# mulns/AccFlow

Hardware: AMD Instinct MI355X
Metric: frame-pairs/s (estimator pair-evals/s), AccFlow(RAFT) 7-frame 480x1024 backward accumulation (higher is better)
Workload: dtype f32 (direct-kernel operands split into 2 fp16 terms - activations kept pre-split in HBM as fp16 hi+lo, 4 B per element; other kernels 3 bf16 terms; f32 accumulate)

## Files before the change

### accflow_amd/_lib.py

```python
import ctypes
import os
import threading

_HERE = os.path.dirname(os.path.abspath(__file__))
LIB_PATH = os.environ.get("ACCFLOW_HIP_LIB") or os.path.join(_HERE, "lib", "libaccflow_hip.so")

ABI_VERSION = 20
c_f = ctypes.c_void_p
c_ll = ctypes.c_longlong
c_i = ctypes.c_int


class ConvSrc(ctypes.Structure):
    _fields_ = [
        ("ptr", c_f), ("bs", c_ll),
        ("C", c_i), ("Hs", c_i), ("Ws", c_i),
        ("step", c_i), ("oy", c_i), ("ox", c_i),
        ("KH", c_i), ("KW", c_i), ("padH", c_i), ("padW", c_i),
        ("reserved", c_i),
    ]


MAX_SRC = 4


class ConvDesc(ctypes.Structure):
    _fields_ = [
        ("in0", c_f), ("in1", c_f),
        ("in0_bs", c_ll), ("in1_bs", c_ll),
        ("C0", c_i), ("C1", c_i),
        ("B", c_i), ("H", c_i), ("W", c_i),
        ("OH", c_i), ("OW", c_i),
        ("KH", c_i), ("KW", c_i), ("stride", c_i), ("padH", c_i), ("padW", c_i),
        ("Cout", c_i),
        ("wpack", c_f), ("ktab", c_f),
        ("Kpad", c_i), ("CoutPad", c_i),
        ("bias", c_f),
        ("out", c_f), ("out_bs", c_ll),
        ("act", c_i), ("epi", c_i),
        ("e0", c_f), ("e0_bs", c_ll),
        ("e1", c_f), ("e1_bs", c_ll),
        ("out2", c_f), ("out2_bs", c_ll),
        ("offset", c_f), ("offset_bs", c_ll),
        ("dmask", c_f), ("dmask_bs", c_ll),
        ("wsplit", c_f), ("mode", c_i),
        ("wpatch", c_f),
        ("wsplit_bs", c_ll),
        ("kws", c_f), ("kws_elems", c_ll),
        ("wpatch16", c_f), ("guard", c_f),
        ("wscale16", c_f), ("wsplit16", c_f), 
        ("stats", c_f), ("stat_slots", c_i), ("pre", c_f), ("pre_bs", c_ll), ("in_norm", c_f), ("acc_scale", ctypes.c_float),
        ("in_fmt", c_i), ("out16", c_f), ("out16_bs", c_ll),
        ("cb", c_i), ("out_cbs", c_ll), ("e0_cbs", c_ll), ("out16_cbs", c_ll),
        ("nsrc", c_i), ("src", ConvSrc * MAX_SRC),
        ("e0_fmt", c_i),
        ("tg_w16", c_f), ("tg_scale", c_f), ("tg_out", c_f), ("tg_out_bs", c_ll), ("tg_out_ps", c_ll),
        ("tg_rows", c_i), ("tg_coutpad", c_i),
        ("split_c0", c_i), ("p32", c_i),
    ]


SIGNATURES = {
    "accflow_abi_version": [],
    "accflow_conv_desc_bytes": [],
    "accflow_conv_src_bytes": [],
    "accflow_s16_item_words": [c_i, c_i, c_i],
    "accflow_to_s16_f32": [c_f, c_ll, c_f, c_ll, c_f, c_i, c_i, c_i, c_f],
    "accflow_conv_kpad": [c_i, c_i, c_i],
    "accflow_conv_coutpad": [c_i],
    "accflow_conv_pack_f32": [c_f, c_f, c_i, c_i, c_i, c_i, c_i, c_i, c_f, c_f, c_f],
    "accflow_conv_pack_bf16s": [c_f, c_f, c_i, c_i, c_i, c_i, c_f, c_f],
    "accflow_conv_patch_elems": [c_i, c_i, c_i, c_i],
    "accflow_conv_pack_patch": [c_f, c_f, c_i, c_i, c_i, c_i, c_f, c_f],
    "accflow_conv_pack_patch16": [c_f, c_f, c_i, c_i, c_i, c_i, c_f, c_f, c_f],
    "accflow_conv_pack_split16": [c_f, c_f, c_i, c_i, c_i, c_i, c_f, c_f, c_f],
    "accflow_conv_multi_pack_elems": [c_i, c_i, ctypes.POINTER(c_i), ctypes.POINTER(c_i), ctypes.POINTER(c_i)],
    "accflow_conv_pack_multi16": [ctypes.POINTER(c_f), c_f, c_i, c_i, ctypes.POINTER(c_i), ctypes.POINTER(c_i), ctypes.POINTER(c_i),
                                  c_f, c_f, c_f],
    "accflow_conv2d_f32": [ctypes.POINTER(ConvDesc), c_f],
    "accflow_conv_stat_slots": [ctypes.POINTER(ConvDesc)],
    "accflow_conv_in_norm_supported": [ctypes.POINTER(ConvDesc)],
    "accflow_conv_plan_query": [ctypes.POINTER(ConvDesc), ctypes.POINTER(c_i), c_i],
    "accflow_conv_gru16_supported": [],
    "accflow_instance_stats_finalize_f32": [c_f, c_i, c_f, c_i, c_i, ctypes.c_float, c_f],
    "accflow_instance_norm_apply_f32": [c_f, c_f, c_i, c_f, c_f, c_f, c_i, c_i, c_i, ctypes.c_float, c_i, c_f],
    "accflow_instance_norm_apply_s16_f32": [c_f, c_f, c_i, c_f, c_f, c_f, c_f, c_ll, c_f, c_i, c_i, c_i, ctypes.c_float, c_i, c_f],
    "accflow_instance_norm_apply_s16res_f32": [c_f, c_f, c_i, c_f, c_f, c_ll, c_f, c_f, c_ll, c_f, c_i, c_i, c_i, ctypes.c_float, c_f],
    "accflow_instance_stats_finalize_sub_f32": [c_f, c_i, c_i, c_i, c_f, c_i, c_i, ctypes.c_float, c_f],
    "accflow_instance_norm_apply_s16proj_f32": [c_f, c_f, c_i, c_f, c_ll, c_f, c_i, c_i, c_i, c_f, c_f, c_ll, c_f, c_i, c_i, c_i,
                                                ctypes.c_float, c_f],
    "accflow_get_occ_s16": [c_f, c_ll, c_f, c_ll, c_f, c_ll, c_f, c_ll, c_f, c_i, c_i, c_i, c_i, c_i, c_f],
    "accflow_blend_s16": [c_f, c_f, c_f, c_f, c_ll, c_f, c_i, c_i, c_i, c_f],
    "accflow_deform_columns_s16": [c_f, c_ll, c_f, c_ll, c_f, c_ll, c_i, c_f, c_ll, c_f, c_i, c_i, c_i, c_i, c_i, c_i, c_i, c_i, c_f],
    "accflow_corr_volume_f32": [c_f, c_f, c_f, c_f, c_f, c_f, c_i, c_i, c_i, c_i, c_f],
    "accflow_corr_volume_ws_bytes": [c_i, c_i, c_i],
    "accflow_corr_volume_split_f32": [c_f, c_f, c_f, c_f, c_f, c_f, c_f, c_i, c_i, c_i, c_i, c_i, c_f],
    "accflow_corr_lookup_f32": [c_f, c_f, c_f, c_f, c_f, c_f, c_ll, c_i, c_i, c_i, c_f],
    "accflow_corr_lookup_r3_f32": [c_f, c_f, c_f, c_f, c_f, c_f, c_ll, c_i, c_i, c_i, c_f],
    "accflow_corr_disp_supported": [c_i, c_i],
    "accflow_corr_disp_level_elems": [c_i, c_i, c_i],
    "accflow_corr_volume_disp_f32": [c_f, c_f, c_f, c_f, c_f, c_f, c_f, c_i, c_f, c_i, c_i, c_i, c_i, c_f],
    "accflow_corr_pack_bytes": [c_i, c_i, c_i],
    "accflow_corr_pack_f32": [c_f, c_f, c_i, c_f, c_i, c_i, c_i, c_i, c_f],
    "accflow_corr_volume_disp_packed_f32": [c_f, c_i, ctypes.POINTER(c_i), ctypes.POINTER(c_i), c_f, c_f, c_f, c_f, c_i, c_f, c_i, c_i, c_i,
                                            c_i, c_f],
    "accflow_corr_disp_pool_f32": [c_f, c_f, c_f, c_f, c_i, c_i, c_i, c_f],
    "accflow_corr_lookup_disp_f32": [c_f, c_f, c_f, c_f, c_f, c_f, c_ll, c_i, c_i, c_i, c_f],
    "accflow_corr_lookup_disp_s16": [c_f, c_f, c_f, c_f, c_f, c_f, c_ll, c_f, c_i, c_i, c_i, c_f],
    "accflow_corr_alt_pyramid_elems": [c_i, c_i, c_i],
    "accflow_corr_alt_pyramid_f32": [c_f, c_f, c_i, c_i, c_i, c_i, c_f],
    "accflow_corr_lookup_alt_f32": [c_f, c_i, c_f, c_f, c_f, c_ll, c_i, c_i, c_i, c_i, c_f],
    "accflow_corr_lookup_alt_s16": [c_f, c_i, c_f, c_f, c_f, c_ll, c_f, c_i, c_i, c_i, c_i, c_f],
    "accflow_corr_lookup_convc1_kpad": [],
    "accflow_corr_lookup_convc1_s16": [c_f, c_f, c_f, c_f, c_f, c_f, c_f, c_f, c_f, c_ll, c_f, c_ll, c_i, c_f, c_i, c_i, c_i, c_i, c_f],
    "accflow_flow_from_coords_s16": [c_f, c_f, c_ll, c_f, c_ll, c_f, c_ll, c_f, c_ll, c_i, c_f, c_i, c_i, c_i, c_i, c_f],
    "accflow_convex_upsample_f32": [c_f, c_ll, c_f, c_ll, c_f, c_i, c_i, c_i, c_f],
    "accflow_backwarp_f32": [c_f, c_ll, c_f, c_ll, c_f, c_ll, c_i, c_i, c_i, c_i, c_f],
    "accflow_compose_flow_f32": [c_f, c_ll, c_f, c_ll, c_f, c_ll, c_i, c_i, c_i, c_f],
    "accflow_get_occ_f32": [c_f, c_ll, c_f, c_ll, c_f, c_ll, c_f, c_ll, c_i, c_i, c_i, c_i, c_i, c_f],
    "accflow_downflow8_f32": [c_f, c_f, c_i, c_i, c_i, c_i, c_f],
    "accflow_upflow8_f32": [c_f, c_ll, c_f, c_ll, c_i, c_i, c_i, c_f],
    "accflow_forward_interpolate_f32": [c_f, c_f, c_i, c_i, c_i, c_f],
    "accflow_fb_occlusion_f32": [c_f, c_ll, c_f, c_ll, c_f, c_ll, c_f, c_ll, ctypes.c_float, ctypes.c_float, c_i, c_i, c_i, c_f],
    "accflow_flow_metrics_ws_bytes": [c_i, c_i, c_i],
    "accflow_flow_metrics_f32": [c_f, c_ll, c_f, c_ll, c_f, c_ll, c_f, c_ll, c_i, ctypes.c_float, ctypes.c_float, c_f, c_f, c_i, c_i,
                                 c_i, c_f],
    "accflow_instance_norm_f32": [c_f, c_f, c_f, c_i, c_i, c_i, ctypes.c_float, c_i, c_f],
    "accflow_split_tanh_relu_f32": [c_f, c_f, c_ll, c_f, c_ll, c_i, c_i, c_i, c_i, c_f],
    "accflow_split_tanh_relu_idx_f32": [c_f, c_i, ctypes.POINTER(c_i), c_f, c_ll, c_f, c_ll, c_i, c_i, c_i, c_i, c_f],
    "accflow_coords_grid_f32": [c_f, c_f, c_i, c_i, c_i, c_f],
    "accflow_flow_from_coords_f32": [c_f, c_f, c_ll, c_f, c_ll, c_f, c_i, c_i, c_i, c_i, c_f],
    "accflow_deform_columns_f32": [c_f, c_ll, c_f, c_ll, c_f, c_ll, c_f, c_i, c_i, c_i, c_i, c_i, c_i, c_i, c_i, c_f],
    "accflow_conv_pack_all_f32": [c_f, c_f, c_i, c_i, c_i, c_i, c_i, c_i, c_i, c_f, c_f, c_f, c_f, c_f, c_f, c_f, c_f],
    "accflow_tap_sum_f32": [c_f, c_f, c_f, c_ll, c_f, c_ll, c_i, c_i, c_i, c_i, c_i, c_i, c_i, c_i, c_i, c_i, c_f],
    "accflow_tap_sum_parts_f32": [c_f, c_i, c_ll, c_ll, c_f, c_f, c_ll, c_f, c_ll, c_i, c_i, c_i, c_i, c_i, c_i, c_i, c_i, c_i, c_i, c_f],
    "accflow_blend_f32": [c_f, c_f, c_f, c_f, c_i, c_i, c_i, c_f],
    "accflow_activation_f32": [c_f, c_ll, c_i, c_i, c_i, c_i, c_f],
    "accflow_copy_f32": [c_f, c_ll, c_f, c_ll, c_i, c_i, c_i, c_f],
    "accflow_gma_attention_f32": [c_f, c_f, c_i, c_i, c_i, ctypes.c_float, c_f],
    "accflow_gma_attention_ws_bytes": [c_i, c_i, c_i],
    "accflow_gma_attention_t_f32": [c_f, c_f, c_f, c_i, c_i, c_i, c_i, c_i, ctypes.c_float, c_f],
    "accflow_gma_aggregate_ws_bytes": [c_i, c_i, c_i],
    "accflow_gma_attention_s16_ws_bytes": [c_i, c_i, c_i],
    "accflow_gma_attention_s16": [c_f, c_f, c_f, c_f, c_i, c_i, c_i, c_i, ctypes.c_float, c_f],
    "accflow_gma_aggregate_s16_ws_bytes": [c_i, c_i, c_i],
    "accflow_gma_aggregate_s16": [c_f, c_f, c_f, c_ll, c_f, c_f, c_ll, c_f, c_ll, c_f, c_f, c_i, c_i, c_i, c_i, c_f],
    "accflow_gma_attention_alt_ws_bytes": [c_i, c_i, c_i],
    "accflow_gma_attention_alt": [c_f, c_f, c_f, c_f, c_f, c_f, c_i, c_i, c_i, c_i, ctypes.c_float, c_f],
    "accflow_gma_aggregate_alt_ws_bytes": [c_i, c_i, c_i],
    "accflow_gma_aggregate_alt": [c_f, c_f, c_f, c_f, c_f, c_ll, c_f, c_f, c_ll, c_f, c_ll, c_f, c_f, c_i, c_i, c_i, c_i, c_f],
    "accflow_gma_aggregate_t_f32": [c_f, c_f, c_f, c_f, c_f, c_ll, c_f, c_i, c_f, c_i, c_i, c_i, c_i, c_f],
    "accflow_gma_aggregate_f32": [c_f, c_f, c_f, c_f, c_f, c_ll, c_i, c_i, c_i, c_f],
    "accflow_gma_pos_tables_f32": [c_f, c_f, c_f, c_f, c_i, c_i, c_i, c_i, c_i, ctypes.c_float, c_f],
    "accflow_gma_attention_pos_f32": [c_f, c_f, c_f, c_i, c_i, c_i, c_i, c_i, ctypes.c_float, c_f],
    "accflow_gma_attention_pos_ws_bytes": [c_i, c_i, c_i, c_i, c_i],
    "accflow_gma_attention_pos_t": [c_f, c_f, c_f, c_f, c_f, c_i, c_i, c_i, c_i, c_i, c_i, ctypes.c_float, c_f],
    "accflow_act_backward_f32": [c_f, c_ll, c_f, c_ll, c_f, c_ll, c_i, c_ll, c_i, c_f],
    "accflow_add_f32": [c_f, c_ll, c_f, c_ll, c_i, c_ll, c_f],
    "accflow_l1_grad_f32": [c_f, c_f, c_f, c_ll, ctypes.c_float, c_f],
    "accflow_dilate_f32": [c_f, c_ll, c_f, c_i, c_i, c_i, c_i, c_i, c_i, c_i, c_f],
    "accflow_blend_backward_f32": [c_f, c_f, c_f, c_f, c_f, c_f, c_f, c_i, c_i, c_i, c_f],
    "accflow_convex_upsample_backward_f32": [c_f, c_f, c_f, c_f, c_f, c_i, c_i, c_i, c_f],
    "accflow_conv_wgrad_f32": [c_f, c_ll, c_f, c_ll, c_f, c_f, c_i, c_i, c_i, c_i, c_i, c_i, c_i, c_i, c_i, c_i, c_f],
    "accflow_deform_conv_backward_f32": [c_f, c_ll, c_f, c_ll, c_f, c_ll, c_f, c_f, c_ll, c_f, c_f, c_i, c_i, c_i, c_i, c_i, c_i, c_i,
                                         c_i, c_f],
}

RETURNS_LONGLONG = frozenset((
    "accflow_conv_patch_elems", "accflow_conv_multi_pack_elems", "accflow_corr_pack_bytes", "accflow_corr_volume_ws_bytes",
    "accflow_gma_aggregate_ws_bytes", "accflow_gma_attention_ws_bytes", "accflow_gma_aggregate_s16_ws_bytes",
    "accflow_gma_attention_s16_ws_bytes", "accflow_gma_attention_alt_ws_bytes", "accflow_gma_aggregate_alt_ws_bytes",
    "accflow_corr_disp_level_elems", "accflow_corr_alt_pyramid_elems", "accflow_s16_item_words",
    "accflow_gma_attention_pos_ws_bytes", "accflow_flow_metrics_ws_bytes",
))

_lock = threading.Lock()
_lib = None


def _promote_hip_runtime():
    import torch
    cand = os.path.join(os.path.dirname(torch.__file__), "lib", "libamdhip64.so")
    if os.path.exists(cand):
        ctypes.CDLL(cand, mode=ctypes.RTLD_GLOBAL)
    else:
        ctypes.CDLL("libamdhip64.so", mode=ctypes.RTLD_GLOBAL)


def load():
    global _lib
    if _lib is not None:
        return _lib
    with _lock:
        if _lib is not None:
            return _lib
        if not os.path.exists(LIB_PATH):
            raise RuntimeError(
                "accflow_amd: %s not found - run `python -m accflow_amd.build` (hipcc, gfx950). "
                "There is no non-HIP fallback." % LIB_PATH)
        _promote_hip_runtime()
        lib = ctypes.CDLL(LIB_PATH)
        for name, argtypes in SIGNATURES.items():
            fn = getattr(lib, name)
            fn.argtypes = argtypes
            fn.restype = ctypes.c_longlong if name in RETURNS_LONGLONG else ctypes.c_int
        if lib.accflow_abi_version() != ABI_VERSION:
            raise RuntimeError("accflow_amd: ABI version mismatch")
        if (lib.accflow_conv_desc_bytes() != ctypes.sizeof(ConvDesc) or lib.accflow_conv_src_bytes() != ctypes.sizeof(ConvSrc)):
            raise RuntimeError("accflow_amd: accflow_conv_desc is %d / %d bytes in the library, %d / %d in _lib.py's mirror" % (
                lib.accflow_conv_desc_bytes(), lib.accflow_conv_src_bytes(), ctypes.sizeof(ConvDesc), ctypes.sizeof(ConvSrc)))
        _lib = lib
    return _lib
# ... 1 lines not shown
```

### accflow_amd/csrc/conv2d_direct.hip

```cpp
#include "conv2d_direct_kernel.h"

namespace {

__global__ __launch_bounds__(256) void conv_ksplit_reduce_kernel(const accflow_conv_desc d, int Z) {
  const int OHW = d.OH * d.OW;
  const long long n = (long long)d.B * d.Cout * OHW;
  const long long i = (long long)blockIdx.x * 256 + threadIdx.x;
  if (i >= n) return;
  const int px = (int)(i % OHW);
  const int ch = (int)((i / OHW) % d.Cout);
  const int b = (int)(i / ((long long)OHW * d.Cout));
  float v = d.kws[i];
  for (int z = 1; z < Z; ++z) v += d.kws[(long long)z * n + i];
  v = fmaf(v, d.wscale16 ? d.wscale16[(d.wsplit_bs ? (long long)b * d.CoutPad : 0) + ch] : 1.0f, d.bias ? d.bias[ch] : 0.0f);
  if (d.pre && (d.epi == ACCFLOW_EPI_GRU_ZR || d.epi == ACCFLOW_EPI_GRU_Q)) v += d.pre[b * d.pre_bs + (long long)ch * OHW + px];
  v = apply_act(v, d.act);
  const long long o = (long long)ch * OHW + px;
  const int half = d.Cout >> 1;
  if (d.cb) {
    const int blk = ch / d.cb;
    const long long oc = (long long)(ch - blk * d.cb) * OHW + px;
    const float r = d.epi == ACCFLOW_EPI_ACCUM ? d.e0[b * d.e0_bs + blk * d.e0_cbs + oc] + v : v;
    d.out[b * d.out_bs + blk * d.out_cbs + oc] = r;
    return;
  }
  switch (d.epi) {
    case ACCFLOW_EPI_RES_RELU: d.out[b * d.out_bs + o] = fmaxf(d.e0[b * d.e0_bs + o] + v, 0.0f); break;
    case ACCFLOW_EPI_GRU_ZR:
      if (ch < half) d.out[b * d.out_bs + o] = v;
      else d.out2[b * d.out2_bs + o - (long long)half * OHW] = v * d.e0[b * d.e0_bs + o - (long long)half * OHW];
      break;
    case ACCFLOW_EPI_GRU_Q: {
      const float z = d.e1[b * d.e1_bs + o], h = d.e0[b * d.e0_bs + o];
      d.out[b * d.out_bs + o] = gru_blend(z, h, v);
    } break;
    case ACCFLOW_EPI_ACCUM: d.out[b * d.out_bs + o] = d.e0[b * d.e0_bs + o] + v; break;
    default: d.out[b * d.out_bs + o] = v;
  }
}


__global__ __launch_bounds__(256) void conv_ksplit_reduce_s16_kernel(const accflow_conv_desc d, int Z) {
  const int OHW = d.OH * d.OW;
  const int O = (d.Cout + 7) >> 3;
  const long long n = (long long)d.B * d.Cout * OHW;
  const long long i = (long long)blockIdx.x * 256 + threadIdx.x;
  if (i >= (long long)d.B * O * OHW) return;
  const int px = (int)(i % OHW);
  const int oct = (int)((i / OHW) % O);
  const int b = (int)(i / ((long long)OHW * O));
  const int half = d.Cout >> 1;
  const bool zr = d.epi == ACCFLOW_EPI_GRU_ZR;
  float res[8];
  bool in16[8];
#pragma unroll
  for (int j = 0; j < 8; ++j) {
    const int ch = oct * 8 + j;
    res[j] = 0.0f;
    in16[j] = false;
    if (ch >= d.Cout) continue;
    const long long e = ((long long)b * d.Cout + ch) * OHW + px;
    float v = d.kws[e];
    for (int z = 1; z < Z; ++z) v += d.kws[(long long)z * n + e];
    v = fmaf(v, d.wscale16 ? d.wscale16[(d.wsplit_bs ? (long long)b * d.CoutPad : 0) + ch] : 1.0f, d.bias ? d.bias[ch] : 0.0f);
    if (d.pre && (zr || d.epi == ACCFLOW_EPI_GRU_Q)) v += d.pre[b * d.pre_bs + (long long)ch * OHW + px];
    v = apply_act(v, d.act);
    const long long o = (long long)ch * OHW + px;
    float r = v;
    if (d.cb) {
      const int blk = ch / d.cb;
      const long long oc = (long long)(ch - blk * d.cb) * OHW + px;
      r = d.epi == ACCFLOW_EPI_ACCUM ? d.e0[b * d.e0_bs + blk * d.e0_cbs + oc] + v : v;
      if (d.out) d.out[b * d.out_bs + blk * d.out_cbs + oc] = r;
      res[j] = r;
      in16[j] = true;
      continue;
    }
    switch (d.epi) {
      case ACCFLOW_EPI_RES_RELU: r = fmaxf(d.e0[b * d.e0_bs + o] + v, 0.0f); break;
      case ACCFLOW_EPI_GRU_ZR:
        if (ch >= half) r = v * d.e0[b * d.e0_bs + o - (long long)half * OHW];
        break;
      case ACCFLOW_EPI_GRU_Q: {
        const float z = d.e1[b * d.e1_bs + o], h = d.e0[b * d.e0_bs + o];
        r = gru_blend(z, h, v);
      } break;
      case ACCFLOW_EPI_ACCUM: r = d.e0[b * d.e0_bs + o] + v; break;
      default: break;
    }
    if (zr && ch >= half) {
      if (d.out2) d.out2[b * d.out2_bs + o - (long long)half * OHW] = r;
    } else if (d.out) {
      d.out[b * d.out_bs + o] = r;
    }
    res[j] = r;
    in16[j] = !zr || ch >= half;
  }
  if (!d.out16) return;
  const int c16 = oct * 8 - (zr ? half : 0);
  if (c16 < 0) return;
  const int n16 = zr ? half : d.Cout;
  const int nvalid = min(8, ((n16 + 1) & ~1) - c16);
  constexpr float ASC = (float)(1 << ACCFLOW_F16_ASHIFT);
  unsigned hi[4], lo[4];
  bool bad = false;
#pragma unroll
  for (int k = 0; k < 4; ++k) {
    const float a = in16[2 * k] ? res[2 * k] * ASC : 0.0f, c = in16[2 * k + 1] ? res[2 * k + 1] * ASC : 0.0f;
    bad |= !(fabsf(a) < 65520.0f) | !(fabsf(c) < 65520.0f);
    const f32x2 v2 = {a, c};
    const f16x2 hq = __builtin_convertvector(v2, f16x2);
    const f32x2 back = __builtin_convertvector(hq, f32x2);
    const f32x2 rest = {a - back[0], c - back[1]};
    const f16x2 lq = __builtin_convertvector(rest, f16x2);
    hi[k] = __builtin_bit_cast(unsigned, hq);
    lo[k] = __builtin_bit_cast(unsigned, lq);
  }
  unsigned* base = reinterpret_cast<unsigned*>(d.out16) + b * d.out16_bs;
  int o16 = c16 >> 3;
  if (d.cb) {
    base += (long long)(c16 / d.cb) * d.out16_cbs;
    o16 = (c16 % d.cb) >> 3;
  }
  unsigned* ph = base + (((long long)(o16 * 2 + 0)) * OHW + px) * 4;
  unsigned* pl = base + (((long long)(o16 * 2 + 1)) * OHW + px) * 4;
#pragma unroll
  for (int k = 0; k < 4; ++k)
    if (2 * k < nvalid) { ph[k] = hi[k]; pl[k] = lo[k]; }
  if (bad && d.guard) atomicOr(d.guard, 1);
}

__global__ __launch_bounds__(256) void conv_ksplit_reduce_s16q_kernel(const accflow_conv_desc d, int Z) {
  const int OHW = d.OH * d.OW;
  const int Q = d.Cout >> 2;
  const long long n = (long long)d.B * d.Cout * OHW;
  const long long i = (long long)blockIdx.x * 256 + threadIdx.x;
  if (i >= (long long)d.B * Q * OHW) return;
  const int px = (int)(i % OHW);
  const int q = (int)((i / OHW) % Q);
  const int b = (int)(i / ((long long)OHW * Q));
  float v[4];
#pragma unroll
  for (int j = 0; j < 4; ++j) v[j] = d.kws[((long long)b * d.Cout + q * 4 + j) * OHW + px];
  for (int z = 1; z < Z; ++z)
#pragma unroll
    for (int j = 0; j < 4; ++j) v[j] += d.kws[(long long)z * n + ((long long)b * d.Cout + q * 4 + j) * OHW + px];
  float res[4];
#pragma unroll
  for (int j = 0; j < 4; ++j) {
    const int ch = q * 4 + j;
    float t = fmaf(v[j], d.wscale16 ? d.wscale16[(d.wsplit_bs ? (long long)b * d.CoutPad : 0) + ch] : 1.0f, d.bias ? d.bias[ch] : 0.0f);
    if (d.pre && d.epi == ACCFLOW_EPI_GRU_Q) t += d.pre[b * d.pre_bs + (long long)ch * OHW + px];
    t = apply_act(t, d.act);
    const long long o = (long long)ch * OHW + px;
    if (d.cb) {
      const int blk = ch / d.cb;
      const long long oc = (long long)(ch - blk * d.cb) * OHW + px;
      if (d.epi == ACCFLOW_EPI_ACCUM) t = d.e0[b * d.e0_bs + blk * d.e0_cbs + oc] + t;
      if (d.out) d.out[b * d.out_bs + blk * d.out_cbs + oc] = t;
      res[j] = t;
      continue;
    }
    switch (d.epi) {
      case ACCFLOW_EPI_RES_RELU: t = fmaxf(d.e0[b * d.e0_bs + o] + t, 0.0f); break;
      case ACCFLOW_EPI_GRU_Q: {
        const float zz = d.e1[b * d.e1_bs + o], h = d.e0[b * d.e0_bs + o];
        t = gru_blend(zz, h, t);
      } break;
      case ACCFLOW_EPI_ACCUM: t = d.e0[b * d.e0_bs + o] + t; break;
      default: break;
    }
    if (d.out) d.out[b * d.out_bs + o] = t;
    res[j] = t;
  }
  constexpr float ASC = (float)(1 << ACCFLOW_F16_ASHIFT);
  unsigned hi[2], lo[2];
  bool bad = false;
#pragma unroll
  for (int k = 0; k < 2; ++k) {
    const float a = res[2 * k] * ASC, c = res[2 * k + 1] * ASC;
    bad |= !(fabsf(a) < 65520.0f) | !(fabsf(c) < 65520.0f);
    const f32x2 v2 = {a, c};
    const f16x2 hq = __builtin_convertvector(v2, f16x2);
    const f32x2 back = __builtin_convertvector(hq, f32x2);
    const f32x2 rest = {a - back[0], c - back[1]};
    const f16x2 lq = __builtin_convertvector(rest, f16x2);
    hi[k] = __builtin_bit_cast(unsigned, hq);
    lo[k] = __builtin_bit_cast(unsigned, lq);
  }
  unsigned* base = reinterpret_cast<unsigned*>(d.out16) + b * d.out16_bs;
  int oct = q >> 1;
  const int w0 = (q & 1) * 2;
  if (d.cb) {
    base += (long long)((q * 4) / d.cb) * d.out16_cbs;
    oct = ((q * 4) % d.cb) >> 3;
  }
  unsigned* ph = base + (((long long)(oct * 2 + 0)) * OHW + px) * 4 + w0;
  unsigned* pl = base + (((long long)(oct * 2 + 1)) * OHW + px) * 4 + w0;
  typedef unsigned u2_ __attribute__((ext_vector_type(2)));
  *reinterpret_cast<u2_*>(ph) = u2_{hi[0], hi[1]};
  *reinterpret_cast<u2_*>(pl) = u2_{lo[0], lo[1]};
  if (bad && d.guard) atomicOr(d.guard, 1);
}

}

int conv_ksplit_reduce_launch(const accflow_conv_desc& d, int Z, hipStream_t st) {
  if (d.out16 && !(d.Cout & 7) && !(d.cb & 7) && d.epi != ACCFLOW_EPI_GRU_ZR) {
    const long long nthr = (long long)d.B * (d.Cout / 4) * d.OH * d.OW;
    hipLaunchKernelGGL(conv_ksplit_reduce_s16q_kernel, dim3(cdiv(nthr, 256)), dim3(256), 0, st, d, Z);
  } else if (d.out16) {
    const long long nthr = (long long)d.B * ((d.Cout + 7) / 8) * d.OH * d.OW;
    hipLaunchKernelGGL(conv_ksplit_reduce_s16_kernel, dim3(cdiv(nthr, 256)), dim3(256), 0, st, d, Z);
  } else {
    const long long nout = (long long)d.B * d.Cout * d.OH * d.OW;
    hipLaunchKernelGGL(conv_ksplit_reduce_kernel, dim3(cdiv(nout, 256)), dim3(256), 0, st, d, Z);
  }
  ACCFLOW_RETURN_LAUNCH_STATUS();
}

namespace {

int launch_conv_direct(const accflow_conv_desc& d, const conv_plan& p, hipStream_t st) {
  const int tiles = cdiv(d.OW, DIR_TW) * cdiv(d.OH, DIR_TH);
  dim3 grid((unsigned)((long long)d.B * tiles), cdiv(d.Cout, 2 * p.tc * 32), p.Z);
  const bool f16 = p.mode == ACCFLOW_CONV_F16X3 && d.wpatch16;
  const int nt = p.mode == ACCFLOW_CONV_BF16X3 ? 2 : 3;
  int rc;
  if (p.tapgemm) {
    rc = p.loop == CONV_LOOP_TAP9 ? accflow_direct_launch_s16k9(d, 2, true, grid, st) : accflow_direct_launch_s16tg(d, grid, st);
  } else if (d.in_fmt) {
    if (p.loop == CONV_LOOP_TAP5) rc = accflow_direct_launch_s16k(d, 5, grid, st);
    else if (p.loop == CONV_LOOP_TAP9) rc = accflow_direct_launch_s16k9(d, p.tc, false, grid, st);
    else rc = accflow_direct_launch_s16(d, p.tc, grid, st);
  } else if (p.norm) {
// ... 447 lines not shown
```

### accflow_amd/csrc/conv_common.h

```cpp
#pragma once
#include "common.h"
#include <stdlib.h>
#include "launchers.h"

#ifndef ACCFLOW_EPI_GRU_AHEAD
#define ACCFLOW_EPI_GRU_AHEAD 3
#endif
#ifndef ACCFLOW_CONV_XCD_ORDER
#define ACCFLOW_CONV_XCD_ORDER 1
#endif
#ifndef ACCFLOW_CONV_XCD_MIN_K
#define ACCFLOW_CONV_XCD_MIN_K 8192
#endif

namespace {


struct XLoaderCtx {
  const float* base0;
  const float* base1;
  int iy0, ix0, H, W, HW;
  unsigned pixbyte0, pixbyte1;
  bool pvalid;
  const float* off;
  const float* dmk;
  int OHW, KW;
};

__device__ __forceinline__ float load_x_deform(const XLoaderCtx& c, const int4 e) {
  const float* src = e.w ? c.base1 : c.base0;
  if (!c.pvalid || e.y >= (1 << 19)) return 0.0f;
  const int tap = e.y * c.KW + e.z;
  const float dy = c.off[(2 * tap) * c.OHW], dx = c.off[(2 * tap + 1) * c.OHW];
  const float m = c.dmk[tap * c.OHW];
  const float h = (float)(c.iy0 + e.y) + dy, w = (float)(c.ix0 + e.z) + dx;
  if (!(h > -1.0f && h < (float)c.H && w > -1.0f && w < (float)c.W)) return 0.0f;
  const float* plane = src + e.x * c.HW;
  const float fh = floorf(h), fw = floorf(w);
  const int hl = (int)fh, wl = (int)fw, hh = hl + 1, wh = wl + 1;
  const float lh = h - fh, lw = w - fw, uh = 1.0f - lh, uw = 1.0f - lw;
  const float v1 = (hl >= 0 && wl >= 0) ? plane[hl * c.W + wl] : 0.0f;
  const float v2 = (hl >= 0 && wh <= c.W - 1) ? plane[hl * c.W + wh] : 0.0f;
  const float v3 = (hh <= c.H - 1 && wl >= 0) ? plane[hh * c.W + wl] : 0.0f;
  const float v4 = (hh <= c.H - 1 && wh <= c.W - 1) ? plane[hh * c.W + wh] : 0.0f;
  return m * (uh * uw * v1 + uh * lw * v2 + lh * uw * v3 + lh * lw * v4);
}

template <int CTRL>
__device__ __forceinline__ float dpp_add(float v) {
  return v + __builtin_bit_cast(float, __builtin_amdgcn_update_dpp(0, __builtin_bit_cast(int, v), CTRL, 0xF, 0xF, true));
}
__device__ __forceinline__ float row16_sum(float v) {
  v = dpp_add<0xB1>(v);
  v = dpp_add<0x4E>(v);
  v = dpp_add<0x141>(v);
  v = dpp_add<0x140>(v);
  return v;
}
__device__ __forceinline__ float half32_sum(float v) {
  v = row16_sum(v);
  return v + __builtin_bit_cast(float, __builtin_amdgcn_ds_swizzle(__builtin_bit_cast(int, v), 0x401F));
}
__device__ __forceinline__ void stat_store(const accflow_conv_desc& d, int b, int ch, int slot, float s, float m2, float n) {
  float* p = d.stats + (((long long)b * d.Cout + ch) * d.stat_slots + slot) * 3;
  p[0] = s; p[1] = m2; p[2] = n;
}

__device__ __forceinline__ float gru_blend(float z, float h, float q) { return __builtin_fmaf(z, q, (1.0f - z) * h); }

template <int EPI, int ACT, int WC, int WP, int TC, int TP, class PixMap, bool OUT16 = false>
__device__ __forceinline__ void conv_epilogue_impl(const accflow_conv_desc& d, f32x16 (&acc)[TC][TP], int cblk0, int wc,
                                                   int wp, int lane, int OHW, PixMap pixmap, int stat_b = 0,
                                                   int stat_slot = 0) {
  constexpr unsigned MASKED = 0xFFFFFFFFu;
  const int l31 = lane & 31, lh4 = (lane >> 5) * 4;
  const int epi = EPI >= 0 ? EPI : d.epi;
  const int half = d.Cout >> 1;
  const bool has_h = epi != ACCFLOW_EPI_STORE, has_z = epi == ACCFLOW_EPI_GRU_Q, zr = epi == ACCFLOW_EPI_GRU_ZR;
  const int nout = zr ? half : d.Cout;
  auto span = [&](long long bs, int nch) { return (int)(unsigned)((((long long)(d.B - 1)) * bs + (long long)nch * OHW) * 4); };
  const int cb = d.cb;
  auto chbyte = [&](int ch, long long cbs) -> int {
    if (!cb) return ch * OHW * 4;
    const int blk = ch / cb;
    return (int)(unsigned)(((long long)blk * cbs + (long long)(ch - blk * cb) * OHW) * 4);
  };
  auto span_cb = [&](long long bs, int nch, long long cbs) {
    if (!cb) return span(bs, nch);
    return (int)(unsigned)((((long long)(d.B - 1)) * bs + (long long)((nch - 1) / cb) * cbs + (long long)cb * OHW) * 4);
  };
  const __amdgpu_buffer_rsrc_t r_out =
      __builtin_amdgcn_make_buffer_rsrc(d.out, 0, d.out ? span_cb(d.out_bs, nout, d.out_cbs) : 0, 0x00020000);
  const __amdgpu_buffer_rsrc_t r_o2 =
      __builtin_amdgcn_make_buffer_rsrc(zr ? d.out2 : d.out, 0, (zr && d.out2) ? span(d.out2_bs, half) : 0, 0x00020000);
  const bool has16 = OUT16 && d.out16 != nullptr;
  const int n16 = zr ? half : d.Cout, O16 = (n16 + 7) >> 3;
  const __amdgpu_buffer_rsrc_t r_o16 = __builtin_amdgcn_make_buffer_rsrc(
      d.out16 ? d.out16 : (void*)d.out, 0,
      has16 ? (cb ? (int)(unsigned)((((long long)(d.B - 1)) * d.out16_bs + (long long)((n16 - 1) / cb) * d.out16_cbs +
                                     (long long)(cb / 8) * 2 * OHW * 4) * 4)
                  : (int)(unsigned)((((long long)(d.B - 1)) * d.out16_bs + (long long)O16 * 2 * OHW * 4) * 4)) : 0, 0x00020000);
  const __amdgpu_buffer_rsrc_t r_e0 = __builtin_amdgcn_make_buffer_rsrc(
      const_cast<float*>(has_h ? d.e0 : d.out), 0, has_h ? span_cb(d.e0_bs, zr ? half : d.Cout, d.e0_cbs) : 0, 0x00020000);
  const __amdgpu_buffer_rsrc_t r_e1 = __builtin_amdgcn_make_buffer_rsrc(
      const_cast<float*>(has_z ? d.e1 : d.out), 0, has_z ? span(d.e1_bs, d.Cout) : 0, 0x00020000);
  const bool has_pre = (EPI == ACCFLOW_EPI_GRU_ZR || EPI == ACCFLOW_EPI_GRU_Q) && d.pre != nullptr;
  const __amdgpu_buffer_rsrc_t r_pre = __builtin_amdgcn_make_buffer_rsrc(
      const_cast<float*>(has_pre ? d.pre : d.out), 0, has_pre ? span(d.pre_bs, d.Cout) : 0, 0x00020000);

  unsigned vo_out[TP], vo_o2[TP], vo_e0[TP], vo_e1[TP], vo_pre[TP], vo_16[TP];
#pragma unroll
  for (int tp = 0; tp < TP; ++tp) {
    int b;
    const int rem = pixmap(wp * TP * 32 + tp * 32 + l31, b);
    const bool ok = rem >= 0;
    const long long lp = (long long)rem + (long long)lh4 * OHW;
    vo_16[tp] = ok && has16 ? (unsigned)((b * d.out16_bs + (long long)rem * 4) * 4 + lh4 * 2) : MASKED;
    vo_out[tp] = ok ? (unsigned)((b * d.out_bs + lp) * 4) : MASKED;
    vo_o2[tp] = ok && zr ? (unsigned)((b * d.out2_bs + lp) * 4) : MASKED;
    vo_e0[tp] = ok && has_h ? (unsigned)((b * d.e0_bs + lp) * 4) : MASKED;
    vo_e1[tp] = ok && has_z ? (unsigned)((b * d.e1_bs + lp) * 4) : MASKED;
    vo_pre[tp] = ok && has_pre ? (unsigned)((b * d.pre_bs + lp) * 4) : MASKED;
  }
  const int rowbase = cblk0 + wc * TC * 32;
  const int OHW4 = OHW * 4;
  typedef const __attribute__((address_space(4))) float* cfloat_ptr;
  const cfloat_ptr sbias = (cfloat_ptr)(unsigned long long)d.bias;
  float sb0[2], sb1[2];
  const cfloat_ptr sscale = (cfloat_ptr)(unsigned long long)d.wscale16;
  float ss0[2], ss1[2];
  constexpr bool GRU_EPI = EPI == ACCFLOW_EPI_GRU_ZR || EPI == ACCFLOW_EPI_GRU_Q;
  constexpr int AH = GRU_EPI ? ACCFLOW_EPI_GRU_AHEAD : 1, NS = AH + 1;
  float h[NS][TP], z[NS][TP], pa[NS][TP];
  float s16v[TP][4];
  bool bad16 = false;
  typedef float f32x2_ __attribute__((ext_vector_type(2)));
  typedef _Float16 f16x2_ __attribute__((ext_vector_type(2)));
  typedef unsigned u32x2_ __attribute__((ext_vector_type(2)));
#pragma unroll
  for (int i = 0; i < NS; ++i)
#pragma unroll
    for (int tp = 0; tp < TP; ++tp) pa[i][tp] = 0.0f;
#define EPI_CHU(G) (rowbase + ((G) / 16) * 32 + ((G) & 3) + 8 * (((G) & 15) >> 2))
#define EPI_FETCH(G, HH, ZZ)                                                                                     \
  do {                                                                                                           \
    if (has_h) {                                                                                                 \
      const int chu_ = EPI_CHU(G);                                                                               \
      const int che_ = zr ? chu_ - half : chu_;                                                                  \
      const bool live_ = che_ >= 0;                                                                              \
      const bool in_ = chu_ + lh4 < d.Cout;                                                                      \
      _Pragma("unroll") for (int tp = 0; tp < TP; ++tp) {                                                        \
        HH[tp] = __builtin_bit_cast(float, __builtin_amdgcn_raw_buffer_load_b32(                                 \
            r_e0, (int)((live_ && in_) ? vo_e0[tp] : MASKED), live_ ? chbyte(che_, d.e0_cbs) : 0, 0));           \
        if (has_z) ZZ[tp] = __builtin_bit_cast(float, __builtin_amdgcn_raw_buffer_load_b32(                      \
            r_e1, (int)(in_ ? vo_e1[tp] : MASKED), chu_ * OHW4, 0));                                             \
        if (has_pre) pa[(G) % NS][tp] = __builtin_bit_cast(float, __builtin_amdgcn_raw_buffer_load_b32(          \
            r_pre, (int)(in_ ? vo_pre[tp] : MASKED), chu_ * OHW4, 0));                                           \
      }                                                                                                          \
    }                                                                                                            \
  } while (0)
#define EPI_BIAS(G, S)                                                                                           \
  do {                                                                                                           \
    const int chu_ = EPI_CHU(G);                                                                                 \
    sb0[S] = d.bias ? sbias[min(chu_, d.Cout - 1)] : 0.0f;                                                       \
    sb1[S] = d.bias ? sbias[min(chu_ + 4, d.Cout - 1)] : 0.0f;                                                   \
    ss0[S] = d.wscale16 ? sscale[min(chu_, d.Cout - 1)] : 1.0f;                                                  \
    ss1[S] = d.wscale16 ? sscale[min(chu_ + 4, d.Cout - 1)] : 1.0f;                                              \
  } while (0)
#pragma unroll
  for (int g0 = 0; g0 < AH && g0 < TC * 16; ++g0) EPI_FETCH(g0, h[g0 % NS], z[g0 % NS]);
  EPI_BIAS(0, 0);
  constexpr bool CAN_STATS = EPI == ACCFLOW_EPI_STORE && ACT == ACCFLOW_ACT_NONE;
  float stat_n = 0.0f;
  if constexpr (CAN_STATS) {
    if (d.stats) {
#pragma unroll
      for (int tp = 0; tp < TP; ++tp) stat_n += vo_out[tp] != MASKED ? 1.0f : 0.0f;
      stat_n = half32_sum(stat_n);
    }
  }
#pragma unroll
  for (int g = 0; g < TC * 16; ++g) {
    __builtin_amdgcn_sched_barrier(0);
    const float bv = lh4 ? sb1[g & 1] : sb0[g & 1];
    const float sv = lh4 ? ss1[g & 1] : ss0[g & 1];
    __builtin_amdgcn_sched_barrier(0);
    if (g + AH < TC * 16) EPI_FETCH(g + AH, h[(g + AH) % NS], z[(g + AH) % NS]);
    if (g + 1 < TC * 16) EPI_BIAS(g + 1, (g + 1) & 1);
    const int tc = g / 16, r = g & 15;
    const int chu = EPI_CHU(g);
    const bool in = chu + lh4 < d.Cout;
    if constexpr (CAN_STATS) {
      if (d.stats) {
        float s = 0.0f;
#pragma unroll
        for (int tp = 0; tp < TP; ++tp) s += vo_out[tp] != MASKED ? fmaf(acc[tc][tp][r], sv, bv) : 0.0f;
        s = half32_sum(s);
        const float mean = s / fmaxf(stat_n, 1.0f);
        float q = 0.0f;
#pragma unroll
        for (int tp = 0; tp < TP; ++tp) {
          const float dv = fmaf(acc[tc][tp][r], sv, bv) - mean;
          q += vo_out[tp] != MASKED ? dv * dv : 0.0f;
        }
        q = half32_sum(q);
// ... 114 lines not shown
  const bool no_scale = d.wscale16 == nullptr;
  bool bad16 = false;
  typedef float f32x2_ __attribute__((ext_vector_type(2)));
  typedef _Float16 f16x2_ __attribute__((ext_vector_type(2)));
  typedef unsigned u32x2_ __attribute__((ext_vector_type(2)));
  constexpr float ASC16 = (float)(1 << ACCFLOW_F16_ASHIFT);
#pragma unroll
  for (int tc = 0; tc < TC; ++tc)
#pragma unroll
    for (int m = 0; m < 4; ++m) {
      float o[TP][4];
#pragma unroll
      for (int q = 0; q < 4; ++q) {
        const int r = 4 * m + q;
        const float s = no_scale ? 1.0f : sv[tc][m][q];
        const int so = (rowbase + tc * 32 + 8 * m + q) * OHW4;
#pragma unroll
        for (int tp = 0; tp < TP; ++tp) {
          float v = fmaf(acc[tc][tp][r], s, bv[tc][m][q]) + 0.0f;
          if (ACT == ACCFLOW_ACT_RELU) v = fmaxf(v, 0.0f);
          o[tp][q] = v;
#ifndef ACCFLOW_KPROF_NOSTORE
          if (!p32o) __builtin_amdgcn_raw_buffer_store_b32(__builtin_bit_cast(unsigned, v), r_out, (int)vo_out[tp], so, 0);
#endif
        }
      }
      if (p32o) {
        const int so32 = ((rowbase + tc * 32 + 8 * m) >> 3) * OHW * 32;
#pragma unroll
        for (int tp = 0; tp < TP; ++tp) {
          const u32x4_ pv = {__builtin_bit_cast(unsigned, o[tp][0]), __builtin_bit_cast(unsigned, o[tp][1]),
                             __builtin_bit_cast(unsigned, o[tp][2]), __builtin_bit_cast(unsigned, o[tp][3])};
          __builtin_amdgcn_raw_buffer_store_b128(pv, r_out, (int)vo_out[tp], so32, 0);
        }
      }
      if (has16) {
        const int so16 = ((rowbase + tc * 32 + 8 * m) >> 3) * 2 * OHW * 16;
#pragma unroll
        for (int tp = 0; tp < TP; ++tp) {
          unsigned hi2[2], lo2[2];
#pragma unroll
          for (int k = 0; k < 2; ++k) {
            const float a = o[tp][2 * k] * ASC16, b = o[tp][2 * k + 1] * ASC16;
            bad16 |= !(fabsf(a) < 65520.0f) | !(fabsf(b) < 65520.0f);
            const f32x2_ v2 = {a, b};
            const f16x2_ hq = __builtin_convertvector(v2, f16x2_);
            const f32x2_ back = __builtin_convertvector(hq, f32x2_);
            const f32x2_ rest = {a - back[0], b - back[1]};
            const f16x2_ lq = __builtin_convertvector(rest, f16x2_);
            hi2[k] = __builtin_bit_cast(unsigned, hq);
            lo2[k] = __builtin_bit_cast(unsigned, lq);
          }
          const u32x2_ hv = {hi2[0], hi2[1]}, lv = {lo2[0], lo2[1]};
#ifndef ACCFLOW_KPROF_NOSTORE
          __builtin_amdgcn_raw_buffer_store_b64(hv, r_o16, (int)vo_16[tp], so16, 0);
          __builtin_amdgcn_raw_buffer_store_b64(lv, r_o16, (int)vo_16[tp], so16 + OHW * 16, 0);
#endif
        }
      }
    }
  if (has16 && bad16 && d.guard) atomicOr(d.guard, 1);
}


template <bool ZR, int TP, class PixMap>
__device__ __forceinline__ void conv_epilogue_gru16(const accflow_conv_desc& d, f32x16 (&acc)[1][TP], int cblk0, int wc, int lane,
                                                    int OHW, PixMap pixmap) {
  static_assert(TP == 4, "the 4 x 1 wave layout: 32 channels x 128 pixels per wave");
  constexpr unsigned MASKED = 0xFFFFFFFFu;
  constexpr int TPH = 2;
  typedef float f32x4_ __attribute__((ext_vector_type(4)));
  typedef float f32x2_ __attribute__((ext_vector_type(2)));
  typedef _Float16 f16x2_ __attribute__((ext_vector_type(2)));
  typedef unsigned u32x2_ __attribute__((ext_vector_type(2)));
  typedef unsigned u32x4_ __attribute__((ext_vector_type(4)));
  const int l31 = lane & 31, lh4 = (lane >> 5) * 4;
  const int rowbase = cblk0 + wc * 32;
  const int half = d.Cout >> 1;
  const bool zrow = ZR && rowbase < half;
  const bool need_h = !zrow;
  const int nst = ZR ? half : d.Cout;
  const int cst = ZR ? rowbase - half : rowbase;
  auto rng = [&](long long bs, int nch) { return (int)(unsigned)((((long long)(d.B - 1)) * bs + (long long)nch * OHW) * 4); };
  const __amdgpu_buffer_rsrc_t r_pre = __builtin_amdgcn_make_buffer_rsrc(const_cast<float*>(d.pre), 0, rng(d.pre_bs, d.Cout), 0x00020000);
  const __amdgpu_buffer_rsrc_t r_z = __builtin_amdgcn_make_buffer_rsrc(ZR ? (float*)d.out : const_cast<float*>(d.e1), 0,
                                                                      ZR ? rng(d.out_bs, half) : rng(d.e1_bs, d.Cout), 0x00020000);
  const int s16rng = (int)(unsigned)((((long long)(d.B - 1)) * d.e0_bs + (long long)((nst + 7) >> 3) * 2 * OHW * 4) * 4);
  const __amdgpu_buffer_rsrc_t r_h = __builtin_amdgcn_make_buffer_rsrc(const_cast<float*>(d.e0), 0, s16rng, 0x00020000);
  const __amdgpu_buffer_rsrc_t r_o16 = __builtin_amdgcn_make_buffer_rsrc(
      d.out16, 0, (int)(unsigned)((((long long)(d.B - 1)) * d.out16_bs + (long long)((nst + 7) >> 3) * 2 * OHW * 4) * 4), 0x00020000);
  const __amdgpu_buffer_rsrc_t r_b = __builtin_amdgcn_make_buffer_rsrc(const_cast<float*>(d.bias ? d.bias : d.wscale16), 0,
                                                                      d.bias ? d.Cout * 4 : 0, 0x00020000);
  const __amdgpu_buffer_rsrc_t r_s = __builtin_amdgcn_make_buffer_rsrc(const_cast<float*>(d.wscale16), 0, d.CoutPad * 4, 0x00020000);
  constexpr float ASC16 = (float)(1 << ACCFLOW_F16_ASHIFT);
  bool bad16 = false;
#pragma unroll
  for (int hh = 0; hh < TP / TPH; ++hh) {
    unsigned vo_p[TPH], vo_z[TPH], vo_h[TPH], vo_o[TPH];
#pragma unroll
    for (int t = 0; t < TPH; ++t) {
      int b;
      const int rem = pixmap((hh * TPH + t) * 32 + l31, b);
      const bool ok = rem >= 0;
      vo_p[t] = ok ? (unsigned)((b * d.pre_bs + (long long)rem * 8 + lh4) * 4) : MASKED;
      vo_z[t] = ok ? (unsigned)((b * (ZR ? d.out_bs : d.e1_bs) + (long long)rem * 8 + lh4) * 4) : MASKED;
      vo_h[t] = ok ? (unsigned)((b * d.e0_bs + (long long)rem * 4) * 4 + lh4 * 2) : MASKED;
      vo_o[t] = ok ? (unsigned)((b * d.out16_bs + (long long)rem * 4) * 4 + lh4 * 2) : MASKED;
    }
    f32x4_ pre[2][TPH], zz[2][TPH], bv[2], sv[2];
    u32x2_ hhi[2][TPH], hlo[2][TPH];
#define GRU16_FETCH(M, S)                                                                                          \
    do {                                                                                                           \
      const int ch_ = rowbase + 8 * (M);                             \
      bv[S] = __builtin_bit_cast(f32x4_, __builtin_amdgcn_raw_buffer_load_b128(r_b, (ch_ + lh4) * 4, 0, 0));       \
      sv[S] = __builtin_bit_cast(f32x4_, __builtin_amdgcn_raw_buffer_load_b128(r_s, (ch_ + lh4) * 4, 0, 0));       \
      const int sop_ = (ch_ >> 3) * OHW * 32;                           \
      const int so16_ = ((cst + 8 * (M)) >> 3) * 2 * OHW * 16;                   \
      _Pragma("unroll") for (int t = 0; t < TPH; ++t) {                                                            \
        pre[S][t] = __builtin_bit_cast(f32x4_, __builtin_amdgcn_raw_buffer_load_b128(r_pre, (int)vo_p[t], sop_, 0)); \
        if (!ZR) zz[S][t] = __builtin_bit_cast(f32x4_, __builtin_amdgcn_raw_buffer_load_b128(r_z, (int)vo_z[t], sop_, 0)); \
        if (need_h) {                                                                                              \
          hhi[S][t] = __builtin_bit_cast(u32x2_, __builtin_amdgcn_raw_buffer_load_b64(r_h, (int)vo_h[t], so16_, 0)); \
          hlo[S][t] = __builtin_bit_cast(u32x2_, __builtin_amdgcn_raw_buffer_load_b64(r_h, (int)vo_h[t], so16_ + OHW * 16, 0)); \
        }                                                                                                          \
      }                                                                                                            \
    } while (0)
    GRU16_FETCH(0, 0);
#pragma unroll
    for (int m = 0; m < 4; ++m) {
      const int S = m & 1;
      if (m + 1 < 4) GRU16_FETCH(m + 1, S ^ 1);
#pragma unroll
      for (int t = 0; t < TPH; ++t) {
        const int tp = hh * TPH + t;
        float o[4];
#pragma unroll
        for (int q = 0; q < 4; ++q) {
          const float v = apply_act(fmaf(acc[0][tp][4 * m + q], sv[S][q], bv[S][q]) + pre[S][t][q],
                                    ZR ? ACCFLOW_ACT_SIGMOID : ACCFLOW_ACT_TANH);
          if (need_h) {
            const unsigned wh = hhi[S][t][q >> 1], wl = hlo[S][t][q >> 1];
            const unsigned short hq = (unsigned short)((q & 1) ? wh >> 16 : wh & 0xFFFFu), lq = (unsigned short)((q & 1) ? wl >> 16 : wl & 0xFFFFu);
            const float hv = ((float)__builtin_bit_cast(_Float16, hq) + (float)__builtin_bit_cast(_Float16, lq)) * (1.0f / ASC16);
            o[q] = ZR ? v * hv : gru_blend(zz[S][t][q], hv, v);
          } else {
            o[q] = v;
          }
        }
        if (zrow) {
          const u32x4_ pv = {__builtin_bit_cast(unsigned, o[0]), __builtin_bit_cast(unsigned, o[1]), __builtin_bit_cast(unsigned, o[2]),
                             __builtin_bit_cast(unsigned, o[3])};
          __builtin_amdgcn_raw_buffer_store_b128(pv, r_z, (int)vo_z[t], ((rowbase + 8 * m) >> 3) * OHW * 32, 0);
        } else {
          unsigned hi2[2], lo2[2];
#pragma unroll
          for (int k = 0; k < 2; ++k) {
            const float a = o[2 * k] * ASC16, b2 = o[2 * k + 1] * ASC16;
            bad16 |= !(fabsf(a) < 65520.0f) | !(fabsf(b2) < 65520.0f);
            const f32x2_ v2 = {a, b2};
            const f16x2_ hq2 = __builtin_convertvector(v2, f16x2_);
            const f32x2_ back = __builtin_convertvector(hq2, f32x2_);
            const f32x2_ rest = {a - back[0], b2 - back[1]};
            const f16x2_ lq2 = __builtin_convertvector(rest, f16x2_);
            hi2[k] = __builtin_bit_cast(unsigned, hq2);
            lo2[k] = __builtin_bit_cast(unsigned, lq2);
          }
          const u32x2_ hv2 = {hi2[0], hi2[1]}, lv2 = {lo2[0], lo2[1]};
          const int so16 = ((cst + 8 * m) >> 3) * 2 * OHW * 16;
          __builtin_amdgcn_raw_buffer_store_b64(hv2, r_o16, (int)vo_o[t], so16, 0);
          __builtin_amdgcn_raw_buffer_store_b64(lv2, r_o16, (int)vo_o[t], so16 + OHW * 16, 0);
        }
      }
    }
#undef GRU16_FETCH
  }
  if (bad16 && d.guard) atomicOr(d.guard, 1);
}

template <int WC, int WP, int TC, int TP, class PixMap, bool OUT16 = false>
__device__ __forceinline__ void conv_epilogue_px(const accflow_conv_desc& d, f32x16 (&acc)[TC][TP], int cblk0, int wc,
                                                 int wp, int lane, int OHW, PixMap pixmap, int stat_b = 0,
                                                 int stat_slot = 0) {
#define ACCFLOW_EPI_CASE(E, A)                                                                          \
  case (E) * 8 + (A): conv_epilogue_impl<E, A, WC, WP, TC, TP, PixMap, OUT16>(d, acc, cblk0, wc, wp, lane, OHW, pixmap, stat_b, stat_slot); break;
  switch (d.epi * 8 + d.act) {
    ACCFLOW_EPI_CASE(ACCFLOW_EPI_STORE, ACCFLOW_ACT_NONE)
    ACCFLOW_EPI_CASE(ACCFLOW_EPI_STORE, ACCFLOW_ACT_RELU)
// ... 245 lines not shown
```

### accflow_amd/csrc/conv_plan.cpp

```cpp
#include "conv_plan.h"
#include <stdlib.h>

namespace {

inline int cdiv(long long a, long long b) { return (int)((a + b - 1) / b); }

long long env_ll(const char* name, long long dflt) {
  const char* e = getenv(name);
  return e ? atoll(e) : dflt;
}

int fill_parts(long long nb) {
  int Z = 1;
  double best = 0.0;
  for (int z = 1; z <= 8; ++z) {
    const double fill = (double)(nb * z) / (double)(cdiv(nb * z, 768) * 768);
    if (fill > best + 0.03) { best = fill; Z = z; }
  }
  return Z;
}

int conv_split_k(const accflow_conv_desc& d, bool want_stats, long long nb, bool deep, int zenv, int nchunk) {
  if (!d.kws || want_stats || d.e0_fmt || d.split_c0) return 1;
  if (d.out16 && d.epi == ACCFLOW_EPI_GRU_ZR && ((d.Cout >> 1) & 7)) return 1;
// ... 166 lines not shown
  auto tile = [&](int wc, int wp, int tc, int tp) { p.wc = wc; p.wp = wp; p.tc = tc; p.tp = tp; return 0; };
  constexpr long long MIN_BLOCKS = 384;
  if (d.Cout <= 32) return tile(1, 4, 1, blocks(32, 256) >= MIN_BLOCKS ? 2 : 1);
  if (d.Cout <= 64) return tile(2, 2, 1, blocks(64, 128) >= MIN_BLOCKS ? 2 : 1);
  if (d.Cout % 96 == 0 && d.Cout % 128 != 0 && blocks(96, 128) >= MIN_BLOCKS) return tile(1, 4, 3, 1);
  if (blocks(128, 128) >= MIN_BLOCKS) return tile(2, 2, 2, 2);
  if (blocks(128, 64) >= MIN_BLOCKS) return tile(2, 2, 2, 1);
  return tile(2, 2, 1, 1);
}

}

const conv_switches& conv_switches_get() {
  static const conv_switches sw = [] {
    conv_switches s;
    s.direct_w4 = env_ll("ACCFLOW_DIRECT_W4", 1) != 0;
    s.direct_kt = env_ll("ACCFLOW_DIRECT_KT", 1) != 0;
    s.direct_kt9 = env_ll("ACCFLOW_DIRECT_KT9", 1) != 0;
    s.s16m = env_ll("ACCFLOW_S16M", 0) != 0;
    s.s16m_kt9 = env_ll("ACCFLOW_S16M_KT9", 1) != 0;
    s.s16m_lay = (int)env_ll("ACCFLOW_S16M_LAY", -1);
    s.stem = env_ll("ACCFLOW_CONV_STEM", 1) != 0;
    s.patch_min_blocks = env_ll("ACCFLOW_PATCH_MIN_BLOCKS", 300);
    s.direct_ksplit = (int)env_ll("ACCFLOW_DIRECT_KSPLIT", 0);
    s.im2col_ksplit = (int)env_ll("ACCFLOW_IM2COL_KSPLIT", 0);
    return s;
  }();
  return sw;
}

extern "C" long long accflow_s16_item_words(int C, int H, int W) {
  return (long long)((C + 7) / 8) * 2 * H * W * 4;
}

extern "C" int accflow_conv_kpad(int Cin, int KH, int KW) {
  const int K = Cin * KH * KW;
  return (K + 31) / 32 * 32;
}

extern "C" int accflow_conv_coutpad(int Cout) { return (Cout + 127) / 128 * 128; }

extern "C" int accflow_conv_gru16_supported(void) {
  const conv_switches& sw = conv_switches_get();
  return sw.direct_kt && sw.direct_w4 && !sw.s16m ? 1 : 0;
}

bool accflow_conv_direct_eligible(const accflow_conv_desc& d) {
  if (!d.wpatch || d.wsplit_bs || d.mode == ACCFLOW_CONV_F32 || d.offset || d.stride != 1 || d.Cout <= 4) return false;
  if (d.OH != d.H || d.OW != d.W) return false;
  if ((DIR_TH + d.KH - 1) * (DIR_TW + d.KW - 1) > DIR_NPMAX) return false;
  if (d.C0 + d.C1 < 16) return false;
  if (d.in1 && (d.C0 % (d.KH * d.KW == 1 ? 32 : 16))) return false;
  return true;
}

int conv_validate(const accflow_conv_desc* desc, accflow_conv_desc& dd) {
  if (!desc) return 1;
  dd = *desc;
  if (dd.mode == ACCFLOW_CONV_F16X3 && (dd.wpatch16 || dd.wsplit16) && !dd.wscale16) return 1;
  if (dd.mode != ACCFLOW_CONV_F16X3) { dd.wpatch16 = nullptr; dd.wsplit16 = nullptr; }
  if (!dd.wpatch16 && !dd.wsplit16) dd.wscale16 = nullptr;
  dd.acc_scale = 0.0f;
  if (dd.nsrc < 0 || dd.nsrc > ACCFLOW_CONV_MAX_SRC) return 1;
  const bool gru16 = !dd.nsrc && dd.e0_fmt;
  if (gru16 && !(dd.in_fmt == (dd.in1 ? 3 : 1) && dd.e0 && dd.pre && dd.out16 && dd.mode == ACCFLOW_CONV_F16X3 && !dd.cb && !dd.kws &&
                 dd.KH * dd.KW == 5 && dd.stride == 1 && accflow_conv_gru16_supported() && !dd.stats &&
                 ((dd.epi == ACCFLOW_EPI_GRU_ZR && dd.p32 == 3 && dd.out && dd.Cout == 256) ||
                  (dd.epi == ACCFLOW_EPI_GRU_Q && dd.p32 == 6 && dd.e1 && dd.Cout == 128))))
    return 1;
  if (!gru16 && dd.p32 && !(dd.p32 == 1 && !dd.nsrc && dd.in_fmt == (dd.in1 ? 3 : 1) && dd.mode == ACCFLOW_CONV_F16X3 && dd.out && !dd.out16 &&
                            dd.epi == ACCFLOW_EPI_STORE && (dd.act == ACCFLOW_ACT_NONE || dd.act == ACCFLOW_ACT_RELU) && !dd.cb &&
                            !dd.kws && !dd.stats && dd.stride == 1 && (dd.Cout % 128) == 0 && accflow_conv_gru16_supported()))
    return 1;
  const bool multi = dd.nsrc > 0;
  if (multi) {
    if (dd.mode != ACCFLOW_CONV_F16X3 || !dd.wpatch16 || dd.in_norm || dd.offset || dd.wsplit_bs) return 1;
    dd.in_fmt = 0; dd.in0 = nullptr; dd.in1 = nullptr; dd.H = dd.OH; dd.W = dd.OW;
    dd.CoutPad = accflow_conv_coutpad(dd.Cout);
  }
  const accflow_conv_desc& d = dd;
  if ((!multi && (!d.in0 || !d.wpack || !d.ktab)) || d.B <= 0 || d.Cout <= 0 || d.OH <= 0 || d.OW <= 0) return 1;
  if (d.epi == ACCFLOW_EPI_TAPGEMM) {
    if (multi || d.mode != ACCFLOW_CONV_F16X3 || !d.wpatch16 || !d.wscale16 || d.in_fmt != (d.in1 ? 3 : 1) || d.act != ACCFLOW_ACT_RELU ||
        (d.Cout & 127) || d.kws || d.stats || d.in_norm || d.cb || d.pre || d.offset || !d.tg_w16 || !d.tg_scale || !d.tg_out ||
        d.tg_rows < 1 || d.tg_rows > ACCFLOW_TAPGEMM_MAXROWS || d.tg_coutpad < 32 || (d.tg_coutpad & 31) ||
        d.tg_out_bs < (long long)d.tg_rows * d.OH * d.OW || (d.Cout > 128 && d.tg_out_ps <= 0) || !accflow_conv_direct_eligible(d) ||
        d.Kpad != accflow_conv_kpad(d.C0 + d.C1, d.KH, d.KW) || d.CoutPad != accflow_conv_coutpad(d.Cout))
      return 1;
    if ((((long long)(d.B - 1)) * d.in0_bs + accflow_s16_item_words(d.C0, d.H, d.W)) * 4 >= (1LL << 32)) return 1;
    if (d.in1 && (((long long)(d.B - 1)) * d.in1_bs + accflow_s16_item_words(d.C1, d.H, d.W)) * 4 >= (1LL << 32)) return 1;
    return 0;
  }
  if (!d.out && (!d.out16 || d.epi == ACCFLOW_EPI_GRU_ZR)) return 1;
  if (d.epi == ACCFLOW_EPI_GRU_ZR && !d.out2 && !d.out16) return 1;
  if ((d.in_fmt || d.out16) && d.mode != ACCFLOW_CONV_F16X3) return 1;
  if (d.in_fmt & ~3) return 1;
  if (d.out16) {
    const int ea = d.epi * 8 + d.act;
    if (ea != ACCFLOW_EPI_STORE * 8 + ACCFLOW_ACT_NONE && ea != ACCFLOW_EPI_STORE * 8 + ACCFLOW_ACT_RELU &&
        ea != ACCFLOW_EPI_STORE * 8 + ACCFLOW_ACT_SIGMOID && ea != ACCFLOW_EPI_RES_RELU * 8 + ACCFLOW_ACT_RELU &&
        ea != ACCFLOW_EPI_RES_RELU * 8 + ACCFLOW_ACT_NONE &&
        ea != ACCFLOW_EPI_GRU_ZR * 8 + ACCFLOW_ACT_SIGMOID && ea != ACCFLOW_EPI_GRU_Q * 8 + ACCFLOW_ACT_TANH &&
        ea != ACCFLOW_EPI_ACCUM * 8 + ACCFLOW_ACT_NONE)
      return 1;
  }
  if (d.cb && ((d.cb & 31) || (d.epi != ACCFLOW_EPI_STORE && d.epi != ACCFLOW_EPI_ACCUM) || d.stats || d.Cout % d.cb)) return 1;
  if (!multi && (d.Kpad != accflow_conv_kpad(d.C0 + d.C1, d.KH, d.KW) || d.CoutPad != accflow_conv_coutpad(d.Cout))) return 1;
  if ((d.epi == ACCFLOW_EPI_RES_RELU || d.epi == ACCFLOW_EPI_ACCUM) && !d.e0) return 1;
  if (d.epi == ACCFLOW_EPI_GRU_ZR && (!d.e0 || (d.Cout & 1))) return 1;
  if (d.epi == ACCFLOW_EPI_GRU_ZR && d.out16 && ((d.Cout >> 1) & 7)) return 1;
  if (d.epi == ACCFLOW_EPI_GRU_Q && (!d.e0 || !d.e1)) return 1;
  if (d.pre && d.epi != ACCFLOW_EPI_GRU_ZR && d.epi != ACCFLOW_EPI_GRU_Q) return 1;
  if (d.offset && !d.dmask) return 1;
  if ((long long)d.B * d.OH * d.OW >= (1LL << 31)) return 1;
  if (!multi) {
    const long long w0 = (d.in_fmt & 1) ? accflow_s16_item_words(d.C0, d.H, d.W) : (long long)d.C0 * d.H * d.W;
    const long long w1 = (d.in_fmt & 2) ? accflow_s16_item_words(d.C1, d.H, d.W) : (long long)d.C1 * d.H * d.W;
    if ((((long long)(d.B - 1)) * d.in0_bs + w0) * 4 >= (1LL << 32)) return 1;
    if (d.in1 && (((long long)(d.B - 1)) * d.in1_bs + w1) * 4 >= (1LL << 32)) return 1;
  }
  if (d.out16 && (((long long)(d.B - 1)) * d.out16_bs + accflow_s16_item_words(d.Cout, d.OH, d.OW)) * 4 >= (1LL << 32)) return 1;
  if (d.stats && (d.epi != ACCFLOW_EPI_STORE || d.act != ACCFLOW_ACT_NONE || d.stat_slots <= 0)) return 1;
  return 0;
}

int conv_plan_direct(const accflow_conv_desc& d, int tc, bool want_stats, conv_plan& p) {
  if (!accflow_conv_direct_eligible(d)) return 1;
  const int rc = plan_direct_tile(d, tc, want_stats, p);
  if (!rc && tc == 2)
    p.ch0 = conv_tail_ch0(d, want_stats, (long long)d.B * cdiv(d.OW, DIR_TW) * cdiv(d.OH, DIR_TH) * cdiv(d.Cout, 128));
  return rc;
}

void conv_tail_split(const accflow_conv_desc& d, int ch0, accflow_conv_desc& head, accflow_conv_desc& tail) {
  const long long OHW = (long long)d.OH * d.OW;
  head = d;
  tail = d;
  head.Cout = ch0;
  tail.Cout = d.Cout - ch0;
  tail.out = d.out ? d.out + ch0 * OHW : nullptr;
  if (d.bias) tail.bias = d.bias + ch0;
  if (d.wscale16) tail.wscale16 = d.wscale16 + ch0;
  if (d.e0) tail.e0 = d.e0 + ch0 * OHW;
  if (d.out16) tail.out16 = reinterpret_cast<char*>(d.out16) + (long long)(ch0 / 8) * 2 * OHW * 16;
  if (d.wpatch) tail.wpatch = reinterpret_cast<const char*>(d.wpatch) + (long long)ch0 * 16;
  if (d.wpatch16) tail.wpatch16 = reinterpret_cast<const char*>(d.wpatch16) + (long long)ch0 * 16;
}

int conv_plan_part(const accflow_conv_desc& part, const conv_plan& whole, bool tail, conv_plan& p) {
  if (whole.family == CONV_FAM_S16M) return plan_s16m_lay(part, tail ? 2 : 0, false, p);
  return plan_direct_tile(part, tail ? 1 : 2, false, p);
}

int conv_make_plan(accflow_conv_desc& d, bool want_stats, conv_plan& p) {
  const conv_switches& sw = conv_switches_get();
  if (d.epi == ACCFLOW_EPI_TAPGEMM) return conv_plan_direct(d, 2, want_stats, p);
  if (d.nsrc > 0) return plan_s16m(d, want_stats, p);
  if (sw.stem && stem_eligible(d)) {
    plan_init(p, CONV_FAM_STEM, d.mode);
    p.slots = cdiv(d.OW, ST_TW) * cdiv(d.OH, ST_TH) * 2;
    return 0;
  }
  if (d.in_fmt && sw.s16m) {
    if (!accflow_conv_direct_eligible(d) || !d.wpatch16 || d.in_norm) return 1;
    if (d.in_fmt != (d.in1 ? 3 : 1)) return 1;
    s16m_from_legacy(d);
    return plan_s16m(d, want_stats, p);
  }
  if (d.in_fmt || d.out16 || d.cb) {
    if (!d.wpatch16 || d.stats || d.in_norm) return 1;
    if (d.in_fmt && d.in_fmt != (d.in1 ? 3 : 1)) return 1;
    return conv_plan_direct(d, d.Cout > 64 ? 2 : 1, want_stats, p);
  }
  if (d.Cout <= 4 && !d.offset && (d.epi == ACCFLOW_EPI_STORE || d.epi == ACCFLOW_EPI_ACCUM || d.epi == ACCFLOW_EPI_RES_RELU)) {
    const bool same = d.stride == 1 && d.OH == d.H && d.OW == d.W && d.KH * d.KW >= 2 && d.C0 + d.C1 >= 16 &&
                      (8 + d.KH - 1) * (16 + d.KW - 1) <= 192 && d.KH * d.KW <= 25 && (!d.in1 || d.C0 % 16 == 0);
    plan_init(p, same ? CONV_FAM_SMALL_PATCH : CONV_FAM_SMALL, d.mode);
    return 0;
  }
  if (accflow_conv_direct_eligible(d)) {
    const long long nb = (long long)d.B * cdiv(d.OW, DIR_TW) * cdiv(d.OH, DIR_TH);
    const long long minb = (d.kws && (d.KH * d.KW >= 2 || d.C0 + d.C1 >= 512)) ? 0 : sw.patch_min_blocks;
    if (d.Cout > 64 && nb * cdiv(d.Cout, 128) >= minb) return conv_plan_direct(d, 2, want_stats, p);
    if (nb * cdiv(d.Cout, 64) >= minb) return conv_plan_direct(d, 1, want_stats, p);
  }
  if (d.mode == ACCFLOW_CONV_F16X3 && !(d.wsplit16 && !d.offset && d.Cout > 32)) {
    d.mode = ACCFLOW_CONV_BF16X6;
    d.wpatch = nullptr;
    d.wpatch16 = nullptr; d.wsplit16 = nullptr; d.wscale16 = nullptr;
  }
  if (d.wsplit_bs) {
    if ((d.OH * d.OW) % 64) return 1;
    if (d.mode != ACCFLOW_CONV_F16X3 && (d.mode == ACCFLOW_CONV_F32 || !d.wsplit || d.offset || d.Cout <= 32)) return 1;
    return plan_im2col(d, d.Cout > 64 ? 2 : 1, 1, want_stats, true, p);
  }
// ... 8 lines not shown
```

### accflow_amd/csrc/misc.hip

```cpp
#include "common.h"

namespace {

__device__ __forceinline__ double block_sum(double v, double* red) {
#pragma unroll
  for (int o = 32; o > 0; o >>= 1) v += __shfl_xor(v, o, 64);
  const int lane = threadIdx.x & 63, wave = threadIdx.x >> 6, nw = blockDim.x >> 6;
  __syncthreads();
  if (lane == 0) red[wave] = v;
  __syncthreads();
  double t = 0.0;
  for (int i = 0; i < nw; ++i) t += red[i];
  return t;
}

__global__ __launch_bounds__(512) void instance_norm_kernel(const float* x, const float* res,
                                                            float* out, int HW, float eps, int mode) {
  __shared__ double red[8];
  const long long base = (long long)blockIdx.x * HW;
  const float* p = x + base;
  const bool vec = (HW & 3) == 0;
  double s = 0.0;
  if (vec) {
    const float4* p4 = reinterpret_cast<const float4*>(p);
// ... 60 lines not shown
  for (int u = 0; u < MAXR; ++u) { s += (double)rs[u]; n += (double)rn[u]; }
  for (int i = tid + 256 * MAXR; i < slots; i += 256) { s += (double)p[3 * i]; n += (double)p[3 * i + 2]; }
  for (int off = 32; off > 0; off >>= 1) { s += __shfl_xor(s, off, 64); n += __shfl_xor(n, off, 64); }
  if (lane == 0) { red[0][wave] = s; red[1][wave] = n; }
  __syncthreads();
  s = ((red[0][0] + red[0][1]) + red[0][2]) + red[0][3];
  n = ((red[1][0] + red[1][1]) + red[1][2]) + red[1][3];
  const double mean = n > 0.0 ? s / n : 0.0;
  double m2 = 0.0;
#pragma unroll
  for (int u = 0; u < MAXR; ++u) {
    const double nb = rn[u];
    if (nb > 0.0) {
      const double dd = (double)rs[u] - nb * mean;
      m2 += (double)rm[u] + dd * dd / nb;
    }
  }
  for (int i = tid + 256 * MAXR; i < slots; i += 256) {
    const double nb = p[3 * i + 2];
    if (nb > 0.0) {
      const double dd = (double)p[3 * i] - nb * mean;
      m2 += (double)p[3 * i + 1] + dd * dd / nb;
    }
  }
  for (int off = 32; off > 0; off >>= 1) m2 += __shfl_xor(m2, off, 64);
  if (lane == 0) red[2][wave] = m2;
  __syncthreads();
  if (tid == 0) {
    m2 = ((red[2][0] + red[2][1]) + red[2][2]) + red[2][3];
    const double var = n > 0.0 ? m2 / n : 0.0;
    meanrstd[2 * plane] = (float)mean;
    meanrstd[2 * plane + 1] = (float)(1.0 / sqrt(var + (double)eps));
  }
}
static void launch_finalize(const float* stats, int slots, int Ctot, int c0, float* mr, int B, int C, float eps, hipStream_t st,
                            const float* stats2 = nullptr, int slots2 = 0, int Ctot2 = 0, int c02 = 0, float* mr2 = nullptr) {
  finalize_args a0{stats, slots, Ctot, c0, mr}, a1{stats2, slots2, Ctot2, c02, mr2};
  hipLaunchKernelGGL(instance_stats_finalize_kernel, dim3((unsigned)((long long)B * C), stats2 ? 2 : 1), dim3(256), 0, st, a0, a1,
                     eps, C);
}

__global__ __launch_bounds__(256) void instance_norm_apply_kernel(const float* __restrict__ x, const float* __restrict__ meanrstd,
                                                                  const float* __restrict__ res, float* __restrict__ out,
                                                                  int HW, long long total, int mode) {
  const long long i4 = ((long long)blockIdx.x * 256 + threadIdx.x) * 4;
  if (i4 >= total) return;
  if ((HW & 3) == 0) {
    const long long plane = i4 / HW;
    const float mean = meanrstd[2 * plane], rstd = meanrstd[2 * plane + 1];
    const float4 v = *reinterpret_cast<const float4*>(x + i4);
    float o[4] = {(v.x - mean) * rstd, (v.y - mean) * rstd, (v.z - mean) * rstd, (v.w - mean) * rstd};
    if (mode >= 1)
      for (int k = 0; k < 4; ++k) o[k] = fmaxf(o[k], 0.0f);
    if (mode == 2) {
      const float4 r = *reinterpret_cast<const float4*>(res + i4);
      o[0] = fmaxf(r.x + o[0], 0.0f); o[1] = fmaxf(r.y + o[1], 0.0f); o[2] = fmaxf(r.z + o[2], 0.0f); o[3] = fmaxf(r.w + o[3], 0.0f);
    }
    *reinterpret_cast<float4*>(out + i4) = make_float4(o[0], o[1], o[2], o[3]);
  } else {
    for (long long i = i4; i < i4 + 4 && i < total; ++i) {
      const long long plane = i / HW;
      float v = (x[i] - meanrstd[2 * plane]) * meanrstd[2 * plane + 1];
      if (mode >= 1) v = fmaxf(v, 0.0f);
      if (mode == 2) v = fmaxf(res[i] + v, 0.0f);
      out[i] = v;
    }
  }
}

__global__ void split_tanh_relu_kernel(const float* __restrict__ cnet, float* __restrict__ net, long long net_bs,
                                       float* __restrict__ inp, long long inp_bs, int B, int hd, int cd, int HW) {
  const long long per = (long long)(hd + cd) * HW;
  const long long g = (long long)blockIdx.x * blockDim.x + threadIdx.x;
  if (g >= B * per) return;
  const int b = (int)(g / per);
  const long long r = g - b * per;
  const int c = (int)(r / HW), pix = (int)(r - (long long)c * HW);
  const float v = cnet[g];
  if (c < hd) net[b * net_bs + (long long)c * HW + pix] = tanhf(v);
  else inp[b * inp_bs + (long long)(c - hd) * HW + pix] = fmaxf(v, 0.0f);
}

struct split_idx { int v[64]; };
__global__ void split_tanh_relu_idx_kernel(const float* __restrict__ cnet, split_idx idx, float* __restrict__ net,
                                           long long net_bs, float* __restrict__ inp, long long inp_bs, int B, int hd, int cd,
                                           int HW) {
  const long long per = (long long)(hd + cd) * HW;
  const long long g = (long long)blockIdx.x * blockDim.x + threadIdx.x;
  if (g >= B * per) return;
  const int b = (int)(g / per);
  const long long r = g - b * per;
  const int c = (int)(r / HW), pix = (int)(r - (long long)c * HW);
  const float v = cnet[(long long)idx.v[b] * per + r];
  if (c < hd) net[b * net_bs + (long long)c * HW + pix] = tanhf(v);
  else inp[b * inp_bs + (long long)(c - hd) * HW + pix] = fmaxf(v, 0.0f);
}

__global__ void coords_grid_kernel(float* __restrict__ coords, const float* __restrict__ flow_init, int B, int H8,
                                   int W8) {
  const int P = H8 * W8;
  const long long g = (long long)blockIdx.x * blockDim.x + threadIdx.x;
  if (g >= (long long)B * 2 * P) return;
  const int pix = (int)(g % P), ch = (int)((g / P) & 1);
  const int y = pix / W8, x = pix - y * W8;
  float v = ch == 0 ? (float)x : (float)y;
  if (flow_init) v += flow_init[g];
  coords[g] = v;
}

__global__ void flow_from_coords_kernel(const float* __restrict__ coords1, float* __restrict__ dst0,
                                        long long dst0_bs, float* __restrict__ dst1, long long dst1_bs,
                                        float* __restrict__ stack, int B, int H8, int W8, int is_flow) {
  const int P = H8 * W8;
  const long long g = (long long)blockIdx.x * blockDim.x + threadIdx.x;
  if (g >= (long long)B * 2 * P) return;
  const int b = (int)(g / (2 * P));
  const int r = (int)(g - (long long)b * 2 * P);
  const int ch = r / P, pix = r - ch * P;
  const int y = pix / W8, x = pix - y * W8;
  const float v = is_flow ? coords1[g] : coords1[g] - (ch == 0 ? (float)x : (float)y);
  if (dst0) dst0[b * dst0_bs + r] = v;
  if (dst1) dst1[b * dst1_bs + r] = v;
  if (stack) {
    float* s = stack + (long long)b * 16 * P + pix;
#pragma unroll
    for (int ky = 0; ky < 7; ++ky) {
      const int ys = y + ky - 3;
      const bool ok = (unsigned)ys < (unsigned)H8;
      const float c = ok ? coords1[g + (long long)(ky - 3) * W8] : 0.0f;
      const float u = (ok && !is_flow) ? c - (ch == 0 ? (float)x : (float)ys) : c;
      s[(long long)(ch * 7 + ky) * P] = u;
    }
    s[(long long)(14 + ch) * P] = 0.0f;
  }
}

__global__ __launch_bounds__(256) void flow_from_coords_s16_kernel(const float* __restrict__ coords1, float* __restrict__ dst0,
                                                                   long long dst0_bs, float* __restrict__ dst1, long long dst1_bs,
                                                                   mu32x4* __restrict__ stack, long long stack_bs,
                                                                   unsigned* __restrict__ motion, long long motion_bs, int motion_ch,
                                                                   int* guard, int B, int H8, int W8, int is_flow) {
  const int P = H8 * W8;
  const long long g = (long long)blockIdx.x * 256 + threadIdx.x;
  if (g >= (long long)B * P) return;
  const int b = (int)(g / P), pix = (int)(g - (long long)b * P);
  const int y = pix / W8, x = pix - y * W8;
  const float* c = coords1 + (long long)b * 2 * P + pix;
  float st[16];
#pragma unroll
  for (int ch = 0; ch < 2; ++ch)
#pragma unroll
    for (int ky = 0; ky < 7; ++ky) {
      const int ys = y + ky - 3;
      const bool ok = (unsigned)ys < (unsigned)H8;
      const float cv = ok ? c[(long long)ch * P + (long long)(ky - 3) * W8] : 0.0f;
      st[ch * 7 + ky] = (ok && !is_flow) ? cv - (ch == 0 ? (float)x : (float)ys) : cv;
    }
  st[14] = 0.0f; st[15] = 0.0f;
  const float fx = st[3], fy = st[10];
  if (dst0) { dst0[b * dst0_bs + pix] = fx; dst0[b * dst0_bs + P + pix] = fy; }
  if (dst1) { dst1[b * dst1_bs + pix] = fx; dst1[b * dst1_bs + P + pix] = fy; }
  bool bad = false;
  if (stack) {
    mu32x4* sb = stack + (b * stack_bs) / 4;
#pragma unroll
    for (int o = 0; o < 2; ++o) {
      float v[8];
#pragma unroll
      for (int j = 0; j < 8; ++j) v[j] = st[o * 8 + j];
      mu32x4 hi, lo;
      s16_split8(v, hi, lo, bad);
      sb[((long long)(o * 2 + 0)) * P + pix] = hi;
      sb[((long long)(o * 2 + 1)) * P + pix] = lo;
    }
  }
  if (motion) {
    float v[8] = {fx, fy, 0.0f, 0.0f, 0.0f, 0.0f, 0.0f, 0.0f};
    mu32x4 hi, lo;
// ... 186 lines not shown
  hipLaunchKernelGGL(instance_norm_kernel, dim3((unsigned)((long long)B * C)), dim3(512), 0, as_stream(stream), x, res,
                     out, HW, eps, mode);
  ACCFLOW_RETURN_LAUNCH_STATUS();
}

extern "C" int accflow_instance_stats_finalize_f32(const float* stats, int slots, float* meanrstd, int B, int C, float eps,
                                                   void* stream) {
  if (!stats || !meanrstd || slots <= 0 || B <= 0 || C <= 0) return 1;
  launch_finalize(stats, slots, C, 0, meanrstd, B, C, eps, as_stream(stream));
  ACCFLOW_RETURN_LAUNCH_STATUS();
}

extern "C" int accflow_instance_stats_finalize_sub_f32(const float* stats, int slots, int Ctot, int c0, float* meanrstd, int B,
                                                       int C, float eps, void* stream) {
  if (!stats || !meanrstd || slots <= 0 || B <= 0 || C <= 0 || c0 < 0 || c0 + C > Ctot) return 1;
  launch_finalize(stats, slots, Ctot, c0, meanrstd, B, C, eps, as_stream(stream));
  ACCFLOW_RETURN_LAUNCH_STATUS();
}

extern "C" int accflow_instance_norm_apply_s16proj_f32(const float* x, const float* stats, int slots, const float* res,
                                                       long long res_bs, const float* res_stats, int res_slots, int res_ctot,
                                                       int res_c0, float* meanrstd, void* out16, long long out16_bs, int* guard,
                                                       int B, int C, int HW, float eps, void* stream) {
  if (!x || !stats || !res || !res_stats || !meanrstd || !out16 || slots <= 0 || res_slots <= 0 || B <= 0 || C <= 0 || HW <= 0 ||
      res_c0 < 0 || res_c0 + C > res_ctot)
    return 1;
  hipStream_t st = as_stream(stream);
  float* mr3 = meanrstd + 2LL * B * C;
  launch_finalize(stats, slots, C, 0, meanrstd, B, C, eps, st, res_stats, res_slots, res_ctot, res_c0, mr3);
  const long long n = (long long)B * ((C + 7) / 8) * HW;
  hipLaunchKernelGGL(instance_norm_apply_s16proj_kernel, dim3(cdiv(n, 256)), dim3(256), 0, st, x, meanrstd, res, res_bs, mr3,
                     reinterpret_cast<mu32x4*>(out16), out16_bs, guard, B, C, HW);
  ACCFLOW_RETURN_LAUNCH_STATUS();
}

extern "C" int accflow_instance_norm_apply_f32(const float* x, const float* stats, int slots, float* meanrstd,
                                               const float* res, float* out, int B, int C, int HW, float eps, int mode,
                                               void* stream) {
  if (!x || !stats || !meanrstd || !out || slots <= 0 || B <= 0 || C <= 0 || HW <= 0 || mode < 0 || mode > 2 ||
      (mode == 2 && !res))
    return 1;
  const long long total = (long long)B * C * HW;
  launch_finalize(stats, slots, C, 0, meanrstd, B, C, eps, as_stream(stream));
  hipLaunchKernelGGL(instance_norm_apply_kernel, dim3(cdiv(cdiv(total, 4), 256)), dim3(256), 0, as_stream(stream), x,
                     meanrstd, res, out, HW, total, mode);
  ACCFLOW_RETURN_LAUNCH_STATUS();
}

extern "C" int accflow_instance_norm_apply_s16_f32(const float* x, const float* stats, int slots, float* meanrstd,
                                                   const float* res, float* out, void* out16, long long out16_bs, int* guard,
                                                   int B, int C, int HW, float eps, int mode, void* stream) {
  if (!x || !stats || !meanrstd || !out16 || slots <= 0 || B <= 0 || C <= 0 || HW <= 0 || mode < 0 || mode > 2 ||
      (mode == 2 && !res))
    return 1;
  launch_finalize(stats, slots, C, 0, meanrstd, B, C, eps, as_stream(stream));
  const long long n = (long long)B * ((C + 7) / 8) * HW;
  hipLaunchKernelGGL(instance_norm_apply_s16_kernel, dim3(cdiv(n, 256)), dim3(256), 0, as_stream(stream), x, meanrstd, res,
                     out, reinterpret_cast<mu32x4*>(out16), out16_bs, guard, B, C, HW, mode);
  ACCFLOW_RETURN_LAUNCH_STATUS();
}

extern "C" int accflow_instance_norm_apply_s16res_f32(const float* x, const float* stats, int slots, float* meanrstd,
                                                      const void* res16, long long res16_bs, float* out, void* out16,
                                                      long long out16_bs, int* guard, int B, int C, int HW, float eps,
                                                      void* stream) {
  if (!x || !stats || !meanrstd || !res16 || !out16 || slots <= 0 || B <= 0 || C <= 0 || HW <= 0) return 1;
  launch_finalize(stats, slots, C, 0, meanrstd, B, C, eps, as_stream(stream));
  const long long n = (long long)B * ((C + 7) / 8) * HW;
  hipLaunchKernelGGL(instance_norm_apply_s16res_kernel, dim3(cdiv(n, 256)), dim3(256), 0, as_stream(stream), x, meanrstd,
                     reinterpret_cast<const mu32x4*>(res16), res16_bs, out, reinterpret_cast<mu32x4*>(out16), out16_bs, guard,
                     B, C, HW);
  ACCFLOW_RETURN_LAUNCH_STATUS();
}

extern "C" int accflow_split_tanh_relu_f32(const float* cnet, float* net, long long net_bs, float* inp,
                                           long long inp_bs, int B, int hd, int cd, int HW, void* stream) {
  if (!cnet || !net || !inp || B <= 0 || hd <= 0 || cd <= 0 || HW <= 0) return 1;
  const long long n = (long long)B * (hd + cd) * HW;
  hipLaunchKernelGGL(split_tanh_relu_kernel, dim3(cdiv(n, 256)), dim3(256), 0, as_stream(stream), cnet, net, net_bs,
                     inp, inp_bs, B, hd, cd, HW);
  ACCFLOW_RETURN_LAUNCH_STATUS();
}

extern "C" int accflow_split_tanh_relu_idx_f32(const float* cnet, int n_items, const int* idx, float* net, long long net_bs,
                                               float* inp, long long inp_bs, int B, int hd, int cd, int HW, void* stream) {
  if (!cnet || !idx || !net || !inp || n_items <= 0 || B <= 0 || hd <= 0 || cd <= 0 || HW <= 0) return 1;
  for (int b = 0; b < B; ++b)
    if (idx[b] < 0 || idx[b] >= n_items) return 1;
  for (int b0 = 0; b0 < B; b0 += 64) {
    const int nb = B - b0 < 64 ? B - b0 : 64;
    split_idx a;
    for (int k = 0; k < 64; ++k) a.v[k] = k < nb ? idx[b0 + k] : 0;
    const long long n = (long long)nb * (hd + cd) * HW;
    hipLaunchKernelGGL(split_tanh_relu_idx_kernel, dim3(cdiv(n, 256)), dim3(256), 0, as_stream(stream), cnet, a,
                       net + b0 * net_bs, net_bs, inp + b0 * inp_bs, inp_bs, nb, hd, cd, HW);
  }
  ACCFLOW_RETURN_LAUNCH_STATUS();
}

extern "C" int accflow_coords_grid_f32(float* coords, const float* flow_init, int B, int H8, int W8, void* stream) {
  if (!coords || B <= 0 || H8 <= 0 || W8 <= 0) return 1;
  const long long n = (long long)B * 2 * H8 * W8;
  hipLaunchKernelGGL(coords_grid_kernel, dim3(cdiv(n, 256)), dim3(256), 0, as_stream(stream), coords, flow_init, B, H8,
                     W8);
  ACCFLOW_RETURN_LAUNCH_STATUS();
}

extern "C" int accflow_flow_from_coords_f32(const float* coords1, float* dst0, long long dst0_bs, float* dst1,
                                            long long dst1_bs, float* stack16, int is_flow, int B, int H8, int W8,
                                            void* stream) {
  if (!coords1 || (!dst0 && !dst1 && !stack16) || B <= 0 || H8 <= 0 || W8 <= 0) return 1;
  const long long n = (long long)B * 2 * H8 * W8;
  hipLaunchKernelGGL(flow_from_coords_kernel, dim3(cdiv(n, 256)), dim3(256), 0, as_stream(stream), coords1, dst0,
                     dst0_bs, dst1, dst1_bs, stack16, B, H8, W8, is_flow);
  ACCFLOW_RETURN_LAUNCH_STATUS();
}

extern "C" int accflow_flow_from_coords_s16(const float* coords1, float* dst0, long long dst0_bs, float* dst1,
                                            long long dst1_bs, void* stack16, long long stack16_bs, void* motion16,
                                            long long motion16_bs, int motion_ch, int* guard, int is_flow, int B, int H8,
                                            int W8, void* stream) {
  if (!coords1 || (!dst0 && !dst1 && !stack16 && !motion16) || B <= 0 || H8 <= 0 || W8 <= 0 || motion_ch < 0 || (motion_ch & 1))
    return 1;
  const long long n = (long long)B * H8 * W8;
  hipLaunchKernelGGL(flow_from_coords_s16_kernel, dim3(cdiv(n, 256)), dim3(256), 0, as_stream(stream), coords1, dst0, dst0_bs,
                     dst1, dst1_bs, reinterpret_cast<mu32x4*>(stack16), stack16_bs, reinterpret_cast<unsigned*>(motion16),
                     motion16_bs, motion_ch, guard, B, H8, W8, is_flow);
  ACCFLOW_RETURN_LAUNCH_STATUS();
}

extern "C" int accflow_to_s16_f32(const float* src, long long src_bs, void* dst16, long long dst16_bs, int* guard, int B,
                                  int C, int HW, void* stream) {
  if (!src || !dst16 || B <= 0 || C <= 0 || HW <= 0) return 1;
  const long long n = (long long)B * ((C + 7) / 8) * HW;
  hipLaunchKernelGGL(to_s16_kernel, dim3(cdiv(n, 256)), dim3(256), 0, as_stream(stream), src, src_bs,
                     reinterpret_cast<mu32x4*>(dst16), dst16_bs, guard, B, C, HW);
  ACCFLOW_RETURN_LAUNCH_STATUS();
}

extern "C" int accflow_blend_f32(const float* f1, const float* f2, const float* m, float* out, int B, int C, int HW,
                                 void* stream) {
  if (!f1 || !f2 || !m || !out || B <= 0 || C <= 0 || HW <= 0) return 1;
  const long long n = (long long)B * C * HW;
  hipLaunchKernelGGL(blend_kernel, dim3(cdiv(n, 256)), dim3(256), 0, as_stream(stream), f1, f2, m, out, B, C, HW);
  ACCFLOW_RETURN_LAUNCH_STATUS();
}

extern "C" int accflow_blend_s16(const float* f1, const float* f2, const float* m, void* out16, long long out16_bs, int* guard,
                                 int B, int C, int HW, void* stream) {
  if (!f1 || !f2 || !m || !out16 || B <= 0 || C <= 0 || HW <= 0) return 1;
  const long long n = (long long)B * ((C + 7) / 8) * HW;
  hipLaunchKernelGGL(blend_s16_kernel, dim3(cdiv(n, 256)), dim3(256), 0, as_stream(stream), f1, f2, m,
                     reinterpret_cast<mu32x4*>(out16), out16_bs, guard, B, C, HW);
  ACCFLOW_RETURN_LAUNCH_STATUS();
}

extern "C" int accflow_copy_f32(const float* src, long long src_bs, float* dst, long long dst_bs, int B, int C, int HW,
                                void* stream) {
  if (!src || !dst || B <= 0 || C <= 0 || HW <= 0) return 1;
  const long long per = (long long)C * HW;
  hipLaunchKernelGGL(copy_kernel, dim3(cdiv(B * per, 256)), dim3(256), 0, as_stream(stream), src, src_bs, dst, dst_bs,
                     B, per);
  ACCFLOW_RETURN_LAUNCH_STATUS();
}

__global__ __launch_bounds__(256) void tap_sum_kernel(const float* __restrict__ z, const float* __restrict__ bias,
                                                      const float* __restrict__ e0, long long e0_bs, float* __restrict__ out,
                                                      long long out_bs, int B, int Cout, int H, int W, int KH, int KW,
                                                      int padH, int padW, int act, int epi, int nparts, long long part_stride,
                                                      long long z_bs) {
  const long long n = (long long)B * Cout * H * W;
  const long long i = (long long)blockIdx.x * 256 + threadIdx.x;
  if (i >= n) return;
  const int x = (int)(i % W), y = (int)((i / W) % H);
  const int co = (int)((i / ((long long)W * H)) % Cout), b = (int)(i / ((long long)W * H * Cout));
  const int HW = H * W;
  const float* zb = z + (long long)b * z_bs;
  float v = 0.0f;
  for (int ky = 0; ky < KH; ++ky) {
    const int yy = y + ky - padH;
// ... 47 lines not shown
```

### accflow_amd/networks/gma/gma.py

```python
import argparse
import os

import torch.nn as nn

from ... import ops
from ..raft.extractor import BasicEncoder
from ..raft.raft import RAFT
from .modules import Attention
from .update import GMAUpdateBlock

SHARE_ATTENTION = os.environ.get("ACCFLOW_GMA_SHARE_ATTENTION", "1") != "0"
ALTERNATE_ATTENTION = os.environ.get("ACCFLOW_ALTERNATE_ATTENTION", "0") == "1"


class RAFTGMA(RAFT):
    KEEP_CONTEXT_RUNS = True

    def __init__(self, args):
        nn.Module.__init__(self)
        self.args = args
        self.hidden_dim = hdim = 128
        self.context_dim = cdim = 128
        args.corr_levels = 4
        args.corr_radius = 4
        if "dropout" not in self.args:
            self.args.dropout = 0
        if "alternate_attention" not in self.args:
            self.args.alternate_attention = False
        self.fnet = BasicEncoder(output_dim=256, norm_fn="instance", dropout=args.dropout)
        self.cnet = BasicEncoder(output_dim=hdim + cdim, norm_fn="batch", dropout=args.dropout)
        self.update_block = GMAUpdateBlock(self.args, hidden_dim=hdim)
        self.att = Attention(args=self.args, dim=cdim, heads=self.args.num_heads, max_pos_size=160, dim_head=cdim)

    def _x_dim(self):
        return 384

    def _alternate_attention(self):
        return ALTERNATE_ATTENTION or bool(getattr(self.args, "alternate_attention", False))

    def _positional(self):
        return bool(getattr(self.args, "position_only", False) or getattr(self.args, "position_and_content", False))

    def _prepack(self):
        super()._prepack()
        self.att._packs.conv("qk", self.att.to_qk)

    def _prepare_context(self, ws, cnet_feat, ids=None):
        super()._prepare_context(ws, cnet_feat)
        fast = ops.current_mode() != ops.CONV_F32
        inp = ws.inp.contiguous()
        if not fast:
            ws.attention = self.att(inp)
            return
        runs = None
        if ids is not None and SHARE_ATTENTION and len(set(ids)) < len(ids):
            slot, reps, runs = {}, [], []
            for b, key in enumerate(ids):
                if key not in slot:
                    slot[key] = len(reps)
                    reps.append(b)
                if runs and runs[-1][0] == slot[key]:
                    runs[-1][2] = b + 1
                else:
                    runs.append([slot[key], b, b + 1])
            inp = inp[reps].contiguous()
        if self._alternate_attention() and ops.s16_active() and not self._positional():
            ws.attention = self.att.forward_alt(inp, runs=runs)
            return
        ws.attention = self.att.forward_t(inp, runs=runs)

    def _iteration(self, ws, corr_fn, coords1, last):
        self._lookup_and_flow(ws, corr_fn, coords1)
        return self.update_block.step(ws, coords1, want_mask=last, attention=ws.attention)


def gma_args(position_only=False, position_and_content=False):
    return argparse.Namespace(num_heads=1, mixed_precision=True, position_only=bool(position_only),
                              position_and_content=bool(position_and_content))
```

### accflow_amd/networks/raft/raft.py

```python
import argparse

import torch
import torch.nn as nn

from ... import ops
from .._packs import require_cuda
from . import corr as _corr
from .corr import AlternateCorrBlock, CorrBlock
from .extractor import BasicEncoder, SmallEncoder
from . import update as _update
from .update import BasicUpdateBlock, SmallUpdateBlock, UpdateWorkspace


import os

N_STREAMS = max(1, int(os.environ.get("ACCFLOW_STREAMS", "2")))
PROFILE_STANDALONE_LOOKUP = False
USE_CORR_PACKS = os.environ.get("ACCFLOW_CORR_PACKS", "1") == "1"
ALTERNATE_CORR = os.environ.get("ACCFLOW_ALTERNATE_CORR", "0") == "1"
_STREAMS = {}


ENCODER_STREAMS = int(os.environ.get("ACCFLOW_ENCODER_STREAMS", "2"))
GROUP_STREAM_PRIORITY = int(os.environ.get("ACCFLOW_GROUP_PRIORITY", "-1"))


def _side_streams(device, n):
    key = (str(device), n)
    if key not in _STREAMS:
        _STREAMS[key] = [torch.cuda.Stream(device=device, priority=GROUP_STREAM_PRIORITY) for _ in range(n)]
    return _STREAMS[key]


class RAFT(nn.Module):
    KEEP_CONTEXT_RUNS = False
    small = False

    def __init__(self, args):
        super().__init__()
        self.args = args
        self.small = bool(getattr(args, "small", False))
        if self.small:
            self.hidden_dim = hdim = 96
            self.context_dim = cdim = 64
            args.corr_levels = 4
            args.corr_radius = 3
        else:
            self.hidden_dim = hdim = 128
            self.context_dim = cdim = 128
            args.corr_levels = 4
            args.corr_radius = 4
        if "dropout" not in self.args:
            self.args.dropout = 0
        if "alternate_corr" not in self.args:
            self.args.alternate_corr = False
        if self.small:
            self.fnet = SmallEncoder(output_dim=128, norm_fn="instance", dropout=args.dropout)
            self.cnet = SmallEncoder(output_dim=hdim + cdim, norm_fn="none", dropout=args.dropout)
            self.update_block = SmallUpdateBlock(self.args, hidden_dim=hdim)
        else:
            self.fnet = BasicEncoder(output_dim=256, norm_fn="instance", dropout=args.dropout)
            self.cnet = BasicEncoder(output_dim=hdim + cdim, norm_fn="batch", dropout=args.dropout)
            self.update_block = BasicUpdateBlock(self.args, hidden_dim=hdim)

    def freeze_bn(self):
        for m in self.modules():
            if isinstance(m, nn.BatchNorm2d):
                m.eval()

    def initialize_flow(self, img):
        N, _, H, W = img.shape
        return (ops.coords_grid(N, H // 8, W // 8, img.device), ops.coords_grid(N, H // 8, W // 8, img.device))

    def upsample_flow(self, flow, mask):
        require_cuda(flow, mask)
        return ops.convex_upsample(flow.float(), mask.float())

    def _x_dim(self):
        return 256

    def _alternate(self):
        alt = ALTERNATE_CORR or bool(getattr(self.args, "alternate_corr", False))
        if alt and self.small:
            raise NotImplementedError("alternate_corr is built for radius 4: RAFT-small (radius 3) looks up the correlation volume")
        return alt

    def _workspace(self, B, h, w, dev):
        if self.small:
            return self.update_block.workspace(B, h, w, dev)
        return UpdateWorkspace(B, h, w, dev, hidden=self.hidden_dim, x_dim=self._x_dim())

    def _prepack(self):
        self.update_block.prepack()

    def _prepare_context(self, ws, cnet_feat, ids=None):
        if isinstance(cnet_feat, tuple):
            ops.split_tanh_relu_indexed(cnet_feat[0], cnet_feat[1], ws.net, ws.inp, self.hidden_dim, self.context_dim)
        else:
            ops.split_tanh_relu(cnet_feat, ws.net, ws.inp, self.hidden_dim, self.context_dim)
        if ws.s16:
            ops.to_s16(ws.net, ws.h16)

    def _lookup_and_flow(self, ws, corr_fn, coords1):
        if ws.s16 and corr_fn.supports_s16():
            ub = self.update_block
            if _update.FUSE_LOOKUP and ub.encoder.convc1.out_channels == 256 and isinstance(corr_fn, CorrBlock):
                if PROFILE_STANDALONE_LOOKUP and ops.profiler.ACTIVE is not None:
                    corr_fn.lookup_s16(coords1, ws.corr16)
                corr_fn.lookup_convc1(coords1, ub._packs.conv("c1f", ub.encoder.convc1, lookup_fused=True), ws.c1_16,
                                      cache=(ws.descs, "lookup"))
                ws.c1_fused = True
            else:
                corr_fn.lookup_s16(coords1, ws.corr16, cache=(ws.descs, "lookup"))
            ops.flow_from_coords_s16(coords1, ws.flow, ws.motion_flow if ws.x_dim > 256 else None, ws.stack16, ws.motion16, 126,
                                     cache=(ws.descs, "flow"))
            return
        if ws.s16:
            corr_fn(coords1, out=ws.corr)
            ws.fill_s16_inputs(coords1, is_flow=False)
            return
        corr_fn(coords1, out=ws.corr)
        ops.flow_from_coords(coords1, dst0=ws.flow, dst1=ws.motion_flow, stack16=ws.flow16)

    def _iteration(self, ws, corr_fn, coords1, last):
        self._lookup_and_flow(ws, corr_fn, coords1)
        return self.update_block.step(ws, coords1, want_mask=last)

    @classmethod
    def _group_cuts(cls, B, n_groups, flip=False, ctx_ids=None):
        flip = flip and not cls.KEEP_CONTEXT_RUNS
        cuts = [(g * B + (n_groups - 1 if flip else 0)) // n_groups for g in range(n_groups + 1)]
        if ctx_ids is not None and cls.KEEP_CONTEXT_RUNS:
            for g in range(1, n_groups):
                while cuts[g] < cuts[g + 1] - 1 and ctx_ids[cuts[g]] == ctx_ids[cuts[g] - 1]:
                    cuts[g] += 1
        return cuts

    def _refine(self, fmap1, fmap2, cnet_feat, iters, flow_init, packed=None, ctx_ids=None, ready=None, return_low=False):
        if iters < 1:
            raise ValueError("iters must be >= 1")
        indexed = isinstance(cnet_feat, tuple)
        B = len(cnet_feat[1]) if indexed else cnet_feat.shape[0]
        dev = (cnet_feat[0] if indexed else cnet_feat).device
        _, _, h, w = (cnet_feat[0] if indexed else cnet_feat).shape
        self._prepack()
        n_groups = N_STREAMS if B >= 4 else 1
        ctx_ready, flip = None, False
        if isinstance(ready, tuple):
            ready, ctx_ready, flip = ready
        cuts = self._group_cuts(B, n_groups, flip, ctx_ids)
        bounds = list(zip(cuts[:-1], cuts[1:]))
        main = torch.cuda.current_stream()
        streams = [main] if n_groups == 1 else _side_streams(dev, n_groups)
        out_all = torch.empty((B, 2, 8 * h, 8 * w), dtype=torch.float32, device=dev)
        low_all = torch.empty((B, 2, h, w), dtype=torch.float32, device=dev) if return_low else None
        forked = None
        if ctx_ready is not None:
            forked = torch.cuda.Event()
            forked.record(main)
        state = []
        early = ready is not None and packed is not None and n_groups > 1
        for (b0, b1), st in zip(bounds, streams):
            if st != main:
                if early:
                    st.wait_event(ready)
                else:
                    st.wait_stream(main)
            with torch.cuda.stream(st):
                if packed is not None and isinstance(packed[0], ops.AltPyramid):
                    corr_fn = AlternateCorrBlock.from_frames(packed[0], packed[1][b0:b1], packed[2][b0:b1])
                elif packed is not None:
                    corr_fn = CorrBlock.from_packs(packed[0], packed[1][b0:b1], packed[2][b0:b1])
                else:
                    block = AlternateCorrBlock if self._alternate() else CorrBlock
                    corr_fn = block(fmap1[b0:b1], fmap2[b0:b1], radius=self.args.corr_radius)
                if early and ctx_ready is not None:
                    st.wait_event(ctx_ready)
                elif early:
                    st.wait_stream(main)
                ws = self._workspace(b1 - b0, h, w, dev)
                self._prepare_context(ws, (cnet_feat[0], cnet_feat[1][b0:b1]) if indexed else cnet_feat[b0:b1],
                                      ctx_ids[b0:b1] if ctx_ids is not None else None)
                fi = flow_init[b0:b1] if flow_init is not None else None
                coords1 = ops.coords_grid(b1 - b0, h, w, dev, flow_init=fi)
            state.append((st, corr_fn, ws, coords1))
        masks = [None] * n_groups
        for itr in range(iters):
            for g, (st, corr_fn, ws, coords1) in enumerate(state):
                with torch.cuda.stream(st):
                    masks[g] = self._iteration(ws, corr_fn, coords1, last=(itr == iters - 1))
        for g, (st, corr_fn, ws, coords1) in enumerate(state):
            with torch.cuda.stream(st):
                if forked is not None and early:
                    st.wait_event(forked)
                ops.flow_from_coords(coords1, dst0=ws.flow)
                if masks[g] is None:
                    ops.upflow8(ws.flow, out=out_all[bounds[g][0]:bounds[g][1]])
                else:
                    ops.convex_upsample(ws.flow, masks[g], out=out_all[bounds[g][0]:bounds[g][1]])
                if return_low:
                    low_all[bounds[g][0]:bounds[g][1]].copy_(ws.flow)
            if st != main:
                main.wait_stream(st)
        return (out_all, low_all) if return_low else out_all

    @torch.no_grad()
    def forward(self, image1, image2, iters=12, flow_init=None):
        require_cuda(image1, image2)
        image1 = image1.float().contiguous()
        image2 = image2.float().contiguous()

        def run():
            fmap1, fmap2 = self.fnet([image1, image2])
            cnet_feat = self.cnet(image1)
            return self._refine_guarded(fmap1.contiguous(), fmap2.contiguous(), cnet_feat, iters, flow_init)

        out, tripped = ops.optimistic(run, image1.device)
        return run() if tripped else out

    def _refine_guarded(self, *args, **kwargs):
        dev = next(self.parameters()).device
        return ops.with_range_guard(lambda: self._refine(*args, **kwargs), dev, name="%s.refine" % type(self).__name__)

    @torch.no_grad()
    def encode_frames(self, frames, fnet_ids, cnet_ids, features=None, after_fmap=None):
        feats = features if features is not None else {}
        if feats.get("mode") != ops.current_mode():
            feats.clear()
            feats.update({"fmap": {}, "cnet": {}, "mode": ops.current_mode()})
        jobs = [(key, enc, [f for f in sorted(set(ids)) if f not in feats[key]])
                for key, enc, ids in (("fmap", self.fnet, fnet_ids), ("cnet", self.cnet, cnet_ids))]
        dev = frames[0].device
        side = None
        if (ENCODER_STREAMS in (1, 3) and N_STREAMS > 1 and all(todo for _, _, todo in jobs)
                and (ops.current_mode() != ops.CONV_F16X3 or ops.inside_guard())):
            main = torch.cuda.current_stream(dev)
            side = _side_streams(dev, N_STREAMS)[-1]
            side.wait_stream(main)
        for key, enc, todo in jobs:
            if todo:
                if side is not None and key == "cnet":
                    with torch.cuda.stream(side):
                        outs = enc([frames[f].float().contiguous() for f in todo])
                else:
                    outs = enc([frames[f].float().contiguous() for f in todo])
                base = getattr(outs[0], "_base", None)
                whole = not feats[key] and base is not None and base.shape[0] == len(todo) * outs[0].shape[0]
                feats[key + "_base"] = (base, {f: k for k, f in enumerate(todo)}) if whole else None
                if key == "fmap":
                    feats.pop("corr_packs", None)
                feats[key].update(zip(todo, outs))
            if key == "fmap" and after_fmap is not None:
                after_fmap(feats)
        if side is not None:
            main.wait_stream(side)
            base = feats.get("cnet_base")
            for t in ([base[0]] if base is not None else []) + list(feats["cnet"].values()):
                t.record_stream(main)
        return feats

    @torch.no_grad()
    def estimate_pairs(self, frames, pairs, iters=12, flow_init=None, features=None, return_low=False):
        require_cuda(*frames)
        N = frames[0].shape[0]
        feats = self.encode_pairs(frames, pairs, features)
# ... 107 lines not shown
```

### accflow_amd/networks/raft/update.py

```python
import torch
import torch.nn as nn

import os

from ... import ops
from .._packs import PackCache, require_cuda

FUSE_LOOKUP = os.environ.get("ACCFLOW_FUSE_LOOKUP", "1") == "1"
USE_H16_STATE = os.environ.get("ACCFLOW_H16_STATE", "1") == "1"


def h16_state_supported():
    return not ops.S16_VIA_MULTI and ops.conv_gru16_supported()


class FlowHead(nn.Module):
    def __init__(self, input_dim=128, hidden_dim=256):
        super().__init__()
        self.conv1 = nn.Conv2d(input_dim, hidden_dim, 3, padding=1)
        self.conv2 = nn.Conv2d(hidden_dim, 2, 3, padding=1)
        self.relu = nn.ReLU(inplace=True)


class SepConvGRU(nn.Module):
    def __init__(self, hidden_dim=128, input_dim=192 + 128):
        super().__init__()
        cin = hidden_dim + input_dim
        for suffix, ks, pad in (("1", (1, 5), (0, 2)), ("2", (5, 1), (2, 0))):
            for gate in "zrq":
                setattr(self, "conv%s%s" % (gate, suffix), nn.Conv2d(cin, hidden_dim, ks, padding=pad))
        self.hidden_dim = hidden_dim
        self.input_dim = input_dim


class BasicMotionEncoder(nn.Module):
    def __init__(self, args):
        super().__init__()
        cor_planes = args.corr_levels * (2 * args.corr_radius + 1) ** 2
        self.convc1 = nn.Conv2d(cor_planes, 256, 1, padding=0)
        self.convc2 = nn.Conv2d(256, 192, 3, padding=1)
        self.convf1 = nn.Conv2d(2, 128, 7, padding=3)
        self.convf2 = nn.Conv2d(128, 64, 3, padding=1)
        self.conv = nn.Conv2d(64 + 192, 128 - 2, 3, padding=1)


class UpdateWorkspace:

    def __init__(self, B, h, w, device, hidden=128, x_dim=256):
        def buf(c):
            return torch.empty((B, c, h, w), dtype=torch.float32, device=device)
        self.B, self.h, self.w, self.hidden, self.x_dim = B, h, w, hidden, x_dim
        self._buf = buf
        self.s16 = bool(ops.s16_active())
        self.net_in_h16 = False
        self.c1_fused = False
        self.descs = {}
        self.hx = buf(hidden + x_dim)
        self.net = self.hx[:, :hidden]
        self.inp = self.hx[:, hidden:hidden + 128]
        self.motion = self.hx[:, hidden + 128:hidden + 256]
        self.motion_conv = self.hx[:, hidden + 128:hidden + 254]
        self.motion_flow = self.hx[:, hidden + 254:hidden + 256]
        self.x = self.hx[:, hidden:]
        self.z = buf(hidden)
        self.flow = buf(2)
        self._corr = None
        if not self.s16:
            self.rh = buf(hidden)
            self.flow16 = buf(16)
            self.c1 = buf(256)
            self.corflo = buf(256)
            self.f1 = buf(128)
            self.head = buf(256)
        self.mask = None
        self.gru_pre = None
        if self.s16:
            def s(c, zero=False):
                return ops.S16.empty(B, c, h, w, device, zero=zero)
            self._corr16 = None
            self.stack16 = s(16)
            self.c1_16, self.corflo16, self.f1_16, self.head16 = s(256), s(256), s(128), s(256)
            self.h16, self.rh16 = s(hidden), s(hidden)
            self.net_in_h16 = USE_H16_STATE and h16_state_supported()
            self.x16 = s(x_dim - 128)
            self.motion16 = self.x16.channels(0, 128)


def _fill_s16_inputs(ws, flow_or_coords, is_flow):
    if not ws.s16:
        return
    B, h, w = ws.B, ws.h, ws.w
    c = ws.corr.view(B, 4, 9, 9, h, w).transpose(2, 3).reshape(B, 4, 81, h, w)
    c88 = torch.zeros((B, 4, 88, h, w), dtype=torch.float32, device=ws.corr.device)
    c88[:, :, :81] = c
    ops.to_s16(c88.view(B, 352, h, w), ws.corr16)
    ops.to_s16(ws.net, ws.h16)
    ops.flow_from_coords_s16(flow_or_coords, ws.flow, ws.motion_flow, ws.stack16, ws.motion16, 126, is_flow=is_flow)


UpdateWorkspace.fill_s16_inputs = _fill_s16_inputs


def _ws_corr(ws):
    if ws._corr is None:
        ws._corr = ws._buf(324)
    return ws._corr


UpdateWorkspace.corr = property(_ws_corr)


def _ws_corr16(ws):
    if ws._corr16 is None:
        ws._corr16 = ops.S16.empty(ws.B, ops.LOOKUP_S16_CHANNELS, ws.h, ws.w, ws.hx.device)
    return ws._corr16


UpdateWorkspace.corr16 = property(_ws_corr16)


def _ws_net32(ws):
    return ws.h16.to_float() if (ws.s16 and ws.net_in_h16) else ws.net.contiguous()


UpdateWorkspace.net32 = _ws_net32


class ConvGRU(nn.Module):

    def __init__(self, hidden_dim=128, input_dim=192 + 128):
        super().__init__()
        for gate in "zrq":
            setattr(self, "conv" + gate, nn.Conv2d(hidden_dim + input_dim, hidden_dim, 3, padding=1))
        self.hidden_dim = hidden_dim
        self.input_dim = input_dim


class SmallMotionEncoder(nn.Module):
    def __init__(self, args):
        super().__init__()
        cor_planes = args.corr_levels * (2 * args.corr_radius + 1) ** 2
        self.convc1 = nn.Conv2d(cor_planes, 96, 1, padding=0)
        self.convf1 = nn.Conv2d(2, 64, 7, padding=3)
        self.convf2 = nn.Conv2d(64, 32, 3, padding=1)
        self.conv = nn.Conv2d(128, 80, 3, padding=1)


class SmallUpdateWorkspace:
    HIDDEN, CONTEXT, MOTION, LOOKUP = 96, 64, 80, 196
    s16 = False

    def __init__(self, B, h, w, device):
        def buf(c):
            return torch.empty((B, c, h, w), dtype=torch.float32, device=device)
        hd, cd, md = self.HIDDEN, self.CONTEXT, self.MOTION
        self.B, self.h, self.w, self.hidden, self.x_dim = B, h, w, hd, cd + md + 2
        self.descs = {}
        self.hx = buf(hd + self.x_dim)
# ... 64 lines not shown
        return None

    @torch.no_grad()
    @ops.range_guarded
    def forward(self, net, inp, corr, flow):
        require_cuda(net, inp, corr, flow)
        B, _, h, w = net.shape
        ws = self.workspace(B, h, w, net.device)
        ops.copy_into(net.float(), ws.net)
        ops.copy_into(inp.float(), ws.inp)
        ops.copy_into(corr.float(), ws.corr)
        ops.flow_from_coords(flow.float().contiguous(), dst0=ws.flow, dst1=ws.motion_flow, stack16=ws.flow16, is_flow=True)
        self.motion_encoder(ws)
        self.gru_step(ws)
        delta = self.flow_delta(ws)
        return ws.net32(), None, delta


class BasicUpdateBlock(nn.Module):
    def __init__(self, args, hidden_dim=128, input_dim=128):
        super().__init__()
        self.args = args
        self.encoder = BasicMotionEncoder(args)
        self.gru = SepConvGRU(hidden_dim=hidden_dim, input_dim=128 + hidden_dim)
        self.flow_head = FlowHead(hidden_dim, hidden_dim=256)
        self.mask = nn.Sequential(nn.Conv2d(128, 256, 3, padding=1), nn.ReLU(inplace=True),
                                  nn.Conv2d(256, 64 * 9, 1, padding=0))
        self._packs = PackCache()

    def prepack(self):
        pk, e, g, f = self._packs, self.encoder, self.gru, self.flow_head
        pk.conv("c1", e.convc1); pk.conv("c2", e.convc2); pk.conv("f1s", e.convf1, rows_as_channels=True)
        if ops.s16_active():
            pk.conv("c1s", e.convc1, lookup88=True)
            if FUSE_LOOKUP:
                pk.conv("c1f", e.convc1, lookup_fused=True)
        pk.conv("f2", e.convf2)
        pk.conv("cf", e.conv)
        for s in ("1", "2"):
            self._gru_packs(s)
        pk.conv("fh1", f.conv1); pk.conv("fh2", f.conv2)
        pk.conv("m0", self.mask[0]); pk.conv("m2", self.mask[2], const_scale=0.25)

    def motion_encoder(self, ws):
        pk, e = self._packs, self.encoder
        if ws.s16:
            R, D = ops.ACT_RELU, ws.descs
            fused = ws.c1_fused
            if "c2" in D:
                for k in ("c2", "f1", "f2", "cf") if fused else ("c1", "c2", "f1", "f2", "cf"):
                    ops.conv2d(None, None, cache=(D, k))
                return
            if not fused:
                ops.conv2d(pk.conv("c1s", e.convc1, lookup88=True), ws.corr16, out16=ws.c1_16, act=R, fp32_out=False,
                           algo_cin=324, cache=(D, "c1"))
            ops.conv2d(pk.conv("c2", e.convc2), ws.c1_16, out16=ws.corflo16.channels(0, 192), act=R, fp32_out=False,
                       cache=(D, "c2"))
            ops.conv2d(pk.conv("f1s", e.convf1, rows_as_channels=True), ws.stack16, out16=ws.f1_16, act=R, fp32_out=False,
                       algo_cin=2 * 7, cache=(D, "f1"))
            ops.conv2d(pk.conv("f2", e.convf2), ws.f1_16, out16=ws.corflo16.channels(192, 256), act=R, fp32_out=False,
                       cache=(D, "f2"))
            want32 = ws.x_dim > 256
            ops.conv2d(pk.conv("cf", e.conv), ws.corflo16, out16=ws.motion16.channels(0, 126), act=R, fp32_out=want32,
                       out=ws.motion_conv if want32 else None, cache=(D, "cf"))
            return
        ops.conv2d(pk.conv("c1", e.convc1), ws.corr, out=ws.c1, act=ops.ACT_RELU)
        ops.conv2d(pk.conv("c2", e.convc2), ws.c1, out=ws.corflo[:, :192], act=ops.ACT_RELU)
        ops.conv2d(pk.conv("f1s", e.convf1, rows_as_channels=True), ws.flow16, out=ws.f1, act=ops.ACT_RELU, algo_cin=2 * 7)
        ops.conv2d(pk.conv("f2", e.convf2), ws.f1, out=ws.corflo[:, 192:], act=ops.ACT_RELU)
        ops.conv2d(pk.conv("cf", e.conv), ws.corflo, out=ws.motion_conv, act=ops.ACT_RELU)

    def _gru_packs(self, s):
        pk, g, hd = self._packs, self.gru, self.gru.hidden_dim
        cin = hd + g.input_dim
        var, ctx = [(0, hd), (hd + 128, cin)], [(hd, hd + 128)]
        zr = [getattr(g, "convz" + s), getattr(g, "convr" + s)]
        q = [getattr(g, "convq" + s)]
        return (pk.conv_cat("zr%sv" % s, zr, C0=hd, in_slices=var), pk.conv_cat("zr%sc" % s, zr, in_slices=ctx, with_bias=False),
                pk.conv_cat("q%sv" % s, q, C0=hd, in_slices=var), pk.conv_cat("q%sc" % s, q, in_slices=ctx, with_bias=False))

    def gru_context(self, ws):
        B, h, w, hd = ws.B, ws.h, ws.w, ws.hidden
        ws.gru_pre = {}
        inp = ops.to_s16(ws.inp) if ws.s16 else ws.inp
        p32 = ws.s16 and ws.net_in_h16
        for s in ("1", "2"):
            _, zrc, _, qc = self._gru_packs(s)
            ws.gru_pre["zr" + s] = ops.conv2d(zrc, inp, algo_cin=0, p32_out=p32)
            ws.gru_pre["q" + s] = ops.conv2d(qc, inp, algo_cin=0, p32_out=p32)

    def gru_step(self, ws):
        if getattr(ws, "gru_pre", None) is None:
            self.gru_context(ws)
        rest = ws.hx[:, ws.hidden + 128:]
        cin = ws.hidden + ws.x_dim
        if ws.s16:
            D = ws.descs
            if "zr1" in D:
                for k in ("zr1", "q1", "zr2", "q2"):
                    ops.conv2d(None, None, cache=(D, k))
                return
            h16s = ws.net_in_h16
            for s in ("1", "2"):
                zrv, _, qv, _ = self._gru_packs(s)
                ops.conv2d(zrv, ws.h16, in1=ws.x16, out=ws.z, act=ops.ACT_SIGMOID, epi=ops.EPI_GRU_ZR, e0=ws.h16 if h16s else ws.net,
                           out16=ws.rh16, fp32_out=False, pre=ws.gru_pre["zr" + s], algo_cin=cin, cache=(D, "zr" + s))
                ops.conv2d(qv, ws.rh16, in1=ws.x16, out=None if h16s else ws.net, act=ops.ACT_TANH, epi=ops.EPI_GRU_Q,
                           e0=ws.h16 if h16s else ws.net, e1=ws.z, out16=ws.h16, fp32_out=not h16s,
                           pre=ws.gru_pre["q" + s], algo_cin=cin, cache=(D, "q" + s))
            return
        for s in ("1", "2"):
            zrv, _, qv, _ = self._gru_packs(s)
            ops.conv2d(zrv, ws.net, in1=rest, out=ws.z, act=ops.ACT_SIGMOID, epi=ops.EPI_GRU_ZR, e0=ws.net, out2=ws.rh,
                       pre=ws.gru_pre["zr" + s], algo_cin=cin)
            ops.conv2d(qv, ws.rh, in1=rest, out=ws.net, act=ops.ACT_TANH, epi=ops.EPI_GRU_Q, e0=ws.net, e1=ws.z,
                       pre=ws.gru_pre["q" + s], algo_cin=cin)

    def flow_delta(self, ws, coords1=None, out=None):
        pk, f = self._packs, self.flow_head
        if ws.s16:
            D = ws.descs
            if coords1 is not None and ops.profiler.ACTIVE is None and "fh12" in D and D["fh12"][2] is coords1:
                return ops.conv2d_tapgemm(None, None, None, cache=(D, "fh12"))
            p1, p2 = pk.conv("fh1", f.conv1), pk.conv("fh2", f.conv2)
            if ops.tapgemm_eligible(p1, p2, ws.h16):
                if coords1 is not None:
                    return ops.conv2d_tapgemm(p1, p2, ws.h16, out=coords1, epi=ops.EPI_ACCUM, e0=coords1, cache=(D, "fh12"))
                return ops.conv2d_tapgemm(p1, p2, ws.h16, out=out)
            ops.conv2d(p1, ws.h16, out16=ws.head16, act=ops.ACT_RELU, fp32_out=False, cache=(ws.descs, "fh1"))
            if coords1 is not None:
                return ops.conv2d(pk.conv("fh2", f.conv2), ws.head16, out=coords1, epi=ops.EPI_ACCUM, e0=coords1)
            return ops.conv2d(pk.conv("fh2", f.conv2), ws.head16, out=out)
        ops.conv2d(pk.conv("fh1", f.conv1), ws.net, out=ws.head, act=ops.ACT_RELU)
        if coords1 is not None:
            return ops.conv2d(pk.conv("fh2", f.conv2), ws.head, out=coords1, epi=ops.EPI_ACCUM, e0=coords1)
        return ops.conv2d(pk.conv("fh2", f.conv2), ws.head, out=out)

    def up_mask(self, ws):
        pk = self._packs
        if ws.mask is None:
            ws.mask = torch.empty((ws.B, 576, ws.h, ws.w), dtype=torch.float32, device=ws.hx.device)
        if ws.s16:
            ops.conv2d(pk.conv("m0", self.mask[0]), ws.h16, out16=ws.head16, act=ops.ACT_RELU, fp32_out=False)
            return ops.conv2d(pk.conv("m2", self.mask[2], const_scale=0.25), ws.head16, out=ws.mask)
        ops.conv2d(pk.conv("m0", self.mask[0]), ws.net, out=ws.head, act=ops.ACT_RELU)
        return ops.conv2d(pk.conv("m2", self.mask[2], const_scale=0.25), ws.head, out=ws.mask)

    def step(self, ws, coords1, want_mask):
        self.motion_encoder(ws)
        self.gru_step(ws)
        self.flow_delta(ws, coords1=coords1)
        return self.up_mask(ws) if want_mask else None

    @torch.no_grad()
    @ops.range_guarded
    def forward(self, net, inp, corr, flow, upsample=True):
        require_cuda(net, inp, corr, flow)
        B, _, h, w = net.shape
        ws = UpdateWorkspace(B, h, w, net.device)
        ops.copy_into(net.float(), ws.net)
        ops.copy_into(inp.float(), ws.inp)
        ops.copy_into(corr.float(), ws.corr)
        ws.fill_s16_inputs(flow.float().contiguous(), is_flow=True)
        if not ws.s16:
            ops.flow_from_coords(flow.float().contiguous(), dst0=ws.flow, dst1=ws.motion_flow, stack16=ws.flow16, is_flow=True)
        self.motion_encoder(ws)
        self.gru_step(ws)
        delta = self.flow_delta(ws)
        mask = self.up_mask(ws)
        return ws.net32(), mask, delta
```

### accflow_amd/ops.py

```python
import collections
import contextlib
import ctypes
import functools
import threading

import torch

from . import _lib, profiler
from ._lib import ConvDesc

import os

ACT_NONE, ACT_RELU, ACT_SIGMOID, ACT_TANH = 0, 1, 2, 3
CONV_F32, CONV_BF16X3, CONV_BF16X6, CONV_F16X3 = 0, 2, 3, 4
_MODES = {"f32": CONV_F32, "bf16x3": CONV_BF16X3, "bf16x6": CONV_BF16X6, "f16x3": CONV_F16X3}
CONV_MODE = _MODES[os.environ.get("ACCFLOW_CONV_MODE", "f16x3").lower()]
_tls = threading.local()


USE_PATCH = os.environ.get("ACCFLOW_CONV_PATCH", "1") == "1"


def set_conv_mode(name):
    global CONV_MODE
# ... 316 lines not shown
                                                 _p(self.wpatch), _p(self.wpatch16), _p(self.wscale16), _p(self.wsplit16), _stream()),
                   "accflow_conv_pack_all_f32")
        else:
            _check(lib.accflow_conv_pack_f32(_p(w), _p(sc), self.Cout, self.Cin, self.KH, self.KW, self.C0,
                                             int(self.tap_major), _p(self.wpack), _p(self.ktab), _stream()),
                   "accflow_conv_pack_f32")
            if has_split:
                _check(lib.accflow_conv_pack_bf16s(_p(w), _p(sc), self.Cout, self.Cin, self.KH, self.KW,
                                                   _p(self.wsplit), _stream()), "accflow_conv_pack_bf16s")
            if has_patch:
                _check(lib.accflow_conv_pack_patch(_p(w), _p(sc), self.Cout, self.Cin, self.KH, self.KW,
                                                   _p(self.wpatch), _stream()), "accflow_conv_pack_patch")
                _check(lib.accflow_conv_pack_patch16(_p(w), _p(sc), self.Cout, self.Cin, self.KH, self.KW, _p(self.wpatch16),
                                                     _p(self.wscale16), _stream()), "accflow_conv_pack_patch16")
            if has_split16:
                _check(lib.accflow_conv_pack_split16(_p(w), _p(sc), self.Cout, self.Cin, self.KH, self.KW, _p(self.wsplit16),
                                                     _p(self.wscale16), _stream()), "accflow_conv_pack_split16")
        self.zcols = None
        if self.tap_major and self.stride == 1 and USE_DEFORM_COLUMNS:
            wz = w * sc.view(-1, 1, 1, 1) if sc is not None else w
            wz = wz.permute(0, 2, 3, 1).reshape(self.Cout, self.KH * self.KW * self.Cin, 1, 1).contiguous()
            self.zcols = PackedConv(wz, bias)
        self.ztaps = self.ztaps_acc = None
        if (USE_TAPSUM and not self.tap_major and self.Cout <= 4 and self.stride == 1 and self.KH * self.KW >= 2
                and self.Cin >= 16 and 2 * self.padH == self.KH - 1 and 2 * self.padW == self.KW - 1):
            wz = w * sc.view(-1, 1, 1, 1) if sc is not None else w
            wz = wz.permute(2, 3, 0, 1).reshape(self.KH * self.KW * self.Cout, self.Cin, 1, 1).contiguous()
            self.ztaps = PackedConv(wz, None, C0=self.C0)
            if self.Cin % 128 == 0 and self.KH * self.KW * self.Cout <= TAPGEMM_MAXROWS and self.C0 == self.Cin:
                self.ztaps_acc = PackedConv(wz[:, tapgemm_channel_order(self.Cin, w.device)].contiguous(), None)
        self.bias = _dense(bias.detach().float().contiguous(), "bias") if bias is not None else None

    def out_size(self, H, W):
        OH = (H + 2 * self.padH - self.KH) // self.stride + 1
        OW = (W + 2 * self.padW - self.KW) // self.stride + 1
        return OH, OW


class ConvStats:
    __slots__ = ("partial", "slots")

    def __init__(self, partial, slots):
        self.partial, self.slots = partial, slots


USE_NORM_STATS = os.environ.get("ACCFLOW_NORM_STATS", "1") == "1"
USE_NORM_ON_LOAD = os.environ.get("ACCFLOW_NORM_ON_LOAD", "1") == "1"


def _replay(cache, name):
    if cache is None or profiler.ACTIVE is not None:
        return None
    hit = cache[0].get(cache[1])
    if hit is None:
        return None
    _check(hit[0](*hit[1], _stream()), name + " (cached)")
    return hit[2]


def _launch(fn, args, name, timer=None, cache=None, ret=None, keep=None):
    tm = profiler.ACTIVE
    if tm is not None and timer is not None and tm.wants(timer[0]):
        t0 = tm.begin()
        _check(fn(*args, _stream()), name)
        tm.end(timer[0], t0, *timer[1]())
        return ret
    _check(fn(*args, _stream()), name)
    if cache is not None and tm is None:
        cache[0][cache[1]] = (fn, args, ret, keep)
    return ret


_Form = collections.namedtuple("_Form", "who s16_src via_multi patch_switch f16_always wsplit alloc_out s16_e0")
_FORM_F32 = _Form("conv2d", s16_src=False, via_multi=False, patch_switch=True, f16_always=False, wsplit=True,
                  alloc_out="always", s16_e0=None)
_FORM_S16 = _Form("conv2d", s16_src=True, via_multi=True, patch_switch=False, f16_always=True, wsplit=True,
                  alloc_out="fp32", s16_e0="gru")
_FORM_TAPGEMM = _Form("conv2d_tapgemm", s16_src=True, via_multi=False, patch_switch=False, f16_always=True, wsplit=False,
                      alloc_out="never", s16_e0=None)
_FORM_MULTI = _Form("conv2d_multi", s16_src=True, via_multi=False, patch_switch=False, f16_always=True, wsplit=False,
                    alloc_out="fp32_or_lone", s16_e0="any")


def _set_src(s, ptr, bs, C, Hs, Ws, geo):
    s.ptr, s.bs, s.C, s.Hs, s.Ws = ptr, bs, C, Hs, Ws
    s.step, s.oy, s.ox, s.KH, s.KW, s.padH, s.padW = geo


def _conv_desc(form, pk, srcs, act, epi, md, out=None, out16=None, fp32_out=True, e0=None, e1=None, out2=None, pre=None,
               p32_out=False, offset=None, dmask=None, in_norm=None, stats=False, kws_ok=False, out_hw=None, lay=None, tg=None):
    lib = _lib.load()
    who = form.who
    d = ConvDesc()
    if form is _FORM_MULTI:
        B = srcs[0].shape[0]
        OH, OW = out_hw
        d.nsrc = len(srcs)
        for k, (t, c, g) in enumerate(zip(srcs, pk.C, pk.geo)):
            if not isinstance(t, S16) or t.C != c or t.shape[0] != B:
                raise RuntimeError("conv2d_multi: source %d must be an ops.S16 of %d channels and batch %d" % (k, c, B))
            _set_src(d.src[k], t.ptr(), t.bs, c, t.shape[2], t.shape[3], g)
        if lay is not None:
            d.src[0].reserved = int(lay) + 1
        d.H, d.W = OH, OW
        d.KH = d.KW = d.stride = 1
        d.split_c0 = pk.split_c0
        d.wpatch16, d.wscale16 = pk.wpatch16.data_ptr(), pk.wscale16.data_ptr()
    else:
        in0, in1 = srcs
        fmt, S = 0, []
        for k, t in enumerate(srcs):
            if t is None:
                S.append((None, 0, 0))
            elif form.s16_src and isinstance(t, S16):
                fmt |= 1 << k
                S.append((t.ptr(), t.bs, t.C))
            else:
                bs = _plane4(t, "in%d" % k)
                S.append((t.data_ptr(), bs, t.shape[1]))
        if fmt and fmt != (3 if in1 is not None else 1):
            raise RuntimeError("%s: both sources must have the same format" % who)
        B, _, H, W = in0.shape
        if in1 is not None and (in1.shape[0] != B or tuple(in1.shape[2:]) != (H, W)):
            raise RuntimeError("%s: in0/in1 shape mismatch" % who)
        C0, C1 = S[0][2], S[1][2]
        if C0 != pk.C0 or C0 + C1 != pk.Cin:
            raise RuntimeError("%s: channel split (%d,%d) does not match packed weights (C0=%d, Cin=%d)"
                               % (who, C0, C1, pk.C0, pk.Cin))
        OH, OW = pk.out_size(H, W)
        (d.in0, d.in0_bs, _), (d.in1, d.in1_bs, _) = S
        d.in_fmt = fmt
        if form.via_multi and S16_VIA_MULTI and fmt:
            d.nsrc = 2 if in1 is not None else 1
            for k in range(d.nsrc):
                _set_src(d.src[k], S[k][0], S[k][1], S[k][2], H, W, (1, 0, 0, pk.KH, pk.KW, pk.padH, pk.padW))
        d.C0, d.C1, d.H, d.W = C0, C1, H, W
        d.KH, d.KW, d.stride, d.padH, d.padW = pk.KH, pk.KW, pk.stride, pk.padH, pk.padW
        d.wpack, d.ktab, d.Kpad = pk.wpack.data_ptr(), pk.ktab.data_ptr(), pk.Kpad
        if form.wsplit and pk.wsplit is not None:
            d.wsplit = pk.wsplit.data_ptr()
        if pk.wpatch is not None and (USE_PATCH or not form.patch_switch):
            d.wpatch = pk.wpatch.data_ptr()
        if form.f16_always or (md == CONV_F16X3 and pk.wscale16 is not None):
            if d.wpatch and pk.wpatch16 is not None:
                d.wpatch16 = pk.wpatch16.data_ptr()
            if form.wsplit and pk.wsplit16 is not None:
                d.wsplit16 = pk.wsplit16.data_ptr()
            d.wscale16 = pk.wscale16.data_ptr()
    dev = srcs[0].device
    if d.wscale16:
        d.guard = _guard(dev).data_ptr()
    d.B, d.OH, d.OW, d.Cout, d.CoutPad = B, OH, OW, pk.Cout, pk.CoutPad
    d.bias = pk.bias.data_ptr() if pk.bias is not None else None
    d.act, d.epi, d.mode = act, epi, md
    n_out = pk.Cout // 2 if epi == EPI_GRU_ZR else pk.Cout
    if out is None and form.alloc_out != "never" and (form.alloc_out == "always" or fp32_out or epi == EPI_GRU_ZR
                                                      or (form.alloc_out == "fp32_or_lone" and out16 is None)):
        out = torch.empty((B, n_out, OH, OW), dtype=torch.float32, device=dev)
    if out is not None:
        d.out_bs = _plane4(out, "out")
        if tuple(out.shape) != (B, n_out, OH, OW):
            raise RuntimeError("%s: out shape %s != %s" % (who, tuple(out.shape), (B, n_out, OH, OW)))
        d.out = out.data_ptr()
    if out16 is not None:
        if tuple(out16.shape) != (B, n_out, OH, OW):
            raise RuntimeError("%s: out16 shape %s != %s" % (who, out16.shape, (B, n_out, OH, OW)))
        d.out16, d.out16_bs = out16.ptr(), out16.bs
    ws = None
    if kws_ok and _ksplit_on() and B * OH * OW <= KSPLIT_MAX_PIXELS and pk.Cout > 4:
        ws = _ksplit_ws(4 * B * pk.Cout * OH * OW, dev)
        d.kws, d.kws_elems = ws.data_ptr(), ws.numel()
    if form.s16_e0 == "gru" and isinstance(e0, S16):
        if epi not in (EPI_GRU_ZR, EPI_GRU_Q) or tuple(e0.shape) != (B, n_out, OH, OW):
            raise RuntimeError("conv2d: an S16 e0 is the GRU epilogues' state operand, shape (B, hidden, OH, OW)")
        d.e0_bs, d.e0, d.e0_fmt = e0.bs, e0.ptr(), 1
        d.p32 = 3 if epi == EPI_GRU_ZR else 6
    elif form.s16_e0 == "any" and isinstance(e0, S16):
        if tuple(e0.shape) != (B, pk.Cout, OH, OW):
            raise RuntimeError("conv2d_multi: S16 e0 shape %s != %s" % (e0.shape, (B, pk.Cout, OH, OW)))
        d.e0_bs, d.e0, d.e0_fmt = e0.bs, e0.ptr(), 1
        d.kws, d.kws_elems = None, 0
    elif e0 is not None:
        d.e0_bs, d.e0 = _plane4(e0, "e0"), e0.data_ptr()
    if e1 is not None:
        d.e1_bs, d.e1 = _plane4(e1, "e1"), e1.data_ptr()
    if out2 is not None:
        d.out2_bs, d.out2 = _plane4(out2, "out2"), out2.data_ptr()
    if pre is not None:
        if epi not in (EPI_GRU_ZR, EPI_GRU_Q) or tuple(pre.shape) != (B, pk.Cout, OH, OW):
            raise RuntimeError("%s: `pre` is a (B, Cout, OH, OW) addend of the GRU epilogues" % who)
        d.pre_bs, d.pre = _plane4(pre, "pre"), pre.data_ptr()
    if p32_out:
        if epi != EPI_STORE or out is None or pk.Cout % 128 or isinstance(e0, S16):
            raise RuntimeError("conv2d: p32_out is a plain fp32 store onto a multiple of 128 channels")
        d.p32 = 1
    if offset is not None:
        d.offset_bs, d.offset = _plane4(offset, "offset"), offset.data_ptr()
        d.dmask_bs, d.dmask = _plane4(dmask, "dmask"), dmask.data_ptr()
        if not pk.tap_major:
            raise RuntimeError("deformable conv needs tap-major packed weights")
    if tg is not None:
        pz, z = tg
        rows = pz.Cout
        d.tg_w16, d.tg_scale, d.tg_out = pz.wpatch16.data_ptr(), pz.wscale16.data_ptr(), z.data_ptr()
        d.tg_out_bs, d.tg_out_ps, d.tg_rows, d.tg_coutpad = rows * OH * OW, B * rows * OH * OW, rows, pz.CoutPad
    if in_norm is not None:
        if srcs[1] is not None or tuple(_dense(in_norm, "in_norm").shape) != (B, d.C0, 2):
            raise RuntimeError("conv2d: in_norm is (B, C0, 2) for a single-source input")
        if not lib.accflow_conv_in_norm_supported(ctypes.byref(d)):
            return None
        d.in_norm = in_norm.data_ptr()
    st = None
    if stats:
        slots = lib.accflow_conv_stat_slots(ctypes.byref(d))
        if slots > 0:
            st = ConvStats(torch.empty((B, pk.Cout, slots, 3), dtype=torch.float32, device=dev), slots)
            d.stats, d.stat_slots = st.partial.data_ptr(), slots
    ret = out if (out is not None and (fp32_out or out16 is None)) else out16
    return d, ret, st, (d, pk, srcs, out, out16, e0, e1, out2, pre, ws, offset, dmask, in_norm, tg)


def _conv_figures(pk, d, tag, algo_cin):
    B, OH, OW = d.B, d.OH, d.OW
    acin = pk.Cin if algo_cin is None else algo_cin
    return (2.0 * acin * pk.KH * pk.KW * pk.Cout * B * OH * OW,
            "Cin%d Cout%d k%dx%d s%d B%d %dx%d%s%s" % (pk.Cin, pk.Cout, pk.KH, pk.KW, pk.stride, B, OH, OW, tag,
                                                      "" if algo_cin is None else " (stands for Cin%d)" % algo_cin),
            2.0 * pk.Cin * pk.KH * pk.KW * pk.Cout * B * OH * OW)


def conv2d(pk, in0, in1=None, out=None, act=ACT_NONE, epi=EPI_STORE, e0=None, e1=None, out2=None,
           offset=None, dmask=None, mode=None, want_stats=False, pre=None, algo_cin=None, in_norm=None, out16=None,
           fp32_out=True, cache=None, p32_out=False):
    r = _replay(cache, "accflow_conv2d_f32")
    if r is not None:
        return r
    if pk is None:
        raise RuntimeError("conv2d: no packed weights given and no cached descriptor for %r to replay"
                           % (cache[1] if cache is not None else None,))
    md = current_mode() if mode is None else mode
    if isinstance(in0, S16) and pk.Cout <= 4 and out16 is None and (pk.ztaps is None or (md == CONV_F16X3 and not TAPSUM_F16)):
        in0 = in0.to_float()
        in1 = in1.to_float() if isinstance(in1, S16) else in1
    if (out16 is not None or isinstance(in0, S16)) and not (pk.ztaps is not None and out16 is None):
        if want_stats or offset is not None or in_norm is not None:
            raise RuntimeError("conv2d: S16 tensors are for plain direct-kernel convolutions")
        if md != CONV_F16X3 or (pk.wpatch16 is None and pk.wsplit16 is None):
            raise RuntimeError("conv2d: S16 tensors need the f16x3 mode and a direct-kernel weight pack")
        d, ret, _, keep = _conv_desc(_FORM_S16, pk, (in0, in1), act, epi, md, out, out16, fp32_out, e0, e1, out2, pre, p32_out,
                                     kws_ok=not isinstance(e0, S16) and not p32_out)
        return _launch(_lib.load().accflow_conv2d_f32, (ctypes.byref(d),), "accflow_conv2d_f32 (S16)",
                       ("conv2d", lambda: _conv_figures(pk, d, " S16in" if d.in_fmt else " S16", algo_cin)), cache, ret, keep)
    if p32_out or isinstance(e0, S16):
        raise RuntimeError("conv2d: pixel-major / pre-split operands belong to the S16 direct-kernel form")
    if want_stats:
        if act != ACT_NONE or epi != EPI_STORE or offset is not None:
            raise RuntimeError("conv2d: statistics are gathered for plain convolutions only (store, no activation)")
        pre = algo_cin = None
    r = _conv2d(pk, in0, in1, out, act, epi, e0, e1, out2, offset, dmask, md, want_stats, pre, algo_cin, in_norm)
    if r is None:
        return None
    return r if want_stats else r[0]


def _conv2d(pk, in0, in1, out, act, epi, e0, e1, out2, offset, dmask, md, want_stats, pre, algo_cin, in_norm):
    lib = _lib.load()
    if (pk.ztaps is not None and md != CONV_F32 and offset is None and epi in (EPI_STORE, EPI_ACCUM, EPI_RES_RELU)
            and (isinstance(in0, S16) or in0.shape[0] * in0.shape[2] * in0.shape[3] >= TAPSUM_MIN_PIXELS)):
        z = conv2d(pk.ztaps, in0, in1, mode=CONV_BF16X6 if (md == CONV_F16X3 and not TAPSUM_F16) else md)
        B, _, H, W = in0.shape
        if out is None:
            out = torch.empty((B, pk.Cout, H, W), dtype=torch.float32, device=in0.device)
        out_bs = _plane4(out, "out")
        e0_bs = _plane4(e0, "e0") if e0 is not None else 0
        args = (_p(z), _p(pk.bias) if pk.bias is not None else None, _p(e0) if e0 is not None else None, e0_bs, _p(out), out_bs,
                B, pk.Cout, H, W, pk.KH, pk.KW, pk.padH, pk.padW, int(act), int(epi))
        _launch(lib.accflow_tap_sum_f32, args, "accflow_tap_sum_f32",
                ("conv2d", lambda: (0.0, "tap_sum Cout%d k%dx%d B%d %dx%d" % (pk.Cout, pk.KH, pk.KW, B, H, W))))
        return out, None
    if offset is not None and pk.zcols is not None and md != CONV_F32 and in1 is None:
        cols = _deform_columns(pk, in0, offset, dmask)
        return conv2d(pk.zcols, cols, out=out, act=act, epi=epi, e0=e0, e1=e1, out2=out2, mode=md), None
    b = _conv_desc(_FORM_F32, pk, (in0, in1), act, epi, md, out, e0=e0, e1=e1, out2=out2, pre=pre, offset=offset, dmask=dmask,
                   in_norm=in_norm, stats=want_stats and USE_NORM_STATS, kws_ok=pk.wpatch is not None and USE_PATCH)
    if b is None:
        return None
    d, ret, st, _ = b
    _launch(lib.accflow_conv2d_f32, (ctypes.byref(d),), "accflow_conv2d_f32",
            ("conv2d", lambda: _conv_figures(pk, d, " deform" if offset is not None else "", algo_cin)))
    return ret, st


def _deform_columns(pk, x, offset, dmask, name="in0"):
    B, C, H, W = x.shape
    cols = torch.empty((B, pk.KH * pk.KW * C, H, W), dtype=torch.float32, device=x.device)
    args = (_p(x), _plane4(x, name), _p(offset), _plane4(offset, "offset"), _p(dmask), _plane4(dmask, "dmask"), _p(cols),
            B, C, H, W, pk.KH, pk.KW, pk.padH, pk.padW)
    _launch(_lib.load().accflow_deform_columns_f32, args, "accflow_deform_columns_f32",
            ("conv2d", lambda: (0.0, "deform_columns C%d k%dx%d B%d %dx%d" % (C, pk.KH, pk.KW, B, H, W))))
    return cols



def tapgemm_eligible(pk1, pk2, in0, in1=None):
    if not (FUSE_TAPGEMM and current_mode() == CONV_F16X3 and isinstance(in0, S16) and (in1 is None or isinstance(in1, S16))):
        return False
    B, _, H, W = in0.shape
    nb = B * ((W + 31) // 32) * ((H + 3) // 4) * (pk1.Cout // 128)
    return (pk1.wpatch16 is not None and pk1.Cout % 128 == 0 and pk1.stride == 1 and pk2.ztaps_acc is not None
            and pk2.Cin == pk1.Cout and pk1.out_size(H, W) == (H, W) and not (_ksplit_on() and nb < 320))


def conv2d_tapgemm(pk1, pk2, in0, in1=None, out=None, epi=EPI_STORE, e0=None, cache=None):
    cache2 = (cache[0], (cache[1], "tap_sum")) if cache is not None else None
    if _replay(cache, "accflow_conv2d_f32 (tapgemm)") is not None:
        return _replay(cache2, "accflow_tap_sum_parts_f32")
    if pk1 is None:
        raise RuntimeError("conv2d_tapgemm: no packed weights given and no cached descriptor for %r to replay"
                           % (cache[1] if cache is not None else None,))
    if not tapgemm_eligible(pk1, pk2, in0, in1):
        raise RuntimeError("conv2d_tapgemm: shapes / mode outside the fused form (ops.tapgemm_eligible)")
    if epi not in (EPI_STORE, EPI_ACCUM, EPI_RES_RELU) or (epi != EPI_STORE and e0 is None):
        raise RuntimeError("conv2d_tapgemm: epi is STORE, ACCUM (+ e0) or RES_RELU (+ e0)")
    lib = _lib.load()
    B, _, H, W = in0.shape
    dev = in0.device
    pz = pk2.ztaps_acc
    rows, nparts = pz.Cout, pk1.Cout // 128
    z = torch.empty((nparts, B, rows, H, W), dtype=torch.float32, device=dev)
    if out is None:
        out = torch.empty((B, pk2.Cout, H, W), dtype=torch.float32, device=dev)
    d, _, _, keep = _conv_desc(_FORM_TAPGEMM, pk1, (in0, in1), ACT_RELU, EPI_TAPGEMM, CONV_F16X3, tg=(pz, z), kws_ok=False)
    out_bs = _plane4(out, "out")
    e0_bs = _plane4(e0, "e0") if e0 is not None else 0
    targs = (z.data_ptr(), nparts, B * rows * H * W, rows * H * W, _p(pk2.bias) if pk2.bias is not None else None,
             _p(e0) if e0 is not None else None, e0_bs, _p(out), out_bs, B, pk2.Cout, H, W, pk2.KH, pk2.KW, pk2.padH, pk2.padW,
             int(ACT_NONE), int(epi))
    _launch(lib.accflow_conv2d_f32, (ctypes.byref(d),), "accflow_conv2d_f32 (tapgemm)",
            ("conv2d", lambda: (2.0 * (pk1.Cin * pk1.KH * pk1.KW * pk1.Cout + pk1.Cout * rows) * (B * H * W),
                                "Cin%d Cout%d k%dx%d s1 B%d %dx%d S16in +tapgemm%d" % (pk1.Cin, pk1.Cout, pk1.KH, pk1.KW, B, H, W, rows))),
            cache, out, keep)
    return _launch(lib.accflow_tap_sum_parts_f32, targs, "accflow_tap_sum_parts_f32",
                   ("conv2d", lambda: (0.0, "tap_sum Cout%d k%dx%d B%d %dx%d (%d parts)" % (pk2.Cout, pk2.KH, pk2.KW, B, H, W, nparts))),
                   cache2, out, (pk2, out, e0, z))


class PackedMulti:
    __slots__ = ("wpatch16", "wscale16", "bias", "Cout", "CoutPad", "C", "geo", "out_hw", "flop_per_px", "split_c0")

    def __init__(self, weights, bias, geo, scale=None, split_c0=0):
        lib = _lib.load()
        n = len(weights)
        if not 1 <= n <= _lib.MAX_SRC or len(geo) != n:
            raise RuntimeError("PackedMulti: 1..%d sources" % _lib.MAX_SRC)
        ws = [_dense(w.detach().float().contiguous(), "weight") for w in weights]
        self.Cout = ws[0].shape[0]
        self.C = [w.shape[1] for w in ws]
        self.geo = [tuple(int(v) for v in g) for g in geo]
        for w, g in zip(ws, self.geo):
            if w.shape[0] != self.Cout or tuple(w.shape[2:]) != (g[3], g[4]):
                raise RuntimeError("PackedMulti: weight %s does not match its source geometry %s" % (tuple(w.shape), g))
        self.CoutPad = lib.accflow_conv_coutpad(self.Cout)
        arr = lambda v: (ctypes.c_int * n)(*v)
        C, KH, KW = arr(self.C), arr([g[3] for g in self.geo]), arr([g[4] for g in self.geo])
        dev = ws[0].device
        self.wpatch16 = torch.empty(lib.accflow_conv_multi_pack_elems(self.Cout, n, C, KH, KW), dtype=torch.int16, device=dev)
        self.wscale16 = torch.empty(self.CoutPad, dtype=torch.float32, device=dev)
# ... 660 lines not shown
        nbytes = 4 * src.numel()
        if (tuple(_dense(out, "out").shape) != shape or out.device != flow.device
                or (out.data_ptr() < src.data_ptr() + nbytes and src.data_ptr() < out.data_ptr() + nbytes)):
            raise RuntimeError("forward_interpolate: out must be a float32 tensor of shape %s on %s that does not overlap flow" % (
                shape, flow.device))
    _check(lib.accflow_forward_interpolate_f32(_p(src), _p(out), B, h, w, _stream()), "accflow_forward_interpolate_f32")
    return out


def instance_stats_finalize(stats, eps=1e-5, c0=0, C=None):
    lib = _lib.load()
    B, Ctot = stats.partial.shape[:2]
    C = Ctot - c0 if C is None else C
    mr = torch.empty((B, C, 2), dtype=torch.float32, device=stats.partial.device)
    _check(lib.accflow_instance_stats_finalize_sub_f32(_p(stats.partial), stats.slots, Ctot, int(c0), _p(mr), B, C, float(eps),
                                                       _stream()), "accflow_instance_stats_finalize_sub_f32")
    return mr


def instance_norm_proj(x, stats, proj, proj_stats, proj_c0, out16, eps=1e-5):
    lib = _lib.load()
    x = _dense(x, "x")
    B, C, H, W = x.shape
    pbs = _plane4(proj, "proj")
    if (tuple(proj.shape) != (B, C, H, W) or tuple(out16.shape) != (B, C, H, W) or tuple(stats.partial.shape[:2]) != (B, C)
            or proj_stats.partial.shape[0] != B or proj_c0 + C > proj_stats.partial.shape[1]):
        raise RuntimeError("instance_norm_proj: shape mismatch")
    mr = torch.empty(4 * B * C, dtype=torch.float32, device=x.device)
    _check(lib.accflow_instance_norm_apply_s16proj_f32(_p(x), _p(stats.partial), stats.slots, _p(proj), pbs, _p(proj_stats.partial),
                                                       proj_stats.slots, proj_stats.partial.shape[1], int(proj_c0), _p(mr),
                                                       ctypes.c_void_p(out16.ptr()), out16.bs, _p(_guard(x.device)), B, C, H * W,
                                                       float(eps), _stream()), "accflow_instance_norm_apply_s16proj_f32")
    return out16


def instance_norm(x, mode, res=None, eps=1e-5, out=None, stats=None, out16=None, fp32_out=True):
    lib = _lib.load()
    x = _dense(x, "x")
    B, C, H, W = x.shape
    if out16 is not None:
        if stats is None or tuple(stats.partial.shape[:2]) != (B, C) or tuple(out16.shape) != (B, C, H, W):
            raise RuntimeError("instance_norm: out16 needs the producing convolution's statistics and a matching S16 tensor")
        o32 = (x if out is None else _dense(out, "out")) if fp32_out else None
        mr = torch.empty(2 * B * C, dtype=torch.float32, device=x.device)
        if isinstance(res, S16):
            if mode != 2 or tuple(res.shape) != (B, C, H, W):
                raise RuntimeError("instance_norm: an S16 residual belongs to mode 2 and must match x")
            _check(lib.accflow_instance_norm_apply_s16res_f32(_p(x), _p(stats.partial), stats.slots, _p(mr),
                                                              ctypes.c_void_p(res.ptr()), res.bs, _p(o32),
                                                              ctypes.c_void_p(out16.ptr()), out16.bs, _p(_guard(x.device)), B, C,
                                                              H * W, float(eps), _stream()), "accflow_instance_norm_apply_s16res_f32")
            return o32 if fp32_out else out16
        if res is not None:
            _dense(res, "res")
        _check(lib.accflow_instance_norm_apply_s16_f32(_p(x), _p(stats.partial), stats.slots, _p(mr), _p(res), _p(o32),
                                                       ctypes.c_void_p(out16.ptr()), out16.bs, _p(_guard(x.device)), B, C, H * W,
                                                       float(eps), int(mode), _stream()), "accflow_instance_norm_apply_s16_f32")
        return o32 if fp32_out else out16
    if out is None:
        out = x
    if res is not None:
        _dense(res, "res")
    if stats is not None:
        if tuple(stats.partial.shape[:2]) != (B, C):
            raise RuntimeError("instance_norm: statistics do not belong to this tensor")
        mr = torch.empty(2 * B * C, dtype=torch.float32, device=x.device)
        _check(lib.accflow_instance_norm_apply_f32(_p(x), _p(stats.partial), stats.slots, _p(mr), _p(res), _p(out), B, C, H * W,
                                                   float(eps), int(mode), _stream()), "accflow_instance_norm_apply_f32")
        return out
    _check(lib.accflow_instance_norm_f32(_p(x), _p(res), _p(out), B, C, H * W, float(eps), int(mode), _stream()),
           "accflow_instance_norm_f32")
    return out


def split_tanh_relu(cnet, net, inp, hd, cd):
    lib = _lib.load()
    cnet = _dense(cnet, "cnet")
    B, _, H, W = cnet.shape
    nbs, ibs = _plane4(net, "net"), _plane4(inp, "inp")
    _check(lib.accflow_split_tanh_relu_f32(_p(cnet), _p(net), nbs, _p(inp), ibs, B, hd, cd, H * W, _stream()),
           "accflow_split_tanh_relu_f32")


def split_tanh_relu_indexed(cnet_items, idx, net, inp, hd, cd):
    lib = _lib.load()
    cnet_items = _dense(cnet_items, "cnet")
    n, _, H, W = cnet_items.shape
    B = len(idx)
    nbs, ibs = _plane4(net, "net"), _plane4(inp, "inp")
    if net.shape[0] != B or inp.shape[0] != B:
        raise RuntimeError("split_tanh_relu_indexed: one index per output item")
    arr = (ctypes.c_int * B)(*idx)
    _check(lib.accflow_split_tanh_relu_idx_f32(_p(cnet_items), n, arr, _p(net), nbs, _p(inp), ibs, B, hd, cd, H * W, _stream()),
           "accflow_split_tanh_relu_idx_f32")


def coords_grid(B, H8, W8, device, flow_init=None):
    lib = _lib.load()
    out = torch.empty((B, 2, H8, W8), dtype=torch.float32, device=device)
    if flow_init is not None:
        flow_init = _dense(flow_init.float().contiguous(), "flow_init")
    _check(lib.accflow_coords_grid_f32(_p(out), _p(flow_init), B, H8, W8, _stream()), "accflow_coords_grid_f32")
    return out


def flow_from_coords(coords1, dst0=None, dst1=None, stack16=None, is_flow=False):
    lib = _lib.load()
    coords1 = _dense(coords1, "coords1")
    B, _, H8, W8 = coords1.shape
    b0 = _plane4(dst0, "dst0") if dst0 is not None else 0
    b1 = _plane4(dst1, "dst1") if dst1 is not None else 0
    if stack16 is not None and tuple(_dense(stack16, "stack16").shape) != (B, 16, H8, W8):
        raise RuntimeError("flow_from_coords: stack16 must be (B, 16, h, w)")
    _check(lib.accflow_flow_from_coords_f32(_p(coords1), _p(dst0), b0, _p(dst1), b1, _p(stack16), int(bool(is_flow)), B, H8, W8,
                                            _stream()),
           "accflow_flow_from_coords_f32")


def blend(f1, f2, m, out16=None):
    lib = _lib.load()
    f1, f2, m = _dense(f1, "f1"), _dense(f2, "f2"), _dense(m, "m")
    B, C, H, W = f1.shape
    if out16 is not None:
        if tuple(out16.shape) != (B, C, H, W):
            raise RuntimeError("blend: out16 shape %s" % (out16.shape,))
        _check(lib.accflow_blend_s16(_p(f1), _p(f2), _p(m), ctypes.c_void_p(out16.ptr()), out16.bs, _p(_guard(f1.device)), B, C,
                                     H * W, _stream()), "accflow_blend_s16")
        return out16
    out = torch.empty_like(f1)
    _check(lib.accflow_blend_f32(_p(f1), _p(f2), _p(m), _p(out), B, C, H * W, _stream()), "accflow_blend_f32")
    return out


def activation_(x, act):
    lib = _lib.load()
    xbs = _plane4(x, "x")
    B, C, H, W = x.shape
    _check(lib.accflow_activation_f32(_p(x), xbs, B, C, H * W, int(act), _stream()), "accflow_activation_f32")
    return x


def copy_into(src, dst):
    lib = _lib.load()
    sbs, dbs = _plane4(src, "src"), _plane4(dst, "dst")
    if src.shape != dst.shape:
        raise RuntimeError("copy_into: shape mismatch")
    B, C, H, W = src.shape
    _check(lib.accflow_copy_f32(_p(src), sbs, _p(dst), dbs, B, C, H * W, _stream()), "accflow_copy_f32")
    return dst


def gma_attention(qk, D, scale):
    lib = _lib.load()
    qk = _dense(qk, "qk")
    B, _, H, W = qk.shape
    P = H * W
    attn = torch.empty((B, 1, P, P), dtype=torch.float32, device=qk.device)
    _check(lib.accflow_gma_attention_f32(_p(qk), _p(attn), B, D, P, float(scale), _stream()),
           "accflow_gma_attention_f32")
    return attn


def gma_aggregate(attn, v, fmap, gamma, out=None):
    lib = _lib.load()
    attn, v, fmap = _dense(attn, "attn"), _dense(v, "v"), _dense(fmap, "fmap")
    gamma = _dense(gamma.detach().float().contiguous(), "gamma")
    B, D, H, W = fmap.shape
    if out is None:
        out = torch.empty_like(fmap)
    obs = _plane4(out, "out")
    _check(lib.accflow_gma_aggregate_f32(_p(attn), _p(v), _p(fmap), _p(gamma), _p(out), obs, B, D, H * W, _stream()),
           "accflow_gma_aggregate_f32")
    return out


# ... 158 lines not shown
```

### include/accflow_hip.h

```cpp
#ifndef ACCFLOW_HIP_H
#define ACCFLOW_HIP_H

#ifdef __cplusplus
extern "C" {
#endif

#define ACCFLOW_ABI_VERSION 20

enum { ACCFLOW_ACT_NONE = 0, ACCFLOW_ACT_RELU = 1, ACCFLOW_ACT_SIGMOID = 2, ACCFLOW_ACT_TANH = 3 };

enum {
  ACCFLOW_EPI_STORE = 0,
  ACCFLOW_EPI_RES_RELU = 1,
  ACCFLOW_EPI_GRU_ZR = 2,
  ACCFLOW_EPI_GRU_Q = 3,
  ACCFLOW_EPI_ACCUM = 4,
  ACCFLOW_EPI_TAPGEMM = 5
};

enum {
  ACCFLOW_CONV_F32 = 0,
  ACCFLOW_CONV_BF16X3 = 2,
  ACCFLOW_CONV_BF16X6 = 3,
  ACCFLOW_CONV_F16X3 = 4
};
#define ACCFLOW_F16_ASHIFT 4

typedef struct accflow_conv_src {
  const void* ptr;
  long long bs;
  int C, Hs, Ws;
  int step, oy, ox;
  int KH, KW, padH, padW;
  int reserved;
} accflow_conv_src;
#define ACCFLOW_CONV_MAX_SRC 4

typedef struct accflow_conv_desc {
  const float* in0;  const float* in1;
  long long in0_bs, in1_bs;
  int C0, C1;
  int B, H, W;
  int OH, OW;
  int KH, KW, stride, padH, padW;
  int Cout;
  const float* wpack;
  const int*   ktab;
  int Kpad, CoutPad;
  const float* bias;
  float* out;  long long out_bs;
  int act, epi;
  const float* e0; long long e0_bs;
  const float* e1; long long e1_bs;
  float* out2; long long out2_bs;
  const float* offset; long long offset_bs;
  const float* dmask;  long long dmask_bs;
  const void* wsplit;
  int mode;
  const void* wpatch;
  long long wsplit_bs;
  float* kws; long long kws_elems;
  const void* wpatch16; int* guard;
  const float* wscale16;
  const void* wsplit16;
  float* stats; int stat_slots;
  const float* pre; long long pre_bs;
  const float* in_norm;
  float acc_scale;
  int in_fmt;
  void* out16; long long out16_bs;
  int cb;
  long long out_cbs, e0_cbs, out16_cbs;
  int nsrc;
  accflow_conv_src src[ACCFLOW_CONV_MAX_SRC];
  int e0_fmt;
  const void* tg_w16; const float* tg_scale;
  float* tg_out; long long tg_out_bs, tg_out_ps;
  int tg_rows, tg_coutpad;
  int split_c0;
  int p32;
} accflow_conv_desc;

long long accflow_s16_item_words(int C, int H, int W);
int accflow_to_s16_f32(const float* src, long long src_bs, void* dst16, long long dst16_bs, int* guard, int B, int C,
                       int HW, void* stream);

int accflow_conv_kpad(int Cin, int KH, int KW);
int accflow_conv_coutpad(int Cout);

int accflow_conv_pack_f32(const float* w, const float* scale, int Cout, int Cin, int KH, int KW,
                          int C0, int tap_major, float* wpack, int* ktab, void* stream);

int accflow_conv_pack_bf16s(const float* w, const float* scale, int Cout, int Cin, int KH, int KW,
                            void* wsplit, void* stream);

long long accflow_conv_patch_elems(int Cout, int Cin, int KH, int KW);
int accflow_conv_pack_patch(const float* w, const float* scale, int Cout, int Cin, int KH, int KW,
                            void* wpatch, void* stream);
int accflow_conv_pack_patch16(const float* w, const float* scale, int Cout, int Cin, int KH, int KW,
                              void* wpatch16, float* wscale16, void* stream);

int accflow_conv_pack_split16(const float* w, const float* scale, int Cout, int Cin, int KH, int KW,
                              void* wsplit16, float* wscale16, void* stream);

int accflow_conv_pack_all_f32(const float* w, const float* scale, int Cout, int Cin, int KH, int KW, int C0, int tap_major,
                              int transpose_flip, float* wpack, int* ktab, void* wsplit, void* wpatch, void* wpatch16,
                              float* wscale16, void* wsplit16, void* stream);

long long accflow_conv_multi_pack_elems(int Cout, int nsrc, const int* C, const int* KH, const int* KW);
int accflow_conv_pack_multi16(const float* const* w, const float* scale, int Cout, int nsrc, const int* C, const int* KH,
                              const int* KW, void* wpatch16, float* wscale16, void* stream);

int accflow_conv2d_f32(const accflow_conv_desc* desc, void* stream);
int accflow_conv_stat_slots(const accflow_conv_desc* desc);
int accflow_conv_in_norm_supported(const accflow_conv_desc* desc);
int accflow_conv_plan_query(const accflow_conv_desc* desc, int* out, int n);
int accflow_conv_gru16_supported(void);

int accflow_corr_volume_f32(const float* fmap1, const float* fmap2, float* lvl0, float* lvl1,
                            float* lvl2, float* lvl3, int B, int C, int H8, int W8, void* stream);

long long accflow_corr_volume_ws_bytes(int C, int H8, int W8);
int accflow_corr_volume_split_f32(const float* fmap1, const float* fmap2, float* lvl0, float* lvl1,
                                  float* lvl2, float* lvl3, void* ws, int mode, int B, int C, int H8,
                                  int W8, void* stream);

int accflow_corr_lookup_f32(const float* lvl0, const float* lvl1, const float* lvl2,
                            const float* lvl3, const float* coords, float* out, long long out_bs,
                            int B, int H8, int W8, void* stream);
int accflow_corr_lookup_r3_f32(const float* lvl0, const float* lvl1, const float* lvl2,
                               const float* lvl3, const float* coords, float* out, long long out_bs,
                               int B, int H8, int W8, void* stream);

int accflow_corr_disp_supported(int H8, int W8);
long long accflow_corr_disp_level_elems(int H8, int W8, int level);
int accflow_corr_volume_disp_f32(const float* fmap1, const float* fmap2, float* lvl0, float* lvl1,
                                 float* lvl2, float* lvl3, void* ws, int mode, int* guard, int B, int C,
                                 int H8, int W8, void* stream);
long long accflow_corr_pack_bytes(int C, int H8, int W8);
int accflow_corr_pack_f32(const float* fmaps, void* packs, int mode, int* guard, int F, int C, int H8, int W8,
                          void* stream);
int accflow_corr_volume_disp_packed_f32(const void* packs, int F, const int* idx1, const int* idx2, float* lvl0,
                                        float* lvl1, float* lvl2, float* lvl3, int mode, int* guard, int B, int C, int H8,
                                        int W8, void* stream);
int accflow_corr_disp_pool_f32(const float* lvl0, float* lvl1, float* lvl2, float* lvl3, int B, int H8,
                               int W8, void* stream);
int accflow_corr_lookup_disp_f32(const float* lvl0, const float* lvl1, const float* lvl2,
                                 const float* lvl3, const float* coords, float* out, long long out_bs,
                                 int B, int H8, int W8, void* stream);

int accflow_corr_lookup_disp_s16(const float* lvl0, const float* lvl1, const float* lvl2, const float* lvl3,
                                 const float* coords, void* out16, long long out16_bs, int* guard, int B, int H8,
                                 int W8, void* stream);

long long accflow_corr_alt_pyramid_elems(int C, int H8, int W8);
int accflow_corr_alt_pyramid_f32(const float* fmaps, float* pyr, int F, int C, int H8, int W8, void* stream);
int accflow_corr_lookup_alt_f32(const float* pyr, int F, const int* idx, const float* coords, float* out, long long out_bs,
                                int B, int C, int H8, int W8, void* stream);
int accflow_corr_lookup_alt_s16(const float* pyr, int F, const int* idx, const float* coords, void* out16, long long out16_bs,
                                int* guard, int B, int C, int H8, int W8, void* stream);

int accflow_corr_lookup_convc1_kpad(void);
int accflow_corr_lookup_convc1_s16(const float* lvl0, const float* lvl1, const float* lvl2, const float* lvl3,
                                   const float* coords, const void* wpatch16, const float* wscale16, const float* bias,
                                   void* out16, long long out16_bs, float* out, long long out_bs, int act, int* guard,
                                   int B, int H8, int W8, int Cout, void* stream);

int accflow_convex_upsample_f32(const float* flow, long long flow_bs, const float* mask,
                                long long mask_bs, float* out, int B, int H8, int W8, void* stream);

int accflow_backwarp_f32(const float* img, long long img_bs, const float* flow, long long flow_bs,
                         float* out, long long out_bs, int B, int C, int H, int W, void* stream);

int accflow_compose_flow_f32(const float* step, long long step_bs, const float* acc, long long acc_bs,
                             float* out, long long out_bs, int B, int H, int W, void* stream);

int accflow_get_occ_f32(const float* flow, long long flow_bs, const float* i1, long long i1_bs,
                        const float* i2, long long i2_bs, float* out, long long out_bs, int B, int C,
                        int H, int W, int binary, void* stream);

int accflow_get_occ_s16(const float* flow, long long flow_bs, const float* i1, long long i1_bs, const float* i2,
                        long long i2_bs, void* out16, long long out16_bs, int* guard, int B, int C, int H, int W, int binary,
                        void* stream);

int accflow_downflow8_f32(const float* flow, float* out, int B, int C, int H, int W, void* stream);
int accflow_upflow8_f32(const float* flow, long long flow_bs, float* out, long long out_bs, int B, int h, int w, void* stream);
int accflow_forward_interpolate_f32(const float* flow, float* out, int B, int H8, int W8, void* stream);

int accflow_fb_occlusion_f32(const float* bflow, long long b_bs, const float* fflow, long long f_bs, float* occ_bw,
                             long long obw_bs, float* occ_fw, long long ofw_bs, float alpha, float beta, int B, int H, int W,
                             void* stream);

long long accflow_flow_metrics_ws_bytes(int B, int H, int W);
int accflow_flow_metrics_f32(const float* pred, long long p_bs, const float* gt, long long g_bs, const float* mask,
                             long long m_bs, const float* fflow, long long f_bs, int mode, float alpha, float beta,
                             double* sums, float* ws, int B, int H, int W, void* stream);

int accflow_instance_norm_f32(const float* x, const float* res, float* out, int B, int C, int HW,
                              float eps, int mode, void* stream);

int accflow_instance_stats_finalize_f32(const float* stats, int slots, float* meanrstd, int B, int C, float eps,
                                        void* stream);
int accflow_instance_norm_apply_f32(const float* x, const float* stats, int slots, float* meanrstd, const float* res,
                                    float* out, int B, int C, int HW, float eps, int mode, void* stream);
int accflow_instance_stats_finalize_sub_f32(const float* stats, int slots, int Ctot, int c0, float* meanrstd, int B, int C,
                                            float eps, void* stream);

int accflow_instance_norm_apply_s16_f32(const float* x, const float* stats, int slots, float* meanrstd, const float* res,
                                        float* out, void* out16, long long out16_bs, int* guard, int B, int C, int HW,
                                        float eps, int mode, void* stream);
int accflow_instance_norm_apply_s16res_f32(const float* x, const float* stats, int slots, float* meanrstd, const void* res16,
                                           long long res16_bs, float* out, void* out16, long long out16_bs, int* guard, int B,
                                           int C, int HW, float eps, void* stream);

int accflow_instance_norm_apply_s16proj_f32(const float* x, const float* stats, int slots, const float* res, long long res_bs,
                                            const float* res_stats, int res_slots, int res_ctot, int res_c0, float* meanrstd,
                                            void* out16, long long out16_bs, int* guard, int B, int C, int HW, float eps,
                                            void* stream);

int accflow_split_tanh_relu_f32(const float* cnet, float* net, long long net_bs, float* inp,
                                long long inp_bs, int B, int hd, int cd, int HW, void* stream);
int accflow_split_tanh_relu_idx_f32(const float* cnet, int n_items, const int* idx, float* net, long long net_bs, float* inp,
                                    long long inp_bs, int B, int hd, int cd, int HW, void* stream);

int accflow_coords_grid_f32(float* coords, const float* flow_init, int B, int H8, int W8,
                            void* stream);

int accflow_flow_from_coords_f32(const float* coords1, float* dst0, long long dst0_bs, float* dst1,
                                 long long dst1_bs, float* stack16, int is_flow, int B, int H8, int W8, void* stream);
int accflow_flow_from_coords_s16(const float* coords1, float* dst0, long long dst0_bs, float* dst1, long long dst1_bs,
                                 void* stack16, long long stack16_bs, void* motion16, long long motion16_bs, int motion_ch,
                                 int* guard, int is_flow, int B, int H8, int W8, void* stream);

int accflow_blend_f32(const float* f1, const float* f2, const float* m, float* out, int B, int C,
                      int HW, void* stream);

int accflow_blend_s16(const float* f1, const float* f2, const float* m, void* out16, long long out16_bs, int* guard, int B, int C,
                      int HW, void* stream);

int accflow_deform_columns_f32(const float* x, long long x_bs, const float* offset, long long offset_bs,
                               const float* dmask, long long dmask_bs, float* cols, int B, int C, int H, int W,
                               int KH, int KW, int padH, int padW, void* stream);

int accflow_deform_columns_s16(const float* x, long long x_bs, const float* offset, long long offset_bs, const float* dmask,
                               long long dmask_bs, int mask_is_logit, void* cols16, long long cols16_bs, int* guard, int B, int C,
                               int H, int W, int KH, int KW, int padH, int padW, void* stream);

int accflow_tap_sum_f32(const float* z, const float* bias, const float* e0, long long e0_bs, float* out,
                        long long out_bs, int B, int Cout, int H, int W, int KH, int KW, int padH, int padW,
                        int act, int epi, void* stream);
int accflow_tap_sum_parts_f32(const float* z, int nparts, long long part_stride, long long z_bs, const float* bias,
                              const float* e0, long long e0_bs, float* out, long long out_bs, int B, int Cout, int H, int W,
                              int KH, int KW, int padH, int padW, int act, int epi, void* stream);

int accflow_activation_f32(float* x, long long x_bs, int B, int C, int HW, int act, void* stream);

int accflow_copy_f32(const float* src, long long src_bs, float* dst, long long dst_bs, int B, int C,
                     int HW, void* stream);

int accflow_gma_attention_f32(const float* qk, float* attn, int B, int D, int P, float scale,
                              void* stream);
int accflow_gma_aggregate_f32(const float* attn, const float* v, const float* fmap,
                              const float* gamma, float* out, long long out_bs, int B, int D, int P,
                              void* stream);

long long accflow_gma_attention_ws_bytes(int D, int H, int W);
long long accflow_gma_attention_s16_ws_bytes(int D, int H, int W);
int accflow_gma_attention_s16(const float* qk, void* attn16, void* ws, int* guard, int B, int D, int H, int W, float scale,
                              void* stream);
long long accflow_gma_aggregate_s16_ws_bytes(int n, int D, int P);
int accflow_gma_aggregate_s16(const void* attn16, const float* v, const float* fmap, long long fmap_bs, const float* gamma,
                              float* out, long long out_bs, void* out16, long long out16_bs, void* ws, int* guard, int n, int D,
                              int H, int W, void* stream);
long long accflow_gma_attention_alt_ws_bytes(int D, int H, int W);
int accflow_gma_attention_alt(const float* qk, void* kpack, void* qpack, float* stats, void* ws, int* guard, int B, int D, int H,
                              int W, float scale, void* stream);
long long accflow_gma_aggregate_alt_ws_bytes(int n, int D, int P);
int accflow_gma_aggregate_alt(const void* kpack, const void* qpack, const float* stats, const float* v, const float* fmap,
                              long long fmap_bs, const float* gamma, float* out, long long out_bs, void* out16, long long out16_bs,
                              void* ws, int* guard, int n, int D, int H, int W, void* stream);
int accflow_gma_attention_t_f32(const float* qk, float* attnT, void* ws, int mode, int B, int D, int H, int W,
                                float scale, void* stream);
long long accflow_gma_aggregate_ws_bytes(int B, int D, int P);
int accflow_gma_aggregate_t_f32(const float* attnT, const float* v, const float* fmap, const float* gamma,
                                float* out, long long out_bs, void* ws, int mode, int* guard, int B, int D, int H, int W,
                                void* stream);
int accflow_gma_pos_tables_f32(const float* qk, const float* rel_height, const float* rel_width, float* tab, int B, int D,
                               int H, int W, int max_pos, float scale, void* stream);
int accflow_gma_attention_pos_f32(const float* qk, const float* tab, float* attn, int content, int B, int D, int H, int W,
                                  float scale, void* stream);
long long accflow_gma_attention_pos_ws_bytes(int D, int H, int W, int content, int s16);
int accflow_gma_attention_pos_t(const float* qk, const float* tab, float* attnT, void* attn16, void* ws, int mode, int content,
                                int B, int D, int H, int W, float scale, void* stream);

int accflow_act_backward_f32(const float* dy, long long dy_bs, const float* y, long long y_bs, float* dx, long long dx_bs, int B,
                             long long CHW, int act, void* stream);
int accflow_add_f32(float* dst, long long dst_bs, const float* src, long long src_bs, int B, long long CHW, void* stream);
int accflow_l1_grad_f32(const float* pred, const float* gt, float* dpred, long long n, float scale, void* stream);
int accflow_dilate_f32(const float* src, long long src_bs, float* dst, int B, int C, int OH, int OW, int Hd, int Wd, int stride,
                       void* stream);
int accflow_blend_backward_f32(const float* dy, const float* f1, const float* f2, const float* m, float* df1, float* df2,
                               float* dm, int B, int C, int HW, void* stream);
int accflow_convex_upsample_backward_f32(const float* dup, const float* flow, const float* mask, float* dflow, float* dmask,
                                         int B, int H8, int W8, void* stream);
int accflow_conv_wgrad_f32(const float* x, long long x_bs, const float* dy, long long dy_bs, float* dw, float* db, int B, int Cin,
                           int Cout, int H, int W, int KH, int KW, int stride, int padH, int padW, void* stream);
// ... 13 lines not shown
```

Baseline: 535.2.

## Share per-frame context rows across batch items via pre_map indirection

Batch items that come from the same context frame now share one row of the context features. Only the unique rows are written by split_tanh_relu, and a pre_map index table lets the GRU conv epilogues read the precomputed context addend from the shared row. This cuts the work of the per-item context projection (gru_pre) and the attention input when the context ids repeat. It adds an indirection load in the epilogues and more complex buffer-range handling, plus an ABI struct change.

After: 529.4. 0.989x the previous value.

```diff
diff --git a/accflow_amd/_lib.py b/accflow_amd/_lib.py
--- a/accflow_amd/_lib.py
+++ b/accflow_amd/_lib.py
@@ -49,7 +49,8 @@
         ("kws", c_f), ("kws_elems", c_ll),
         ("wpatch16", c_f), ("guard", c_f),
         ("wscale16", c_f), ("wsplit16", c_f), 
-        ("stats", c_f), ("stat_slots", c_i), ("pre", c_f), ("pre_bs", c_ll), ("in_norm", c_f), ("acc_scale", ctypes.c_float),
+        ("stats", c_f), ("stat_slots", c_i), ("pre", c_f), ("pre_bs", c_ll), ("pre_map", c_f), ("pre_rows", c_i),
+        ("in_norm", c_f), ("acc_scale", ctypes.c_float),
         ("in_fmt", c_i), ("out16", c_f), ("out16_bs", c_ll),
         ("cb", c_i), ("out_cbs", c_ll), ("e0_cbs", c_ll), ("out16_cbs", c_ll),
         ("nsrc", c_i), ("src", ConvSrc * MAX_SRC),
@@ -128,6 +129,8 @@
     "accflow_instance_norm_f32": [c_f, c_f, c_f, c_i, c_i, c_i, ctypes.c_float, c_i, c_f],
     "accflow_split_tanh_relu_f32": [c_f, c_f, c_ll, c_f, c_ll, c_i, c_i, c_i, c_i, c_f],
     "accflow_split_tanh_relu_idx_f32": [c_f, c_i, ctypes.POINTER(c_i), c_f, c_ll, c_f, c_ll, c_i, c_i, c_i, c_i, c_f],
+    "accflow_split_tanh_relu_rows_f32": [c_f, c_i, ctypes.POINTER(c_i), ctypes.POINTER(c_i), c_f, c_ll, c_f, c_ll, c_i, c_i, c_i, c_i,
+                                         c_i, c_f],
     "accflow_coords_grid_f32": [c_f, c_f, c_i, c_i, c_i, c_f],
     "accflow_flow_from_coords_f32": [c_f, c_f, c_ll, c_f, c_ll, c_f, c_i, c_i, c_i, c_i, c_f],
     "accflow_deform_columns_f32": [c_f, c_ll, c_f, c_ll, c_f, c_ll, c_f, c_i, c_i, c_i, c_i, c_i, c_i, c_i, c_i, c_f],
diff --git a/accflow_amd/csrc/conv2d_direct.hip b/accflow_amd/csrc/conv2d_direct.hip
--- a/accflow_amd/csrc/conv2d_direct.hip
+++ b/accflow_amd/csrc/conv2d_direct.hip
@@ -13,7 +13,10 @@
   float v = d.kws[i];
   for (int z = 1; z < Z; ++z) v += d.kws[(long long)z * n + i];
   v = fmaf(v, d.wscale16 ? d.wscale16[(d.wsplit_bs ? (long long)b * d.CoutPad : 0) + ch] : 1.0f, d.bias ? d.bias[ch] : 0.0f);
-  if (d.pre && (d.epi == ACCFLOW_EPI_GRU_ZR || d.epi == ACCFLOW_EPI_GRU_Q)) v += d.pre[b * d.pre_bs + (long long)ch * OHW + px];
+  if (d.pre && (d.epi == ACCFLOW_EPI_GRU_ZR || d.epi == ACCFLOW_EPI_GRU_Q)) {
+    const int prow = conv_pre_row(d, b);
+    if (prow >= 0) v += d.pre[prow * d.pre_bs + (long long)ch * OHW + px];
+  }
   v = apply_act(v, d.act);
   const long long o = (long long)ch * OHW + px;
   const int half = d.Cout >> 1;
@@ -63,7 +66,10 @@
     float v = d.kws[e];
     for (int z = 1; z < Z; ++z) v += d.kws[(long long)z * n + e];
     v = fmaf(v, d.wscale16 ? d.wscale16[(d.wsplit_bs ? (long long)b * d.CoutPad : 0) + ch] : 1.0f, d.bias ? d.bias[ch] : 0.0f);
-    if (d.pre && (zr || d.epi == ACCFLOW_EPI_GRU_Q)) v += d.pre[b * d.pre_bs + (long long)ch * OHW + px];
+    if (d.pre && (zr || d.epi == ACCFLOW_EPI_GRU_Q)) {
+      const int prow = conv_pre_row(d, b);
+      if (prow >= 0) v += d.pre[prow * d.pre_bs + (long long)ch * OHW + px];
+    }
     v = apply_act(v, d.act);
     const long long o = (long long)ch * OHW + px;
     float r = v;
@@ -150,7 +156,10 @@
   for (int j = 0; j < 4; ++j) {
     const int ch = q * 4 + j;
     float t = fmaf(v[j], d.wscale16 ? d.wscale16[(d.wsplit_bs ? (long long)b * d.CoutPad : 0) + ch] : 1.0f, d.bias ? d.bias[ch] : 0.0f);
-    if (d.pre && d.epi == ACCFLOW_EPI_GRU_Q) t += d.pre[b * d.pre_bs + (long long)ch * OHW + px];
+    if (d.pre && d.epi == ACCFLOW_EPI_GRU_Q) {
+      const int prow = conv_pre_row(d, b);
+      if (prow >= 0) t += d.pre[prow * d.pre_bs + (long long)ch * OHW + px];
+    }
     t = apply_act(t, d.act);
     const long long o = (long long)ch * OHW + px;
     if (d.cb) {
diff --git a/accflow_amd/csrc/conv_common.h b/accflow_amd/csrc/conv_common.h
--- a/accflow_amd/csrc/conv_common.h
+++ b/accflow_amd/csrc/conv_common.h
@@ -67,6 +67,13 @@
 }
 
 __device__ __forceinline__ float gru_blend(float z, float h, float q) { return __builtin_fmaf(z, q, (1.0f - z) * h); }
+
+__device__ __forceinline__ int conv_pre_rows(const accflow_conv_desc& d) { return d.pre_map ? d.pre_rows : d.B; }
+__device__ __forceinline__ int conv_pre_row(const accflow_conv_desc& d, int b) {
+  if (!d.pre_map) return b;
+  const int r = d.pre_map[b];
+  return (unsigned)r < (unsigned)d.pre_rows ? r : -1;
+}
 
 template <int EPI, int ACT, int WC, int WP, int TC, int TP, class PixMap, bool OUT16 = false>
 __device__ __forceinline__ void conv_epilogue_impl(const accflow_conv_desc& d, f32x16 (&acc)[TC][TP], int cblk0, int wc,
@@ -106,7 +113,8 @@
       const_cast<float*>(has_z ? d.e1 : d.out), 0, has_z ? span(d.e1_bs, d.Cout) : 0, 0x00020000);
   const bool has_pre = (EPI == ACCFLOW_EPI_GRU_ZR || EPI == ACCFLOW_EPI_GRU_Q) && d.pre != nullptr;
   const __amdgpu_buffer_rsrc_t r_pre = __builtin_amdgcn_make_buffer_rsrc(
-      const_cast<float*>(has_pre ? d.pre : d.out), 0, has_pre ? span(d.pre_bs, d.Cout) : 0, 0x00020000);
+      const_cast<float*>(has_pre ? d.pre : d.out), 0,
+      has_pre ? (int)(unsigned)((((long long)(conv_pre_rows(d) - 1)) * d.pre_bs + (long long)d.Cout * OHW) * 4) : 0, 0x00020000);
 
   unsigned vo_out[TP], vo_o2[TP], vo_e0[TP], vo_e1[TP], vo_pre[TP], vo_16[TP];
 #pragma unroll
@@ -120,7 +128,8 @@
     vo_o2[tp] = ok && zr ? (unsigned)((b * d.out2_bs + lp) * 4) : MASKED;
     vo_e0[tp] = ok && has_h ? (unsigned)((b * d.e0_bs + lp) * 4) : MASKED;
     vo_e1[tp] = ok && has_z ? (unsigned)((b * d.e1_bs + lp) * 4) : MASKED;
-    vo_pre[tp] = ok && has_pre ? (unsigned)((b * d.pre_bs + lp) * 4) : MASKED;
+    const int prow = ok && has_pre ? conv_pre_row(d, b) : -1;
+    vo_pre[tp] = prow >= 0 ? (unsigned)((prow * d.pre_bs + lp) * 4) : MASKED;
   }
   const int rowbase = cblk0 + wc * TC * 32;
   const int OHW4 = OHW * 4;
@@ -401,7 +410,14 @@
   const int nst = ZR ? half : d.Cout;
   const int cst = ZR ? rowbase - half : rowbase;
   auto rng = [&](long long bs, int nch) { return (int)(unsigned)((((long long)(d.B - 1)) * bs + (long long)nch * OHW) * 4); };
-  const __amdgpu_buffer_rsrc_t r_pre = __builtin_amdgcn_make_buffer_rsrc(const_cast<float*>(d.pre), 0, rng(d.pre_bs, d.Cout), 0x00020000);
+  int tile_b;
+  (void)pixmap(0, tile_b);
+  tile_b = __builtin_amdgcn_readfirstlane(tile_b);
+  typedef const __attribute__((address_space(4))) int* cint_ptr;
+  const int prow = d.pre_map ? ((cint_ptr)(unsigned long long)d.pre_map)[tile_b] : tile_b;
+  const bool prow_ok = (unsigned)prow < (unsigned)conv_pre_rows(d);
+  const __amdgpu_buffer_rsrc_t r_pre = __builtin_amdgcn_make_buffer_rsrc(
+      const_cast<float*>(d.pre) + (prow_ok ? prow * d.pre_bs : 0), 0, prow_ok ? d.Cout * OHW * 4 : 0, 0x00020000);
   const __amdgpu_buffer_rsrc_t r_z = __builtin_amdgcn_make_buffer_rsrc(ZR ? (float*)d.out : const_cast<float*>(d.e1), 0,
                                                                       ZR ? rng(d.out_bs, half) : rng(d.e1_bs, d.Cout), 0x00020000);
   const int s16rng = (int)(unsigned)((((long long)(d.B - 1)) * d.e0_bs + (long long)((nst + 7) >> 3) * 2 * OHW * 4) * 4);
@@ -421,7 +437,7 @@
       int b;
       const int rem = pixmap((hh * TPH + t) * 32 + l31, b);
       const bool ok = rem >= 0;
-      vo_p[t] = ok ? (unsigned)((b * d.pre_bs + (long long)rem * 8 + lh4) * 4) : MASKED;
+      vo_p[t] = ok ? (unsigned)((rem * 8 + lh4) * 4) : MASKED;
       vo_z[t] = ok ? (unsigned)((b * (ZR ? d.out_bs : d.e1_bs) + (long long)rem * 8 + lh4) * 4) : MASKED;
       vo_h[t] = ok ? (unsigned)((b * d.e0_bs + (long long)rem * 4) * 4 + lh4 * 2) : MASKED;
       vo_o[t] = ok ? (unsigned)((b * d.out16_bs + (long long)rem * 4) * 4 + lh4 * 2) : MASKED;
diff --git a/accflow_amd/csrc/conv_plan.cpp b/accflow_amd/csrc/conv_plan.cpp
--- a/accflow_amd/csrc/conv_plan.cpp
+++ b/accflow_amd/csrc/conv_plan.cpp
@@ -272,7 +272,7 @@
   if ((!multi && (!d.in0 || !d.wpack || !d.ktab)) || d.B <= 0 || d.Cout <= 0 || d.OH <= 0 || d.OW <= 0) return 1;
   if (d.epi == ACCFLOW_EPI_TAPGEMM) {
     if (multi || d.mode != ACCFLOW_CONV_F16X3 || !d.wpatch16 || !d.wscale16 || d.in_fmt != (d.in1 ? 3 : 1) || d.act != ACCFLOW_ACT_RELU ||
-        (d.Cout & 127) || d.kws || d.stats || d.in_norm || d.cb || d.pre || d.offset || !d.tg_w16 || !d.tg_scale || !d.tg_out ||
+        (d.Cout & 127) || d.kws || d.stats || d.in_norm || d.cb || d.pre || d.pre_map || d.offset || !d.tg_w16 || !d.tg_scale || !d.tg_out ||
         d.tg_rows < 1 || d.tg_rows > ACCFLOW_TAPGEMM_MAXROWS || d.tg_coutpad < 32 || (d.tg_coutpad & 31) ||
         d.tg_out_bs < (long long)d.tg_rows * d.OH * d.OW || (d.Cout > 128 && d.tg_out_ps <= 0) || !accflow_conv_direct_eligible(d) ||
         d.Kpad != accflow_conv_kpad(d.C0 + d.C1, d.KH, d.KW) || d.CoutPad != accflow_conv_coutpad(d.Cout))
@@ -301,6 +301,8 @@
   if (d.epi == ACCFLOW_EPI_GRU_ZR && d.out16 && ((d.Cout >> 1) & 7)) return 1;
   if (d.epi == ACCFLOW_EPI_GRU_Q && (!d.e0 || !d.e1)) return 1;
   if (d.pre && d.epi != ACCFLOW_EPI_GRU_ZR && d.epi != ACCFLOW_EPI_GRU_Q) return 1;
+  if (d.pre_map && (!d.pre || d.pre_rows < 1)) return 1;
+  if (d.pre_map && (((long long)(d.pre_rows - 1)) * d.pre_bs + (long long)d.Cout * d.OH * d.OW) * 4 >= (1LL << 32)) return 1;
   if (d.offset && !d.dmask) return 1;
   if ((long long)d.B * d.OH * d.OW >= (1LL << 31)) return 1;
   if (!multi) {
diff --git a/accflow_amd/csrc/misc.hip b/accflow_amd/csrc/misc.hip
--- a/accflow_amd/csrc/misc.hip
+++ b/accflow_amd/csrc/misc.hip
@@ -166,7 +166,7 @@
 }
 
 struct split_idx { int v[64]; };
-__global__ void split_tanh_relu_idx_kernel(const float* __restrict__ cnet, split_idx idx, float* __restrict__ net,
+__global__ void split_tanh_relu_idx_kernel(const float* __restrict__ cnet, split_idx idx, split_idx row, float* __restrict__ net,
                                            long long net_bs, float* __restrict__ inp, long long inp_bs, int B, int hd, int cd,
                                            int HW) {
   const long long per = (long long)(hd + cd) * HW;
@@ -175,9 +175,10 @@
   const int b = (int)(g / per);
   const long long r = g - b * per;
   const int c = (int)(r / HW), pix = (int)(r - (long long)c * HW);
+  if (c >= hd && row.v[b] < 0) return;
   const float v = cnet[(long long)idx.v[b] * per + r];
   if (c < hd) net[b * net_bs + (long long)c * HW + pix] = tanhf(v);
-  else inp[b * inp_bs + (long long)(c - hd) * HW + pix] = fmaxf(v, 0.0f);
+  else inp[row.v[b] * inp_bs + (long long)(c - hd) * HW + pix] = fmaxf(v, 0.0f);
 }
 
 __global__ void coords_grid_kernel(float* __restrict__ coords, const float* __restrict__ flow_init, int B, int H8,
@@ -530,20 +531,37 @@
   ACCFLOW_RETURN_LAUNCH_STATUS();
 }
 
+static int split_tanh_relu_rows(const float* cnet, int n_items, const int* idx, const int* inp_row, float* net, long long net_bs,
+                                float* inp, long long inp_bs, int inp_rows, int B, int hd, int cd, int HW, void* stream) {
+  if (!cnet || !idx || !net || !inp || n_items <= 0 || B <= 0 || hd <= 0 || cd <= 0 || HW <= 0) return 1;
+  for (int b = 0; b < B; ++b) {
+    if (idx[b] < 0 || idx[b] >= n_items) return 1;
+    if (inp_row && (inp_row[b] < -1 || inp_row[b] >= inp_rows)) return 1;
+  }
+  for (int b0 = 0; b0 < B; b0 += 64) {
+    const int nb = B - b0 < 64 ? B - b0 : 64;
+    split_idx a, r;
+    for (int k = 0; k < 64; ++k) {
+      a.v[k] = k < nb ? idx[b0 + k] : 0;
+      r.v[k] = k < nb ? (inp_row ? inp_row[b0 + k] : b0 + k) : -1;
+    }
+    const long long n = (long long)nb * (hd + cd) * HW;
+    hipLaunchKernelGGL(split_tanh_relu_idx_kernel, dim3(cdiv(n, 256)), dim3(256), 0, as_stream(stream), cnet, a, r,
+                       net + b0 * net_bs, net_bs, inp, inp_bs, nb, hd, cd, HW);
+  }
+  ACCFLOW_RETURN_LAUNCH_STATUS();
+}
+
 extern "C" int accflow_split_tanh_relu_idx_f32(const float* cnet, int n_items, const int* idx, float* net, long long net_bs,
                                                float* inp, long long inp_bs, int B, int hd, int cd, int HW, void* stream) {
-  if (!cnet || !idx || !net || !inp || n_items <= 0 || B <= 0 || hd <= 0 || cd <= 0 || HW <= 0) return 1;
-  for (int b = 0; b < B; ++b)
-    if (idx[b] < 0 || idx[b] >= n_items) return 1;
-  for (int b0 = 0; b0 < B; b0 += 64) {
-    const int nb = B - b0 < 64 ? B - b0 : 64;
-    split_idx a;
-    for (int k = 0; k < 64; ++k) a.v[k] = k < nb ? idx[b0 + k] : 0;
-    const long long n = (long long)nb * (hd + cd) * HW;
-    hipLaunchKernelGGL(split_tanh_relu_idx_kernel, dim3(cdiv(n, 256)), dim3(256), 0, as_stream(stream), cnet, a,
-                       net + b0 * net_bs, net_bs, inp + b0 * inp_bs, inp_bs, nb, hd, cd, HW);
-  }
-  ACCFLOW_RETURN_LAUNCH_STATUS();
+  return split_tanh_relu_rows(cnet, n_items, idx, nullptr, net, net_bs, inp, inp_bs, B, B, hd, cd, HW, stream);
+}
+
+extern "C" int accflow_split_tanh_relu_rows_f32(const float* cnet, int n_items, const int* idx, const int* inp_row, float* net,
+                                                long long net_bs, float* inp, long long inp_bs, int inp_rows, int B, int hd,
+                                                int cd, int HW, void* stream) {
+  if (!inp_row || inp_rows <= 0) return 1;
+  return split_tanh_relu_rows(cnet, n_items, idx, inp_row, net, net_bs, inp, inp_bs, inp_rows, B, hd, cd, HW, stream);
 }
 
 extern "C" int accflow_coords_grid_f32(float* coords, const float* flow_init, int B, int H8, int W8, void* stream) {
diff --git a/accflow_amd/networks/gma/gma.py b/accflow_amd/networks/gma/gma.py
--- a/accflow_amd/networks/gma/gma.py
+++ b/accflow_amd/networks/gma/gma.py
@@ -45,10 +45,14 @@
         super()._prepack()
         self.att._packs.conv("qk", self.att.to_qk)
 
-    def _prepare_context(self, ws, cnet_feat, ids=None):
-        super()._prepare_context(ws, cnet_feat)
+    def _prepare_context(self, ws, cnet_feat, ids=None, share=False):
+        super()._prepare_context(ws, cnet_feat, ids, share)
         fast = ops.current_mode() != ops.CONV_F32
-        inp = ws.inp.contiguous()
+        shared = ws.ctx_map is not None
+        inp = ws.inp[:max(ws.ctx_map) + 1].contiguous() if shared else ws.inp.contiguous()
+        if shared and not (fast and SHARE_ATTENTION):
+            inp = inp[ws.ctx_map].contiguous()
+            shared = False
         if not fast:
             ws.attention = self.att(inp)
             return
@@ -63,7 +67,8 @@
                     runs[-1][2] = b + 1
                 else:
                     runs.append([slot[key], b, b + 1])
-            inp = inp[reps].contiguous()
+            if not shared:
+                inp = inp[reps].contiguous()
         if self._alternate_attention() and ops.s16_active() and not self._positional():
             ws.attention = self.att.forward_alt(inp, runs=runs)
             return
diff --git a/accflow_amd/networks/raft/raft.py b/accflow_amd/networks/raft/raft.py
--- a/accflow_amd/networks/raft/raft.py
+++ b/accflow_amd/networks/raft/raft.py
@@ -93,8 +93,15 @@
     def _prepack(self):
         self.update_block.prepack()
 
-    def _prepare_context(self, ws, cnet_feat, ids=None):
-        if isinstance(cnet_feat, tuple):
+    def _prepare_context(self, ws, cnet_feat, ids=None, share=False):
+        rows = _update.context_rows(ids) if share and not self.small else None
+        if rows is not None:
+            reps, ws.ctx_map = rows
+            src, idx = cnet_feat if isinstance(cnet_feat, tuple) else (cnet_feat, list(range(cnet_feat.shape[0])))
+            first = set(reps)
+            ops.split_tanh_relu_indexed(src, idx, ws.net, ws.inp, self.hidden_dim, self.context_dim,
+                                        inp_rows=[r if b in first else -1 for b, r in enumerate(ws.ctx_map)])
+        elif isinstance(cnet_feat, tuple):
             ops.split_tanh_relu_indexed(cnet_feat[0], cnet_feat[1], ws.net, ws.inp, self.hidden_dim, self.context_dim)
         else:
             ops.split_tanh_relu(cnet_feat, ws.net, ws.inp, self.hidden_dim, self.context_dim)
@@ -180,7 +187,7 @@
                     st.wait_stream(main)
                 ws = self._workspace(b1 - b0, h, w, dev)
                 self._prepare_context(ws, (cnet_feat[0], cnet_feat[1][b0:b1]) if indexed else cnet_feat[b0:b1],
-                                      ctx_ids[b0:b1] if ctx_ids is not None else None)
+                                      ctx_ids[b0:b1] if ctx_ids is not None else None, share=packed is not None)
                 fi = flow_init[b0:b1] if flow_init is not None else None
                 coords1 = ops.coords_grid(b1 - b0, h, w, dev, flow_init=fi)
             state.append((st, corr_fn, ws, coords1))
diff --git a/accflow_amd/networks/raft/update.py b/accflow_amd/networks/raft/update.py
--- a/accflow_amd/networks/raft/update.py
+++ b/accflow_amd/networks/raft/update.py
@@ -8,6 +8,20 @@
 
 FUSE_LOOKUP = os.environ.get("ACCFLOW_FUSE_LOOKUP", "1") == "1"
 USE_H16_STATE = os.environ.get("ACCFLOW_H16_STATE", "1") == "1"
+
+CTX_PER_FRAME = os.environ.get("ACCFLOW_CTX_PER_FRAME", "1") == "1"
+
+
+def context_rows(ids):
+    if ids is None or not CTX_PER_FRAME or len(set(ids)) == len(ids):
+        return None
+    slot, reps, rows = {}, [], []
+    for b, key in enumerate(ids):
+        if key not in slot:
+            slot[key] = len(reps)
+            reps.append(b)
+        rows.append(slot[key])
+    return reps, rows
 
 
 def h16_state_supported():
@@ -74,6 +88,7 @@
             self.head = buf(256)
         self.mask = None
         self.gru_pre = None
+        self.ctx_map = None
         if self.s16:
             def s(c, zero=False):
                 return ops.S16.empty(B, c, h, w, device, zero=zero)
@@ -304,7 +319,8 @@
     def gru_context(self, ws):
         B, h, w, hd = ws.B, ws.h, ws.w, ws.hidden
         ws.gru_pre = {}
-        inp = ops.to_s16(ws.inp) if ws.s16 else ws.inp
+        inp = ws.inp if ws.ctx_map is None else ws.inp[:max(ws.ctx_map) + 1]
+        inp = ops.to_s16(inp) if ws.s16 else inp
         p32 = ws.s16 and ws.net_in_h16
         for s in ("1", "2"):
             _, zrc, _, qc = self._gru_packs(s)
@@ -326,17 +342,17 @@
             for s in ("1", "2"):
                 zrv, _, qv, _ = self._gru_packs(s)
                 ops.conv2d(zrv, ws.h16, in1=ws.x16, out=ws.z, act=ops.ACT_SIGMOID, epi=ops.EPI_GRU_ZR, e0=ws.h16 if h16s else ws.net,
-                           out16=ws.rh16, fp32_out=False, pre=ws.gru_pre["zr" + s], algo_cin=cin, cache=(D, "zr" + s))
+                           out16=ws.rh16, fp32_out=False, pre=ws.gru_pre["zr" + s], pre_map=ws.ctx_map, algo_cin=cin, cache=(D, "zr" + s))
                 ops.conv2d(qv, ws.rh16, in1=ws.x16, out=None if h16s else ws.net, act=ops.ACT_TANH, epi=ops.EPI_GRU_Q,
                            e0=ws.h16 if h16s else ws.net, e1=ws.z, out16=ws.h16, fp32_out=not h16s,
-                           pre=ws.gru_pre["q" + s], algo_cin=cin, cache=(D, "q" + s))
+                           pre=ws.gru_pre["q" + s], pre_map=ws.ctx_map, algo_cin=cin, cache=(D, "q" + s))
             return
         for s in ("1", "2"):
             zrv, _, qv, _ = self._gru_packs(s)
             ops.conv2d(zrv, ws.net, in1=rest, out=ws.z, act=ops.ACT_SIGMOID, epi=ops.EPI_GRU_ZR, e0=ws.net, out2=ws.rh,
-                       pre=ws.gru_pre["zr" + s], algo_cin=cin)
+                       pre=ws.gru_pre["zr" + s], pre_map=ws.ctx_map, algo_cin=cin)
             ops.conv2d(qv, ws.rh, in1=rest, out=ws.net, act=ops.ACT_TANH, epi=ops.EPI_GRU_Q, e0=ws.net, e1=ws.z,
-                       pre=ws.gru_pre["q" + s], algo_cin=cin)
+                       pre=ws.gru_pre["q" + s], pre_map=ws.ctx_map, algo_cin=cin)
 
     def flow_delta(self, ws, coords1=None, out=None):
         pk, f = self._packs, self.flow_head
diff --git a/accflow_amd/ops.py b/accflow_amd/ops.py
--- a/accflow_amd/ops.py
+++ b/accflow_amd/ops.py
@@ -422,13 +422,32 @@
                     alloc_out="fp32_or_lone", s16_e0="any")
 
 
+_PRE_MAPS_LOCK = threading.Lock()
+_PRE_MAPS = {}
+
+
+def _pre_map_tensor(pre_map, B, rows, dev, who):
+    key = tuple(int(r) for r in pre_map)
+    if len(key) != B or any(r < 0 or r >= rows for r in key):
+        raise RuntimeError("%s: pre_map needs %d entries in [0, %d), got %r" % (who, B, rows, key))
+    dev = torch.device(dev)
+    t = _PRE_MAPS.get((dev, key))
+    if t is None:
+        with _PRE_MAPS_LOCK:
+            t = _PRE_MAPS.get((dev, key))
+            if t is None:
+                t = _PRE_MAPS[(dev, key)] = torch.tensor(key, dtype=torch.int32, device=dev)
+    return t
+
+
 def _set_src(s, ptr, bs, C, Hs, Ws, geo):
     s.ptr, s.bs, s.C, s.Hs, s.Ws = ptr, bs, C, Hs, Ws
     s.step, s.oy, s.ox, s.KH, s.KW, s.padH, s.padW = geo
 
 
 def _conv_desc(form, pk, srcs, act, epi, md, out=None, out16=None, fp32_out=True, e0=None, e1=None, out2=None, pre=None,
-               p32_out=False, offset=None, dmask=None, in_norm=None, stats=False, kws_ok=False, out_hw=None, lay=None, tg=None):
+               p32_out=False, offset=None, dmask=None, in_norm=None, stats=False, kws_ok=False, out_hw=None, lay=None, tg=None,
+               pre_map=None):
     lib = _lib.load()
     who = form.who
     d = ConvDesc()
@@ -526,10 +545,17 @@
         d.e1_bs, d.e1 = _plane4(e1, "e1"), e1.data_ptr()
     if out2 is not None:
         d.out2_bs, d.out2 = _plane4(out2, "out2"), out2.data_ptr()
+    pmap = None
     if pre is not None:
-        if epi not in (EPI_GRU_ZR, EPI_GRU_Q) or tuple(pre.shape) != (B, pk.Cout, OH, OW):
-            raise RuntimeError("%s: `pre` is a (B, Cout, OH, OW) addend of the GRU epilogues" % who)
+        rows = B if pre_map is None else pre.shape[0]
+        if epi not in (EPI_GRU_ZR, EPI_GRU_Q) or tuple(pre.shape) != (rows, pk.Cout, OH, OW):
+            raise RuntimeError("%s: `pre` is a (B, Cout, OH, OW) addend of the GRU epilogues (with pre_map: one entry per row)" % who)
         d.pre_bs, d.pre = _plane4(pre, "pre"), pre.data_ptr()
+        if pre_map is not None:
+            pmap = _pre_map_tensor(pre_map, B, rows, dev, who)
+            d.pre_map, d.pre_rows = pmap.data_ptr(), rows
+    elif pre_map is not None:
+        raise RuntimeError("%s: pre_map indexes the rows of `pre`, which is missing" % who)
     if p32_out:
         if epi != EPI_STORE or out is None or pk.Cout % 128 or isinstance(e0, S16):
             raise RuntimeError("conv2d: p32_out is a plain fp32 store onto a multiple of 128 channels")
@@ -557,7 +583,7 @@
             st = ConvStats(torch.empty((B, pk.Cout, slots, 3), dtype=torch.float32, device=dev), slots)
             d.stats, d.stat_slots = st.partial.data_ptr(), slots
     ret = out if (out is not None and (fp32_out or out16 is None)) else out16
-    return d, ret, st, (d, pk, srcs, out, out16, e0, e1, out2, pre, ws, offset, dmask, in_norm, tg)
+    return d, ret, st, (d, pk, srcs, out, out16, e0, e1, out2, pre, pmap, ws, offset, dmask, in_norm, tg)
 
 
 def _conv_figures(pk, d, tag, algo_cin):
@@ -571,7 +597,7 @@
 
 def conv2d(pk, in0, in1=None, out=None, act=ACT_NONE, epi=EPI_STORE, e0=None, e1=None, out2=None,
            offset=None, dmask=None, mode=None, want_stats=False, pre=None, algo_cin=None, in_norm=None, out16=None,
-           fp32_out=True, cache=None, p32_out=False):
+           fp32_out=True, cache=None, p32_out=False, pre_map=None):
     r = _replay(cache, "accflow_conv2d_f32")
     if r is not None:
         return r
@@ -588,7 +614,7 @@
         if md != CONV_F16X3 or (pk.wpatch16 is None and pk.wsplit16 is None):
             raise RuntimeError("conv2d: S16 tensors need the f16x3 mode and a direct-kernel weight pack")
         d, ret, _, keep = _conv_desc(_FORM_S16, pk, (in0, in1), act, epi, md, out, out16, fp32_out, e0, e1, out2, pre, p32_out,
-                                     kws_ok=not isinstance(e0, S16) and not p32_out)
+                                     kws_ok=not isinstance(e0, S16) and not p32_out, pre_map=pre_map)
         return _launch(_lib.load().accflow_conv2d_f32, (ctypes.byref(d),), "accflow_conv2d_f32 (S16)",
                        ("conv2d", lambda: _conv_figures(pk, d, " S16in" if d.in_fmt else " S16", algo_cin)), cache, ret, keep)
     if p32_out or isinstance(e0, S16):
@@ -596,14 +622,14 @@
     if want_stats:
         if act != ACT_NONE or epi != EPI_STORE or offset is not None:
             raise RuntimeError("conv2d: statistics are gathered for plain convolutions only (store, no activation)")
-        pre = algo_cin = None
-    r = _conv2d(pk, in0, in1, out, act, epi, e0, e1, out2, offset, dmask, md, want_stats, pre, algo_cin, in_norm)
+        pre = algo_cin = pre_map = None
+    r = _conv2d(pk, in0, in1, out, act, epi, e0, e1, out2, offset, dmask, md, want_stats, pre, algo_cin, in_norm, pre_map)
     if r is None:
         return None
     return r if want_stats else r[0]
 
 
-def _conv2d(pk, in0, in1, out, act, epi, e0, e1, out2, offset, dmask, md, want_stats, pre, algo_cin, in_norm):
+def _conv2d(pk, in0, in1, out, act, epi, e0, e1, out2, offset, dmask, md, want_stats, pre, algo_cin, in_norm, pre_map=None):
     lib = _lib.load()
     if (pk.ztaps is not None and md != CONV_F32 and offset is None and epi in (EPI_STORE, EPI_ACCUM, EPI_RES_RELU)
             and (isinstance(in0, S16) or in0.shape[0] * in0.shape[2] * in0.shape[3] >= TAPSUM_MIN_PIXELS)):
@@ -622,7 +648,8 @@
         cols = _deform_columns(pk, in0, offset, dmask)
         return conv2d(pk.zcols, cols, out=out, act=act, epi=epi, e0=e0, e1=e1, out2=out2, mode=md), None
     b = _conv_desc(_FORM_F32, pk, (in0, in1), act, epi, md, out, e0=e0, e1=e1, out2=out2, pre=pre, offset=offset, dmask=dmask,
-                   in_norm=in_norm, stats=want_stats and USE_NORM_STATS, kws_ok=pk.wpatch is not None and USE_PATCH)
+                   in_norm=in_norm, stats=want_stats and USE_NORM_STATS, kws_ok=pk.wpatch is not None and USE_PATCH,
+                   pre_map=pre_map)
     if b is None:
         return None
     d, ret, st, _ = b
@@ -1449,15 +1476,22 @@
            "accflow_split_tanh_relu_f32")
 
 
-def split_tanh_relu_indexed(cnet_items, idx, net, inp, hd, cd):
+def split_tanh_relu_indexed(cnet_items, idx, net, inp, hd, cd, inp_rows=None):
     lib = _lib.load()
     cnet_items = _dense(cnet_items, "cnet")
     n, _, H, W = cnet_items.shape
     B = len(idx)
     nbs, ibs = _plane4(net, "net"), _plane4(inp, "inp")
-    if net.shape[0] != B or inp.shape[0] != B:
+    if net.shape[0] != B or (inp.shape[0] != B and inp_rows is None):
         raise RuntimeError("split_tanh_relu_indexed: one index per output item")
     arr = (ctypes.c_int * B)(*idx)
+    if inp_rows is not None:
+        if len(inp_rows) != B:
+            raise RuntimeError("split_tanh_relu_indexed: one inp row (or -1) per output item")
+        rows = (ctypes.c_int * B)(*inp_rows)
+        _check(lib.accflow_split_tanh_relu_rows_f32(_p(cnet_items), n, arr, rows, _p(net), nbs, _p(inp), ibs, inp.shape[0], B, hd, cd,
+                                                    H * W, _stream()), "accflow_split_tanh_relu_rows_f32")
+        return
     _check(lib.accflow_split_tanh_relu_idx_f32(_p(cnet_items), n, arr, _p(net), nbs, _p(inp), ibs, B, hd, cd, H * W, _stream()),
            "accflow_split_tanh_relu_idx_f32")
 
diff --git a/include/accflow_hip.h b/include/accflow_hip.h
--- a/include/accflow_hip.h
+++ b/include/accflow_hip.h
@@ -65,6 +65,7 @@
   const void* wsplit16;
   float* stats; int stat_slots;
   const float* pre; long long pre_bs;
+  const int* pre_map; int pre_rows;
   const float* in_norm;
   float acc_scale;
   int in_fmt;
@@ -222,6 +223,9 @@
                                 long long inp_bs, int B, int hd, int cd, int HW, void* stream);
 int accflow_split_tanh_relu_idx_f32(const float* cnet, int n_items, const int* idx, float* net, long long net_bs, float* inp,
                                     long long inp_bs, int B, int hd, int cd, int HW, void* stream);
+int accflow_split_tanh_relu_rows_f32(const float* cnet, int n_items, const int* idx, const int* inp_row, float* net,
+                                     long long net_bs, float* inp, long long inp_bs, int inp_rows, int B, int hd, int cd, int HW,
+                                     void* stream);
 
 int accflow_coords_grid_f32(float* coords, const float* flow_init, int B, int H8, int W8,
                             void* stream);
```
